# bastienjacquet/CudaDepthMapIntegration

Measured on AMD Instinct MI355X. Metric: Gvoxel-projections/s, higher is better.
Workload: dtype f64

## Files before the change

### cudadepthmapintegration_amd/csrc/dmi_capi.hip

```cpp
#include "dmi_context.h"

#include <chrono>
#include <cmath>
#include <cstdio>
#include <cstdlib>
#include <cstring>
#include <limits>

using dmi::Batch;
using dmi::drain_c2p;
using dmi::drain_events;
using dmi::EventPair;
using dmi::fail;
using dmi::flush_zero_fill;
using dmi::fuse_views;
using dmi::grid_axis_aligned;
using dmi::tile_eligible;
using dmi::FuseArgs;
using dmi::FuseConfig;
using dmi::guarded;
using dmi::MapRec;
using dmi::TileArgs;
using dmi::TileMapRec;

// ... 289 lines not shown
  if (!std::isfinite(czmin)) return;
  const bool per_lane = !(czmin > 0.0) || !(Sc / czmin + 1.0 < 0x1p22);
  const double pmax = per_lane ? 0.0 : Sc / czmin + 1.0;
  const bool index_exact = ((int64_t)ctx->views.H + 2 * dmi::kValidMargin + 8) * ((int64_t)ctx->views.W + 2 * dmi::kValidMargin) + ctx->views.H +
                               2 * dmi::kValidMargin < (int64_t(1) << 24);
  double e1 = cerr + 3.0 * 0x1p-24 * Dz * pmax + 0x1p-22 * Dz + nl * (pmax + 2.0) + 0x1p-53 * std::max(Sx, Sy);
  e1 *= 1.0 + 0x1p-10;
  t.t1_erel = 0x1p-22f * (1.0f + 0x1p-10f);
  t.t1_hspan = float_not_below(D * (1.0 + 0x1p-20));
  if (!(pmax < 0x1p22) || !index_exact || !(e1 > 0x1p-100) || !(Sc < 0x1p60) || !std::isfinite(e1)) return;
  t.t1_e1 = float_not_below(e1);
  t.t1_ok = 1;
  {
    const double *sp = ctx->grid.spacing;
    double d[3][2], c[3];
    for (int ax = 0; ax < 3; ++ax) {
      const double wxs = g[ax] * sp[ax], wys = g[4 + ax] * sp[ax], wzs = g[8 + ax] * sp[ax];
      d[ax][0] = (Pc[0] * wxs + Pc[1] * wys) + Pc[2] * wzs;
      d[ax][1] = (Qc[0] * wxs + Qc[1] * wys) + Qc[2] * wzs;
      c[ax] = (S[0] * wxs + S[1] * wys) + S[2] * wzs;
    }
    const double xpix = (double)(std::max(ctx->views.W, ctx->views.H) / 2 + dmi::kValidMargin + 1);
    const double xmax = xpix + (double)std::max(dmi::kWinAnchorX, dmi::kWinAnchorY);
    const double nl2 = 2.0 * nl;
    const double pwin = (dmi::kWinReach + 0.5) * dmi::kWinCzRatio + 3.0;
    const double steps[3] = {7.0, 7.0, (double)(kMaxColumn - 1)};
    double e_step = 0.0;
    for (int xy = 0; xy < 2; ++xy) {
      double e = 0.0;
      for (int ax = 0; ax < 3; ++ax) e += steps[ax] * (std::fabs(d[ax][xy]) + xmax * std::fabs(c[ax]));
      e_step = std::max(e_step, e * 0x1p-23);
    }
    double ew = (cerr + xmax * nl2) + e_step + pwin * nl2 + 0x1p-53 * std::max(Sx, Sy);
    ew *= 1.0 + 0x1p-10;
    bool ok = std::isfinite(ew) && ew > 0x1p-100 && ew < 0x1p60;
    for (int ax = 0; ax < 3; ++ax) ok = ok && std::fabs(d[ax][0]) < 0x1p60 && std::fabs(d[ax][1]) < 0x1p60 && std::fabs(c[ax]) < 0x1p60;
    if (ok) {
      for (int xy = 0; xy < 2; ++xy) {
        win->di[xy] = (float)d[0][xy];
        win->dj[xy] = (float)d[1][xy];
        win->dk[xy] = (float)d[2][xy];
      }
      win->ci[0] = (float)c[0]; win->ci[1] = (float)(c[0] * (double)dmi::kWinC1);
      win->cj[0] = (float)c[1]; win->cj[1] = (float)(c[1] * (double)dmi::kWinC1);
      win->ck[0] = (float)c[2]; win->ck[1] = (float)(c[2] * (double)dmi::kWinC1);
      win->e_abs = float_not_below(ew);
      for (int cnr = 0; cnr < 8; ++cnr) {
        const double ni = (cnr & 1) ? 7.0 : 0.0, nj = (cnr & 2) ? 7.0 : 0.0;
        for (int v = 0; v < 2; ++v) {
          const double nk = (cnr & 4) ? (v ? 15.0 : 7.0) : 0.0;
          float *dst = v ? foot->s16[cnr] : foot->s8[cnr];
          dst[0] = (float)((ni * d[0][0] + nj * d[1][0]) + nk * d[2][0]);
          dst[1] = (float)((ni * d[0][1] + nj * d[1][1]) + nk * d[2][1]);
          dst[2] = (float)((ni * c[0] + nj * c[1]) + nk * c[2]);
        }
      }
      foot->ferr = float_not_below(cerr + xpix * nl2);
    }
  }
  if (per_lane) {
    const double B = (3.0 * 0x1p-24 * Dz + nl) * (1.0 + 0x1p-10) * (1.0 + 0x1p-10);
    if (!(B < 0x1p60) || !(B >= 0.0)) {
      t.t1_ok = 0;
      t.t1_e1 = std::numeric_limits<float>::infinity();
      return;
    }
    t.t1_b = float_not_below(B);
    t.t1_ok = 2;
  }
}

TileMapRec make_tile_rec(const dmi_context *ctx, const MapRec &r, dmi::WinRec *win, dmi::FootRec *foot, double *zscale_out) {
  TileMapRec t;
  std::memset(&t, 0, sizeof(t));
  const double *rt = r.rt, *k = r.k;
  t.rz0 = rt[8];
  t.rz1 = rt[9];
  t.rz3 = rt[11];
  const bool general = classify_k(r.k, r.rt) == dmi::K_GENERAL;
  double P[4], Q[4], S[4];
  for (int c = 0; c < 4; ++c) {
    if (general) {
      P[c] = (k[0] * rt[c] + k[1] * rt[4 + c]) + k[2] * rt[8 + c];
      Q[c] = (k[4] * rt[c] + k[5] * rt[4 + c]) + k[6] * rt[8 + c];
      S[c] = (k[8] * rt[c] + k[9] * rt[4 + c]) + k[10] * rt[8 + c];
    } else {
      P[c] = k[0] * rt[c] + k[1] * rt[4 + c] + k[2] * rt[8 + c];
      Q[c] = k[5] * rt[4 + c] + k[6] * rt[8 + c];
      S[c] = rt[8 + c];
    }
  }
  if (general) {
    P[3] += k[3];
    Q[3] += k[7];
    S[3] += k[11];
  }
  t.px = P[0]; t.py = P[1]; t.pz = P[2]; t.p0 = P[3];
  t.qx = Q[0]; t.qy = Q[1]; t.qz = Q[2]; t.q0 = Q[3];
  t.sx = S[0]; t.sy = S[1]; t.sz = S[2]; t.s0 = S[3];
  const double *g = ctx->grid.grid_matrix;
  const double sz = ctx->grid.spacing[2];
  t.dhx = (P[0] * (g[2] * sz) + P[1] * (g[6] * sz)) + P[2] * (g[10] * sz);
  t.dhy = (Q[0] * (g[2] * sz) + Q[1] * (g[6] * sz)) + Q[2] * (g[10] * sz);
  t.dhz = (S[0] * (g[2] * sz) + S[1] * (g[6] * sz)) + S[2] * (g[10] * sz);
  double wm[3];
  const bool aligned = grid_axis_aligned(ctx->grid);
  if (aligned) {
    double lo[3], hi[3];
    voxel_world(ctx->grid, 0, 0, ctx->opt.z_first, lo);
    voxel_world(ctx->grid, ctx->grid.cell_dims[0] - 1, ctx->grid.cell_dims[1] - 1,
                ctx->opt.z_first + ctx->grid.cell_dims[2] - 1 + kMaxColumn, hi);
    for (int a = 0; a < 3; ++a) wm[a] = std::max(std::fabs(lo[a]), std::fabs(hi[a]));
  } else {
    double gm[3];
    for (int a = 0; a < 3; ++a)
      gm[a] = std::fabs(ctx->grid.origin[a]) +
              (ctx->grid.cell_dims[a] + 1.0 + (a == 2 ? ctx->opt.z_first + kMaxColumn : 0)) * std::fabs(ctx->grid.spacing[a]);
    for (int a = 0; a < 3; ++a)
      wm[a] = std::fabs(g[4 * a]) * gm[0] + std::fabs(g[4 * a + 1]) * gm[1] + std::fabs(g[4 * a + 2]) * gm[2] + std::fabs(g[4 * a + 3]);
  }
  double M[3];
  for (int row = 0; row < 3; ++row)
    M[row] = std::fabs(rt[4 * row]) * wm[0] + std::fabs(rt[4 * row + 1]) * wm[1] + std::fabs(rt[4 * row + 2]) * wm[2] +
             std::fabs(rt[4 * row + 3]);
  const double Sx = std::fabs(k[0]) * M[0] + std::fabs(k[1]) * M[1] + std::fabs(k[2]) * M[2] + (general ? std::fabs(k[3]) : 0.0);
  const double Sy = (general ? std::fabs(k[4]) * M[0] : 0.0) + std::fabs(k[5]) * M[1] + std::fabs(k[6]) * M[2] +
                    (general ? std::fabs(k[7]) : 0.0);
  const double Sz = general ? std::fabs(k[8]) * M[0] + std::fabs(k[9]) * M[1] + std::fabs(k[10]) * M[2] + std::fabs(k[11]) : M[2];
  t.err = std::max(Sx, Sy) * 0x1p-44;
  t.errz = general ? Sz * 0x1p-44 : 0.0;
  t.cz_err = aligned ? 0.0 : M[2] * 0x1p-47;
  double zabs = Sz, czlo = std::numeric_limits<double>::infinity(), czhi = -czlo;
  if (!general) {
    zabs = 0.0;
    for (int c = 0; c < 8; ++c) {
      double w[3];
      voxel_world(ctx->grid, (c & 1) ? ctx->grid.cell_dims[0] - 1 : 0, (c & 2) ? ctx->grid.cell_dims[1] - 1 : 0,
                  ctx->opt.z_first + ((c & 4) ? ctx->grid.cell_dims[2] - 1 + kMaxColumn : 0), w);
      const double cz = ((rt[8] * w[0] + rt[9] * w[1]) + rt[10] * w[2]) + rt[11];
      zabs = std::max(zabs, std::fabs(cz));
      czlo = std::min(czlo, cz);
      czhi = std::max(czhi, cz);
    }
    zabs = zabs * (1.0 + 0x1p-20) + (aligned ? 1.0 : 2.0) * 32.0 * 0x1p-52 * M[2];
    if (!std::isfinite(zabs)) zabs = Sz;
  }
  double zscale = 1.0;
  if (!general && std::isfinite(czlo) && std::isfinite(czhi)) zscale = std::max(1.0, std::max(czlo, czhi / 16.0));
  t.errk = (t.err + 65536.0 * t.errz) + 0x1p-22 * zabs * (1.0 + 0x1p-20);
  t.depth = r.depth;
  make_centred_rows(ctx, r, P, Q, S, Sx, Sy, M, zabs, zscale, general, aligned, &t, win, foot);
  if (zscale_out) *zscale_out = zscale;
  return t;
}

int add_views_impl(dmi_context *ctx, const double *depth64, const float *depth32, const double *best_cost,
                   double threshold, const double *K4, const double *RT4, int32_t n, int32_t width, int32_t height) {
  if (!ctx) return DMI_ERR_INVALID_ARGUMENT;
  if ((!depth64 && !depth32) || !K4 || !RT4) return fail(ctx, DMI_ERR_INVALID_ARGUMENT, "dmi_add_views: null pointer");
  if (n <= 0) return fail(ctx, DMI_ERR_INVALID_ARGUMENT, "dmi_add_views: n must be positive");
  if (width < 1 || height < 1 || width > 32768 || height > 32768)
    return fail(ctx, DMI_ERR_INVALID_ARGUMENT, "dmi_add_views: depth-map dimensions must be in [1, 32768]");
  if (!ctx->views.batches.empty() && (width != ctx->views.W || height != ctx->views.H))
    return fail(ctx, DMI_ERR_INVALID_ARGUMENT, "dmi_add_views: every view of a context must share width and height");
  DMI_HIP(ctx, hipSetDevice(ctx->opt.device));
  const auto t0 = std::chrono::steady_clock::now();
  if (ctx->views.batches.empty()) {
    ctx->views.W = width;
    ctx->views.H = height;
    ctx->views.depth_f64 = ctx->opt.depth_storage == DMI_DEPTH_F64;
    ctx->views.k_mode = ctx->finite_bounded ? (int)dmi::K_PINHOLE : (int)dmi::K_GENERAL;
    ctx->views.max_tile_err = 0.0;
    ctx->views.pyramid = dmi::make_pyramid_desc(width, height);
  }
  const size_t npix = (size_t)width * height;

  Batch b;
  unsigned long long lossy = 0;
  int rc = upload_batch(ctx, depth64, depth32, best_cost, threshold, n, &b, &lossy);
  if (rc != DMI_OK) return rc;
  if (lossy != 0 && !ctx->views.depth_f64 && ctx->opt.depth_storage == DMI_DEPTH_AUTO) {
    (void)hipFree(b.d_depth);
    (void)hipFree(b.d_pyramid);
    ctx->device_bytes -= npix * n * 4 + b.aux_bytes;
    rc = promote_to_f64(ctx);
    if (rc != DMI_OK) return rc;
    rc = upload_batch(ctx, depth64, depth32, best_cost, threshold, n, &b, &lossy);
    if (rc != DMI_OK) return rc;
  }
  ctx->views.batches.push_back(b);
  const size_t esz = depth_elem(ctx);
  for (int32_t m = 0; m < n; ++m) {
    MapRec r;
    std::memset(&r, 0, sizeof(r));
    std::memcpy(r.rt, RT4 + 16 * (size_t)m, 12 * sizeof(double));
    std::memcpy(r.k, K4 + 16 * (size_t)m, 12 * sizeof(double));
    r.depth = static_cast<const char *>(b.d_depth) + (size_t)m * npix * esz;
    r.pyramid = b.d_pyramid + (size_t)m * ctx->views.pyramid.total_tiles;
    ctx->views.h_maps.push_back(r);
    bool finite = true;
    for (int q = 0; q < 12; ++q) finite = finite && bounded(r.k[q]) && bounded(r.rt[q]);
    const int km = classify_k(r.k, r.rt);
    if (km < ctx->views.k_mode) ctx->views.k_mode = km;
    dmi::WinRec wrec;
    dmi::FootRec frec;
    double zscale = 1.0;
    TileMapRec t = make_tile_rec(ctx, r, &wrec, &frec, &zscale);
    t.valid = reinterpret_cast<const uint8_t *>(b.d_pyramid) + b.valid_offset + (size_t)m * (size_t)dmi::valid_map_bytes(ctx->views.W, ctx->views.H);
    t.vm_c0 = ((float)(ctx->views.H / 2 + dmi::kValidMargin) - 3.5f) * 0.125f;
    t.vm_w8 = (float)(8 * (ctx->views.W + 2 * dmi::kValidMargin) - 8);
    t.vm_base = 8 * (ctx->views.W / 2 + dmi::kValidMargin) + ctx->views.H / 2 + dmi::kValidMargin;
    t.vm_bytes = (int32_t)std::min<int64_t>(dmi::valid_map_bytes(ctx->views.W, ctx->views.H), 0x7fffffff);
    t.vbits = reinterpret_cast<const uint32_t *>(reinterpret_cast<const uint8_t *>(b.d_pyramid) + b.bits_offset +
                                                 (size_t)m * (size_t)dmi::valid_bits_bytes(ctx->views.W, ctx->views.H));
    t.vb_bytes = (int32_t)std::min<int64_t>(dmi::valid_bits_bytes(ctx->views.W, ctx->views.H), 0x7fffffff);
    t.vb_rowskip = (dmi::valid_bits_tiles_x(ctx->views.W) - 1) * 128;
    t.vb_mx = 0x4B400000 + dmi::kValidMargin + ctx->views.W / 2;
    t.vb_my = 0x4B400000 + dmi::kValidMargin + ctx->views.H / 2;
    ctx->views.h_tile_maps.push_back(t);
    wrec.vbits = t.vbits;
    ctx->views.h_win_recs.push_back(wrec);
    ctx->views.h_foot_recs.push_back(frec);
    if (!(t.err <= ctx->views.max_tile_err)) ctx->views.max_tile_err = t.err;
    ctx->views.view_k_mode.push_back((uint8_t)km);
    ctx->views.view_tile_ok.push_back(finite && t.err < 0x1p-12 * zscale && 65536.0 * t.errz < 0x1p-14 && t.cerrk < 0x1p-11 * zscale ? 1 : 0);
  }
  ctx->views.maps_dirty = true;
  ctx->timings.last_upload_ms =
      std::chrono::duration<double, std::milli>(std::chrono::steady_clock::now() - t0).count();
  return DMI_OK;
}

constexpr int64_t kConvertChunk = int64_t(32) << 20;

int ensure_convert_stage(dmi_context *ctx) {
  return dmi::ensure_buffer(ctx, ctx->volume.convert, (uint64_t)std::min<int64_t>(kConvertChunk, ctx->n_voxels) * 8);
}

template <typename HostT>
int upload_converted(dmi_context *ctx, const HostT *src) {
  int rc = ensure_convert_stage(ctx);
  if (rc != DMI_OK) return rc;
  const size_t gsz = grid_elem(ctx);
  for (int64_t i0 = 0; i0 < ctx->n_voxels; i0 += kConvertChunk) {
    const int64_t n = std::min<int64_t>(kConvertChunk, ctx->n_voxels - i0);
    DMI_HIP(ctx, hipMemcpyAsync(ctx->volume.convert.ptr, src + i0, (size_t)n * sizeof(HostT), hipMemcpyHostToDevice, ctx->stream));
    DMI_HIP(ctx, dmi::launch_convert_grid(ctx->volume.convert.ptr, sizeof(HostT) == 8 ? 1 : 0, static_cast<char *>(ctx->volume.d_grid) + (size_t)i0 * gsz, n,
                                          ctx->stream));
  }
  DMI_HIP(ctx, hipStreamSynchronize(ctx->stream));
  return DMI_OK;
}

template <typename HostT>
int download_converted(dmi_context *ctx, HostT *dst) {
  int rc = ensure_convert_stage(ctx);
  if (rc != DMI_OK) return rc;
  const size_t gsz = grid_elem(ctx);
  for (int64_t i0 = 0; i0 < ctx->n_voxels; i0 += kConvertChunk) {
    const int64_t n = std::min<int64_t>(kConvertChunk, ctx->n_voxels - i0);
    DMI_HIP(ctx, dmi::launch_convert_grid(static_cast<const char *>(ctx->volume.d_grid) + (size_t)i0 * gsz, gsz == 8 ? 1 : 0, ctx->volume.convert.ptr, n,
                                          ctx->stream));
    DMI_HIP(ctx, hipMemcpyAsync(dst + i0, ctx->volume.convert.ptr, (size_t)n * sizeof(HostT), hipMemcpyDeviceToHost, ctx->stream));
  }
  DMI_HIP(ctx, hipStreamSynchronize(ctx->stream));
  return DMI_OK;
}

}

extern "C" {

int dmi_abi_version(void) { return DMI_ABI_VERSION; }
size_t dmi_sizeof_info(void) { return sizeof(dmi_info); }
size_t dmi_sizeof_timings(void) { return sizeof(dmi_timings); }

int dmi_get_upload_kernel_ms(dmi_context *ctx, double *last, double *total) {
  if (!ctx) return DMI_ERR_INVALID_ARGUMENT;
  if (last) *last = ctx->views.last_upload_kernel_ms;
  if (total) *total = ctx->views.total_upload_kernel_ms;
  return DMI_OK;
}

int dmi_device_count(void) {
  int n = 0;
  if (hipGetDeviceCount(&n) != hipSuccess) {
    (void)hipGetLastError();
    return 0;
  }
  return n;
}

void dmi_default_options(dmi_options *opt) {
  if (!opt) return;
  std::memset(opt, 0, sizeof(*opt));
  opt->device = 0;
  opt->grid_dtype = DMI_F64;
  opt->depth_storage = DMI_DEPTH_AUTO;
}

const char *dmi_last_error(const dmi_context *ctx) { return ctx ? ctx->err.c_str() : g_create_error.c_str(); }

int dmi_create(const dmi_grid_desc *grid, const dmi_ray_potential *ray, const dmi_options *opt, dmi_context **out) {
  return guarded(nullptr, "dmi_create", [&]() -> int {
  auto bad = [](const char *m) {
    g_create_error = m;
    return (int)DMI_ERR_INVALID_ARGUMENT;
  };
  if (!grid || !ray || !out) return bad("dmi_create: null argument");
  *out = nullptr;
  for (int a = 0; a < 3; ++a)
    if (grid->cell_dims[a] < 1) return bad("dmi_create: cell_dims must be >= 1 (vtk point dims >= 2)");
  dmi_options o;
  dmi_default_options(&o);
  if (opt) o = *opt;
  if (o.grid_dtype != DMI_F32 && o.grid_dtype != DMI_F64) return bad("dmi_create: grid_dtype must be DMI_F32 or DMI_F64");
  if (o.depth_storage < DMI_DEPTH_AUTO || o.depth_storage > DMI_DEPTH_F64) return bad("dmi_create: bad depth_storage");
  if (o.z_first < 0 || (int64_t)o.z_first + grid->cell_dims[2] > (int64_t)0x3fffffff) return bad("dmi_create: z_first out of range");
  if (ray->rho == 0 && ray->thickness == 0) return bad("dmi_create: ray potential rho and thickness are both 0 (filt.cxx:138)");
  if ((int64_t)(grid->cell_dims[1] + 3) / 4 > 65535 || (int64_t)grid->cell_dims[2] > 65535)
    return bad("dmi_create: grid too large for one launch (ny <= 262140, nz <= 65535)");
  int ndev = dmi_device_count();
  if (ndev <= 0) return (g_create_error = "dmi_create: no HIP device available", (int)DMI_ERR_DEVICE);
  if (o.device < 0 || o.device >= ndev) return bad("dmi_create: device ordinal out of range");

  dmi_context *ctx = new (std::nothrow) dmi_context();
  if (!ctx) return (g_create_error = "dmi_create: host allocation failed", (int)DMI_ERR_OUT_OF_MEMORY);
  ctx->grid = *grid;
  ctx->ray = *ray;
  ctx->opt = o;
  ctx->n_voxels = (int64_t)grid->cell_dims[0] * grid->cell_dims[1] * grid->cell_dims[2];
  ctx->finite_bounded = true;
  for (int i = 0; i < 12; ++i) ctx->finite_bounded = ctx->finite_bounded && bounded(grid->grid_matrix[i]);
  for (int a = 0; a < 3; ++a)
    ctx->finite_bounded = ctx->finite_bounded && bounded(grid->origin[a]) &&
                          bounded(grid->spacing[a] * (grid->cell_dims[a] + 1.0 + (a == 2 ? o.z_first : 0)));

  auto hip_fail = [&](hipError_t e, const char *what) {
    (void)hipGetLastError();
    g_create_error = std::string("dmi_create: ") + what + ": " + hipGetErrorString(e);
    int code = e == hipErrorOutOfMemory ? DMI_ERR_OUT_OF_MEMORY : DMI_ERR_DEVICE;
    dmi_destroy(ctx);
    return code;
  };
  hipError_t e = hipSetDevice(o.device);
  if (e != hipSuccess) return hip_fail(e, "hipSetDevice");
  if (o.stream) {
    ctx->stream = static_cast<hipStream_t>(o.stream);
  } else {
    e = hipStreamCreateWithFlags(&ctx->stream, hipStreamNonBlocking);
    if (e != hipSuccess) return hip_fail(e, "hipStreamCreate");
    ctx->own_stream = true;
  }
  {
    int least = 0, greatest = 0;
    if (hipDeviceGetStreamPriorityRange(&least, &greatest) != hipSuccess) {
      (void)hipGetLastError();
      least = greatest = 0;
    }
    e = hipStreamCreateWithPriority(&ctx->upload_stream, hipStreamNonBlocking, greatest);
  }
  if (e != hipSuccess) return hip_fail(e, "hipStreamCreate(upload)");
  int rc = DMI_OK;
  auto own_failed = [&](int code) {
    rc = code;
    if (rc != DMI_OK) g_create_error = "dmi_create: " + ctx->err;
  };
  if (o.external_grid) {
    hipPointerAttribute_t attr;
    e = hipPointerGetAttributes(&attr, o.external_grid);
    if (e != hipSuccess || attr.type != hipMemoryTypeDevice) {
      (void)hipGetLastError();
      g_create_error = "dmi_create: external_grid is not a device pointer";
      dmi_destroy(ctx);
      return DMI_ERR_INVALID_ARGUMENT;
    }
    ctx->volume.d_grid = o.external_grid;
  } else {
    own_failed(dmi::ensure_buffer(ctx, ctx->volume.owned, ctx->n_voxels * grid_elem(ctx)));
    ctx->volume.d_grid = ctx->volume.owned.ptr;
    ctx->volume.own_grid = true;
  }
  if (rc == DMI_OK && o.count_hits) own_failed(dmi::ensure_buffer(ctx, ctx->hits.voxel, ctx->n_voxels * sizeof(uint32_t)));
  if (rc == DMI_OK) own_failed(dmi::ensure_buffer(ctx, ctx->views.lossy, 3 * sizeof(unsigned long long)));
  if (rc == DMI_OK && (hipEventCreate(&ctx->views.up_events[0]) != hipSuccess || hipEventCreate(&ctx->views.up_events[1]) != hipSuccess)) {
    (void)hipGetLastError();
    dmi::destroy_events(ctx->views.up_events);
  }
  if (rc == DMI_OK) own_failed(dmi_reset_grid(ctx));
  if (rc != DMI_OK) {
    dmi_destroy(ctx);
    return rc;
  }
  *out = ctx;
  return DMI_OK;
  });
}

void dmi_destroy(dmi_context *ctx) {
  if (!ctx) return;
  (void)hipSetDevice(ctx->opt.device);
  if (ctx->stream) (void)hipStreamSynchronize(ctx->stream);
  if (ctx->upload_stream) {
    (void)hipStreamSynchronize(ctx->upload_stream);
    (void)hipStreamDestroy(ctx->upload_stream);
  }
  for (EventPair &p : ctx->pending) {
    (void)hipEventDestroy(p.start);
    (void)hipEventDestroy(p.stop);
    (void)hipEventDestroy(p.mid);
  }
  for (EventPair &p : ctx->pool) {
    (void)hipEventDestroy(p.start);
    (void)hipEventDestroy(p.stop);
    (void)hipEventDestroy(p.mid);
  }
  ctx->views.release();
  ctx->hits.release();
  ctx->volume.release();
  ctx->tables.release();
  ctx->c2p.release();
  ctx->mesh.release();
  ctx->extraction.release();
  ctx->components.release();
  ctx->smoothing.release();
  ctx->decimation.release();
  ctx->support.release();
  ctx->coloration.release();
  for (hipEvent_t e : ctx->slab_events) (void)hipEventDestroy(e);
  if (ctx->download_stream) (void)hipStreamDestroy(ctx->download_stream);
  if (ctx->own_stream && ctx->stream) (void)hipStreamDestroy(ctx->stream);
  delete ctx;
}

int dmi_add_views(dmi_context *ctx, const double *depth, const double *best_cost, double threshold, const double *K4,
                  const double *RT4, int32_t n, int32_t width, int32_t height) {
  return guarded(ctx, "dmi_add_views", [&]() -> int {
  return add_views_impl(ctx, depth, nullptr, best_cost, threshold, K4, RT4, n, width, height);
  });
}

int dmi_add_views_f32(dmi_context *ctx, const float *depth, const double *K4, const double *RT4, int32_t n,
                      int32_t width, int32_t height) {
  return guarded(ctx, "dmi_add_views_f32", [&]() -> int {
  return add_views_impl(ctx, nullptr, depth, nullptr, 0.0, K4, RT4, n, width, height);
  });
}

int dmi_clear_views(dmi_context *ctx) {
  return guarded(ctx, "dmi_clear_views", [&]() -> int {
  if (!ctx) return DMI_ERR_INVALID_ARGUMENT;
  DMI_HIP(ctx, hipSetDevice(ctx->opt.device));
  DMI_HIP(ctx, hipStreamSynchronize(ctx->stream));
  const size_t npix = (size_t)ctx->views.W * ctx->views.H;
  for (Batch &b : ctx->views.batches) {
    (void)hipFree(b.d_depth);
    (void)hipFree(b.d_pyramid);
    ctx->device_bytes -= npix * b.n * depth_elem(ctx) + b.aux_bytes;
  }
  ctx->views.batches.clear();
  ctx->views.h_maps.clear();
  ctx->views.h_tile_maps.clear();
  ctx->views.h_win_recs.clear();
  ctx->views.h_foot_recs.clear();
  ctx->views.view_k_mode.clear();
  ctx->views.view_tile_ok.clear();
  ctx->views.max_tile_err = 0.0;
  ctx->views.maps_dirty = true;
  ctx->views.W = ctx->views.H = 0;
  return DMI_OK;
  });
}

int dmi_reset_grid(dmi_context *ctx) {
  return guarded(ctx, "dmi_reset_grid", [&]() -> int {
  if (!ctx) return DMI_ERR_INVALID_ARGUMENT;
  DMI_HIP(ctx, hipSetDevice(ctx->opt.device));
  if (ctx->volume.own_grid) {
    ctx->volume.zero_fill_pending = true;
  } else {
    DMI_HIP(ctx, hipMemsetAsync(ctx->volume.d_grid, 0, ctx->n_voxels * grid_elem(ctx), ctx->stream));
  }
  if (ctx->hits.voxel.ptr) DMI_HIP(ctx, hipMemsetAsync(ctx->hits.voxel.ptr, 0, ctx->n_voxels * sizeof(uint32_t), ctx->stream));
  if (ctx->hits.map.ptr)
    DMI_HIP(ctx, hipMemsetAsync(ctx->hits.map.ptr, 0, ctx->hits.map.capacity, ctx->stream));
  ctx->volume.layer_is_zero.assign((size_t)ctx->grid.cell_dims[2], 1);
  ctx->volume.grid_free_of_negative_zero = ctx->volume.own_grid;
  ctx->c2p.valid = false;
  return DMI_OK;
  });
}

int dmi_upload_grid(dmi_context *ctx, const double *grid) {
  return guarded(ctx, "dmi_upload_grid", [&]() -> int {
  if (!ctx || !grid) return fail(ctx, DMI_ERR_INVALID_ARGUMENT, "dmi_upload_grid: null argument");
  DMI_HIP(ctx, hipSetDevice(ctx->opt.device));
  ctx->volume.zero_fill_pending = false;
  if (ctx->opt.grid_dtype == DMI_F64) {
    DMI_HIP(ctx, hipMemcpyAsync(ctx->volume.d_grid, grid, ctx->n_voxels * 8, hipMemcpyHostToDevice, ctx->stream));
    DMI_HIP(ctx, hipStreamSynchronize(ctx->stream));
  } else {
    int rc_ = upload_converted<double>(ctx, grid);
    if (rc_ != DMI_OK) return rc_;
  }
  ctx->volume.layer_is_zero.assign((size_t)ctx->grid.cell_dims[2], 0);
  ctx->volume.grid_free_of_negative_zero = false;
  ctx->c2p.valid = false;
  return DMI_OK;
  });
}

int dmi_synchronize(dmi_context *ctx) {
  return guarded(ctx, "dmi_synchronize", [&]() -> int {
  if (!ctx) return DMI_ERR_INVALID_ARGUMENT;
  DMI_HIP(ctx, hipSetDevice(ctx->opt.device));
  DMI_HIP(ctx, hipStreamSynchronize(ctx->stream));
  return drain_events(ctx);
  });
}

int dmi_download_grid_f64(dmi_context *ctx, double *out) {
  return guarded(ctx, "dmi_download_grid_f64", [&]() -> int {
  if (!ctx || !out) return fail(ctx, DMI_ERR_INVALID_ARGUMENT, "dmi_download_grid_f64: null argument");
  DMI_HIP(ctx, hipSetDevice(ctx->opt.device));
  { int rc_ = flush_zero_fill(ctx); if (rc_ != DMI_OK) return rc_; }
  const auto t0 = std::chrono::steady_clock::now();
  if (ctx->opt.grid_dtype == DMI_F64) {
    DMI_HIP(ctx, hipMemcpyAsync(out, ctx->volume.d_grid, ctx->n_voxels * 8, hipMemcpyDeviceToHost, ctx->stream));
    DMI_HIP(ctx, hipStreamSynchronize(ctx->stream));
  } else {
    int rc_ = download_converted<double>(ctx, out);
    if (rc_ != DMI_OK) return rc_;
  }
  ctx->timings.last_download_ms =
      std::chrono::duration<double, std::milli>(std::chrono::steady_clock::now() - t0).count();
  return drain_events(ctx);
  });
}

int dmi_download_grid_f32(dmi_context *ctx, float *out) {
  return guarded(ctx, "dmi_download_grid_f32", [&]() -> int {
  if (!ctx || !out) return fail(ctx, DMI_ERR_INVALID_ARGUMENT, "dmi_download_grid_f32: null argument");
  DMI_HIP(ctx, hipSetDevice(ctx->opt.device));
  { int rc_ = flush_zero_fill(ctx); if (rc_ != DMI_OK) return rc_; }
  const auto t0 = std::chrono::steady_clock::now();
  if (ctx->opt.grid_dtype == DMI_F32) {
    DMI_HIP(ctx, hipMemcpyAsync(out, ctx->volume.d_grid, ctx->n_voxels * 4, hipMemcpyDeviceToHost, ctx->stream));
    DMI_HIP(ctx, hipStreamSynchronize(ctx->stream));
  } else {
    int rc_ = download_converted<float>(ctx, out);
    if (rc_ != DMI_OK) return rc_;
  }
  ctx->timings.last_download_ms =
      std::chrono::duration<double, std::milli>(std::chrono::steady_clock::now() - t0).count();
  return drain_events(ctx);
  });
}

int dmi_fuse_range_download(dmi_context *ctx, int32_t first, int32_t count, void *out, int32_t out_dtype, int32_t n_slabs) {
  return guarded(ctx, "dmi_fuse_range_download", [&]() -> int {
  if (!ctx || !out) return fail(ctx, DMI_ERR_INVALID_ARGUMENT, "dmi_fuse_range_download: null argument");
  if (out_dtype != DMI_F64 && out_dtype != DMI_F32) return fail(ctx, DMI_ERR_INVALID_ARGUMENT, "dmi_fuse_range_download: out_dtype must be DMI_F32 or DMI_F64");
  DMI_HIP(ctx, hipSetDevice(ctx->opt.device));
  const int32_t n_views = (int32_t)ctx->views.h_maps.size();
  if (first < 0 || count < 0 || first > n_views || count > n_views - first)
    return fail(ctx, DMI_ERR_INVALID_ARGUMENT, "dmi_fuse_range_download: range outside the resident views");
  const int32_t nz = ctx->grid.cell_dims[2];
  const int32_t max_slabs = std::max(1, (nz + DMI_SLAB_ALIGNMENT - 1) / DMI_SLAB_ALIGNMENT);
  n_slabs = std::min(std::max(n_slabs, 1), max_slabs);
  if (out_dtype != ctx->opt.grid_dtype || n_slabs == 1) {
    if (count > 0) {
      int rc = fuse_views(ctx, first, count, 0, nz);
      if (rc != DMI_OK) return rc;
    }
    return out_dtype == DMI_F64 ? dmi_download_grid_f64(ctx, static_cast<double *>(out)) : dmi_download_grid_f32(ctx, static_cast<float *>(out));
  }
  { int rc_ = flush_zero_fill(ctx); if (rc_ != DMI_OK) return rc_; }
  if (!ctx->download_stream) DMI_HIP(ctx, hipStreamCreateWithFlags(&ctx->download_stream, hipStreamNonBlocking));
  while ((int32_t)ctx->slab_events.size() < n_slabs) {
    hipEvent_t e = nullptr;
    DMI_HIP(ctx, hipEventCreateWithFlags(&e, hipEventDisableTiming));
    ctx->slab_events.push_back(e);
  }
  const auto t0 = std::chrono::steady_clock::now();
  const int32_t units = max_slabs, per = units / n_slabs, extra = units % n_slabs;
  const size_t gsz = grid_elem(ctx);
  const size_t layer = (size_t)ctx->grid.cell_dims[0] * ctx->grid.cell_dims[1];
  int32_t z0 = 0;
  for (int32_t i = 0; i < n_slabs; ++i) {
    const int32_t z1 = std::min(nz, z0 + (per + (i < extra ? 1 : 0)) * DMI_SLAB_ALIGNMENT);
    if (count > 0) {
      int rc = fuse_views(ctx, first, count, z0, z1 - z0);
      if (rc != DMI_OK) {
        (void)hipStreamSynchronize(ctx->download_stream);
        return rc;
      }
    }
    hipError_t he = hipEventRecord(ctx->slab_events[(size_t)i], ctx->stream);
    if (he == hipSuccess) he = hipStreamWaitEvent(ctx->download_stream, ctx->slab_events[(size_t)i], 0);
    if (he == hipSuccess)
      he = hipMemcpyAsync(static_cast<char *>(out) + (size_t)z0 * layer * gsz, static_cast<const char *>(ctx->volume.d_grid) + (size_t)z0 * layer * gsz,
                          (size_t)(z1 - z0) * layer * gsz, hipMemcpyDeviceToHost, ctx->download_stream);
    if (he != hipSuccess) {
      (void)hipStreamSynchronize(ctx->download_stream);
      (void)hipGetLastError();
      return fail(ctx, DMI_ERR_DEVICE, std::string("dmi_fuse_range_download: ") + hipGetErrorString(he));
    }
    z0 = z1;
  }
  DMI_HIP(ctx, hipStreamSynchronize(ctx->download_stream));
  DMI_HIP(ctx, hipStreamSynchronize(ctx->stream));
  ctx->timings.last_download_ms =
      std::chrono::duration<double, std::milli>(std::chrono::steady_clock::now() - t0).count();
  return drain_events(ctx);
  });
}

// ... 237 lines not shown
```

### cudadepthmapintegration_amd/csrc/dmi_capi_fuse.hip

```cpp
#include "dmi_context.h"

#include <algorithm>
#include <cmath>
#include <cstdlib>
#include <cstring>

using dmi::drain_events;
using dmi::EventPair;
using dmi::fail;
using dmi::flush_zero_fill;
using dmi::FuseArgs;
using dmi::FuseConfig;
using dmi::guarded;
using dmi::MapRec;
using dmi::TileArgs;
using dmi::TileMapRec;

namespace {

int sync_maps(dmi_context *ctx) {
  dmi_context::Views &v = ctx->views;
  const size_t n = v.h_maps.size();
  const size_t cap = std::max<size_t>(64, n * 2);
  bool fresh = false;
  int rc = dmi::ensure_idle_buffers(ctx, {{&v.maps, n * sizeof(MapRec), cap * sizeof(MapRec)},
                                          {&v.tile_maps, n * sizeof(TileMapRec), cap * sizeof(TileMapRec)},
                                          {&v.win_recs, n * sizeof(dmi::WinRec), cap * sizeof(dmi::WinRec)},
                                          {&v.foot_recs, n * sizeof(dmi::FootRec), cap * sizeof(dmi::FootRec)}}, &fresh);
  if (rc != DMI_OK) return rc;
  if (fresh) v.maps_dirty = true;
  dmi::DeviceBuffer &hits = ctx->hits.map;
  if (ctx->opt.count_hits && !dmi::holds(hits, n * sizeof(unsigned long long))) {
    dmi::DeviceBuffer grown;
    rc = dmi::ensure_buffer(ctx, grown, cap * sizeof(unsigned long long));
    if (rc != DMI_OK) return rc;
    hipError_t e = hipMemsetAsync(grown.ptr, 0, grown.capacity, ctx->stream);
    if (e == hipSuccess && hits.ptr) {
      e = hipMemcpyAsync(grown.ptr, hits.ptr, hits.capacity, hipMemcpyDeviceToDevice, ctx->stream);
      if (e == hipSuccess) e = hipStreamSynchronize(ctx->stream);
    }
    if (e != hipSuccess) {
      (void)hipGetLastError();
      dmi::drop_buffers(ctx, {&grown});
      return fail(ctx, DMI_ERR_DEVICE, std::string("growth of the views' hit counters: ") + hipGetErrorString(e));
    }
    std::swap(grown, hits);
    dmi::drop_buffers(ctx, {&grown});
  }
  if (v.maps_dirty) {
    DMI_HIP(ctx, hipMemcpyAsync(v.maps.ptr, v.h_maps.data(), n * sizeof(MapRec), hipMemcpyHostToDevice, ctx->stream));
    DMI_HIP(ctx, hipMemcpyAsync(v.tile_maps.ptr, v.h_tile_maps.data(), n * sizeof(TileMapRec), hipMemcpyHostToDevice, ctx->stream));
    DMI_HIP(ctx, hipMemcpyAsync(v.win_recs.ptr, v.h_win_recs.data(), n * sizeof(dmi::WinRec), hipMemcpyHostToDevice, ctx->stream));
    DMI_HIP(ctx, hipMemcpyAsync(v.foot_recs.ptr, v.h_foot_recs.data(), n * sizeof(dmi::FootRec), hipMemcpyHostToDevice, ctx->stream));
    v.maps_dirty = false;
  }
  return DMI_OK;
}

int slot_permutation(dmi_context *ctx, int32_t super_x, int32_t super_y, int32_t super_z, bool zmajor, const int32_t **out) {
  std::vector<dmi_context::SlotPerm> &perms = ctx->tables.slot_perms;
  for (const auto &sp : perms)
    if (sp.super_x == super_x && sp.super_y == super_y && sp.super_z == super_z && sp.zmajor == (zmajor ? 1 : 0)) {
      *out = sp.perm.as<int32_t>();
      return DMI_OK;
    }
  if (super_x > 1023 || super_y > 1023 || super_z > 1023)
    return fail(ctx, DMI_ERR_INVALID_ARGUMENT, "dmi_fuse: more than 1023 super-bricks along an axis");
  const size_t n = (size_t)super_x * super_y * super_z;
  auto spread = [](uint64_t v) {
    v &= 0x3ff;
    v = (v | (v << 16)) & 0x030000ffull;
    v = (v | (v << 8)) & 0x0300f00full;
    v = (v | (v << 4)) & 0x030c30c3ull;
    v = (v | (v << 2)) & 0x09249249ull;
    return v;
  };
  std::vector<std::pair<uint64_t, int32_t>> keyed(n);
  size_t q = 0;
  for (int32_t z = 0; z < super_z; ++z)
    for (int32_t y = 0; y < super_y; ++y)
      for (int32_t x = 0; x < super_x; ++x, ++q)
        keyed[q] = {zmajor ? (uint64_t)q : (spread(x) | (spread(y) << 1) | (spread(z) << 2)), x | (y << 10) | (z << 20)};
  if (!zmajor) std::sort(keyed.begin(), keyed.end());
  std::vector<int32_t> perm(n);
  for (size_t i = 0; i < n; ++i) perm[i] = keyed[i].second;
  dmi::DeviceBuffer d;
  const int rc = dmi::ensure_buffer(ctx, d, n * sizeof(int32_t));
  if (rc != DMI_OK) return rc;
  hipError_t e = hipMemcpyAsync(d.ptr, perm.data(), n * sizeof(int32_t), hipMemcpyHostToDevice, ctx->stream);
  if (e == hipSuccess && perms.size() >= 64) {
    e = hipStreamSynchronize(ctx->stream);
    if (e == hipSuccess) {
      for (auto &sp : perms) dmi::drop_buffers(ctx, {&sp.perm});
      perms.clear();
    }
  }
  if (e != hipSuccess) {
    (void)hipGetLastError();
    dmi::drop_buffers(ctx, {&d});
    return fail(ctx, DMI_ERR_DEVICE, std::string("slot permutation upload: ") + hipGetErrorString(e));
  }
  perms.push_back({super_x, super_y, super_z, zmajor ? 1 : 0, d});
  *out = d.as<int32_t>();
  return DMI_OK;
}


FuseArgs general_args(const dmi_context *ctx, int32_t first, int32_t count, int32_t z_first, int32_t z_count) {
  FuseArgs a;
  std::memset(&a, 0, sizeof(a));
  a.nx = ctx->grid.cell_dims[0];
  a.ny = ctx->grid.cell_dims[1];
  a.nz = ctx->grid.cell_dims[2];
  a.W = ctx->views.W;
  a.H = ctx->views.H;
  a.first_map = first;
  a.n_maps = count;
  a.init_from_grid = 0;
  for (int32_t z = z_first; z < z_first + z_count; ++z)
    if (!ctx->volume.layer_is_zero[(size_t)z]) a.init_from_grid = 1;
  a.kz0 = ctx->opt.z_first;
  a.k_first = z_first;
  a.k_count = z_count;
  a.ox = ctx->grid.origin[0];
  a.oy = ctx->grid.origin[1];
  a.oz = ctx->grid.origin[2];
  a.sx = ctx->grid.spacing[0];
  a.sy = ctx->grid.spacing[1];
  a.sz = ctx->grid.spacing[2];
  std::memcpy(a.g, ctx->grid.grid_matrix, 12 * sizeof(double));
  a.thick = ctx->ray.thickness;
  a.delta = ctx->ray.delta;
  a.rho_pos = ctx->ray.rho * 1.0;
  a.rho_neg = ctx->ray.rho * -1.0;
  a.rho_zero = ctx->ray.rho * 0.0;
  a.slope = ctx->ray.rho / ctx->ray.thickness;
  a.free_space = -ctx->ray.eta * ctx->ray.rho;
  a.maps = ctx->views.maps.as<MapRec>();
  a.grid = ctx->volume.d_grid;
  a.voxel_hits = ctx->hits.voxel.as<uint32_t>();
  a.map_hits = ctx->hits.map.as<unsigned long long>();
  return a;
}

dmi::HoleTraits resident_hole_traits(const dmi_context::Views &v) {
  unsigned long long mingled = 0, without = 0, strips = 0, pixels = 0;
  for (const dmi::Batch &bt : v.batches) {
    mingled += bt.mingled_strips;
    without += bt.holes;
    strips += (unsigned long long)bt.n * (unsigned long long)v.W * (unsigned long long)(v.H / 8);
    pixels += (unsigned long long)bt.n * (unsigned long long)v.W * (unsigned long long)v.H;
  }
  return dmi::hole_traits(mingled, without, strips, pixels);
}

int tile_geometry(dmi_context *ctx, const FuseArgs &a, const FuseConfig &cfg, const dmi::TileShape &sh, bool whole_grid, TileArgs *out) {
  TileArgs &t = *out;
  t.nx = a.nx; t.ny = a.ny; t.nz = a.nz; t.W = a.W; t.H = a.H;
  t.first_map = a.first_map; t.n_maps = a.n_maps; t.init_from_grid = a.init_from_grid;
  t.kpad = (a.nz + sh.tk - 1) / sh.tk * sh.tk;
  t.bricks_x = (a.nx + 8 * sh.wx - 1) / (8 * sh.wx);
  t.bricks_y = (a.ny + 8 * sh.wy - 1) / (8 * sh.wy);
  t.bricks_z = t.kpad / sh.tk;
  t.super_x = (t.bricks_x + 3) / 4;
  t.super_y = (t.bricks_y + 3) / 4;
  t.super_z = (t.bricks_z + 1) / 2;
  if (!whole_grid) {
    t.sbz_first = a.k_first / (2 * sh.tk);
    t.super_z = (a.k_first + a.k_count + 2 * sh.tk - 1) / (2 * sh.tk) - t.sbz_first;
  }
  if (t.bricks_x > 2047 || t.bricks_y > 2047 || t.bricks_z > 1023)
    return fail(ctx, DMI_ERR_INVALID_ARGUMENT, "dmi_fuse: more bricks along an axis than the tiled kernel's order entries hold");
  t.slot_base = t.sbz_first * t.super_x * t.super_y * 32;
  t.slot_count = t.super_x * t.super_y * t.super_z * 32;
  const int rc = slot_permutation(ctx, t.super_x, t.super_y, t.super_z, (cfg.variant & dmi::VAR_ZMAJOR_SLOTS) != 0, &t.sb_perm);
  if (rc != DMI_OK) return rc;
  t.xcd_run_wg = 32 * std::max(1, t.super_x * t.super_y);
  if (((int64_t)t.super_x * t.super_y * t.super_z * 32 + 16 * (int64_t)t.xcd_run_wg + 64) > (int64_t)0x7fffffff)
    return fail(ctx, DMI_ERR_INVALID_ARGUMENT, "dmi_fuse: grid too large for one launch");
  t.depth_bytes = (int32_t)((int64_t)a.W * a.H * (ctx->views.depth_f64 ? 8 : 4));
  t.kz0 = a.kz0;
  t.ox = a.ox; t.oy = a.oy; t.oz = a.oz; t.sx = a.sx; t.sy = a.sy; t.sz = a.sz;
  std::memcpy(t.g, a.g, sizeof(t.g));
  t.thick = a.thick; t.delta = a.delta; t.rho_pos = a.rho_pos; t.rho_neg = a.rho_neg;
  t.slope = a.slope; t.free_space = a.free_space;
  t.tile_maps = ctx->views.tile_maps.as<TileMapRec>();
  t.grid = a.grid; t.voxel_hits = a.voxel_hits; t.map_hits = a.map_hits;
  t.rotated = dmi::grid_axis_aligned(ctx->grid) ? 0 : 1;
  t.flags = ((cfg.variant & dmi::VAR_NO_INTERIOR) ? dmi::TILE_FLAG_NO_INTERIOR : 0) |
            ((cfg.variant & dmi::VAR_XCD_RUNS) ? dmi::TILE_FLAG_XCD_RUNS : 0);
  t.maps = ctx->views.maps.as<MapRec>();
  t.wbricks_x = (a.nx + 7) / 8;
  t.wbricks_y = (a.ny + 7) / 8;
  return DMI_OK;
}

int cz_table(dmi_context *ctx, const FuseArgs &a, TileArgs *t) {
  const size_t table_doubles = std::max<size_t>(ctx->views.h_maps.size(), 4) * (size_t)t->kpad;
  const size_t need = table_doubles + (size_t)dmi::kFreeSumsMax + 1;
  const int rc = dmi::ensure_idle_buffer(ctx, ctx->tables.cz_table, need * 8, need * 2 * 8);
  if (rc != DMI_OK) return rc;
  t->cz_table = ctx->tables.cz_table.as<double>();
  if (!a.init_from_grid && !ctx->opt.count_hits && a.n_maps <= dmi::kFreeSumsMax) t->free_sums = t->cz_table + table_doubles;
  return DMI_OK;
}

int zero_row(dmi_context *ctx, TileArgs *t) {
  bool fresh = false;
  const int rc = dmi::ensure_idle_buffer(ctx, ctx->tables.zero_row, (uint64_t)t->class_pitch, (uint64_t)t->class_pitch, &fresh);
  if (rc != DMI_OK) return rc;
  if (fresh) DMI_HIP(ctx, hipMemsetAsync(ctx->tables.zero_row.ptr, dmi::BRICK_MIXED, (size_t)t->class_pitch, ctx->stream));
  t->classes = ctx->tables.zero_row.as<uint8_t>();
  t->class_pitch = 0;
  return DMI_OK;
}

int class_table(dmi_context *ctx, const dmi::TileShape &sh, bool windows, TileArgs *t) {
  const size_t fine_bytes = ((size_t)t->wbricks_x * t->wbricks_y * t->bricks_z * (size_t)t->class_pitch + 255) / 256 * 256;
  const size_t coarse_end = (fine_bytes + (size_t)dmi::coarse_class_bytes(*t, sh.tk) + 255) / 256 * 256;
  const size_t cbytes = coarse_end + (windows ? fine_bytes * sizeof(dmi::WinPair) : 0);
  ctx->tables.coarse_offset = fine_bytes;
  bool fresh = false;
  const int rc = dmi::ensure_idle_buffer(ctx, ctx->tables.classes, cbytes, cbytes, &fresh);
  if (rc != DMI_OK) return rc;
  if (fresh) DMI_HIP(ctx, hipMemsetAsync(ctx->tables.classes.ptr, dmi::BRICK_SKIP, cbytes, ctx->stream));
  t->classes = ctx->tables.classes.as<uint8_t>();
  if (windows) {
    t->win_origin = reinterpret_cast<dmi::WinPair *>(ctx->tables.classes.as<uint8_t>() + coarse_end);
    t->win_delta = (int64_t)reinterpret_cast<intptr_t>(t->win_origin) - 16 * (int64_t)reinterpret_cast<intptr_t>(t->classes);
    t->win_recs = ctx->views.win_recs.as<dmi::WinRec>();
    t->foot_recs = ctx->views.foot_recs.as<dmi::FootRec>();
    t->vb_bytes = (int32_t)std::min<int64_t>(dmi::valid_bits_bytes(ctx->views.W, ctx->views.H), 0x7fffffff);
    t->vb_rowskip = (dmi::valid_bits_tiles_x(ctx->views.W) - 1) * 128;
    t->win_cx = dmi::kValidMargin + ctx->views.W / 2;
    t->win_cy = dmi::kValidMargin + ctx->views.H / 2;
  }
  return DMI_OK;
}

int order_tables(dmi_context *ctx, const dmi::TileShape &sh, int variant, TileArgs *t) {
  const size_t n_slots = (size_t)t->super_x * t->super_y * t->super_z * 32;
  const size_t order_bytes = (n_slots + 1) * sizeof(int32_t), level_bytes = dmi::order_scratch_bytes(n_slots);
  const int rc = dmi::ensure_idle_buffers(ctx, {{&ctx->tables.order, order_bytes, order_bytes}, {&ctx->tables.order_level, level_bytes, level_bytes}});
  if (rc != DMI_OK) return rc;
  t->order = ctx->tables.order.as<int32_t>() + 1;
  t->n_order = ctx->tables.order.as<int32_t>();
  t->order_levels = reinterpret_cast<const int32_t *>(ctx->tables.order_level.as<uint8_t>() + (n_slots + 15) / 16 * 16);
  t->xcd_run_wg = 32 * (4 / (sh.wx * sh.wy));
  if (dmi::cost_order(sh.wx * sh.wy, variant, n_slots)) {
    t->flags |= dmi::TILE_FLAG_COST_ORDER | dmi::TILE_FLAG_XCD_RUNS;
    t->xcd_run_wg = 16;
  }
  return DMI_OK;
}

#ifdef DMI_TUNING
int tuning_hooks(dmi_context *ctx, TileArgs *out) {
  TileArgs &t = *out;
  if (std::getenv("DMI_DEBUG_NO_DEPTH_LOADS")) t.depth_bytes = 0;
  if (std::getenv("DMI_DEBUG_WG_TIMES")) {
    const size_t per_round = 8 * (size_t)t.xcd_run_wg;
    const size_t blocks = ((size_t)t.super_x * t.super_y * t.super_z * 32 + 32 + per_round - 1) / per_round * per_round;
    const size_t bytes = (blocks * 3 + 2) * sizeof(unsigned long long);
    const int rc = dmi::ensure_idle_buffer(ctx, ctx->tables.wg_times, bytes, bytes);
    if (rc != DMI_OK) return rc;
    ctx->tables.wg_times_blocks = blocks;
    DMI_HIP(ctx, hipMemsetAsync(ctx->tables.wg_times.ptr, 0, bytes, ctx->stream));
    t.wg_times = ctx->tables.wg_times.as<unsigned long long>();
    t.wg_times_n = (int64_t)blocks;
  }
  if (const char *e = std::getenv("DMI_DEBUG_PAIRS")) {
    if (!std::strcmp(e, "nowin")) t.flags |= dmi::TILE_FLAG_DBG_SKIP_WINDOW_PAIRS;
    if (!std::strcmp(e, "onlywin")) t.flags |= dmi::TILE_FLAG_DBG_ONLY_WINDOW_PAIRS;
    if (!std::strcmp(e, "nowinloads")) t.flags |= dmi::TILE_FLAG_DBG_NO_WINDOW_LOADS;
  }
  if (const char *e = std::getenv("DMI_XCD_RUN_WG")) {
    t.xcd_run_wg = std::max(1, std::atoi(e));
    if (((int64_t)t.super_x * t.super_y * t.super_z * 32 + 8 * (int64_t)t.xcd_run_wg) > (int64_t)0x7fffffff)
      return fail(ctx, DMI_ERR_INVALID_ARGUMENT, "dmi_fuse: DMI_XCD_RUN_WG makes the launch too large");
  }
  return DMI_OK;
}
#endif

int tile_tables(dmi_context *ctx, const FuseArgs &a, FuseConfig *cfg, const dmi::TileShape &sh, const dmi::HoleTraits &traits, TileArgs *out) {
  TileArgs &t = *out;
  int rc = cz_table(ctx, a, &t);
  if (rc == DMI_OK) rc = dmi::ensure_buffer(ctx, ctx->tables.queue_heads, 128 * sizeof(int32_t));
  if (rc != DMI_OK) return rc;
  t.queue_heads = ctx->tables.queue_heads.as<int32_t>();
  if (dmi::fuse_without_classes(cfg->variant, (int64_t)t.wbricks_x * t.wbricks_y * (int64_t)t.bricks_z, a.n_maps))
    cfg->variant |= dmi::VAR_NO_BRICK_CLASSES;
  t.class_pitch = dmi::class_table_pitch((int32_t)ctx->views.h_maps.size());
  const bool zero_free = dmi::zero_free(a.init_from_grid != 0, ctx->volume.grid_free_of_negative_zero, ctx->opt.count_hits != 0, cfg->variant);
  if (cfg->variant & dmi::VAR_NO_BRICK_CLASSES) {
    rc = zero_row(ctx, &t);
  } else {
    bool any_tier1 = false;
    for (int32_t m = a.first_map; m < a.first_map + a.n_maps && !any_tier1; ++m) any_tier1 = std::isfinite(ctx->views.h_win_recs[(size_t)m].e_abs);
    dmi::WindowsQuestion q;
    q.tier1 = DMI_TIER1 != 0;
    q.general_k = cfg->general_k != 0;
    q.count_hits = cfg->count_hits != 0;
    q.variant = cfg->variant;
    q.holes = cfg->holes != 0;
    q.many_borders = traits.many_borders;
    q.any_tier1 = any_tier1;
    q.zero_free = zero_free;
    q.depth_f64 = ctx->views.depth_f64;
    rc = class_table(ctx, sh, dmi::use_windows(q), &t);
    if (rc == DMI_OK && !(cfg->variant & dmi::VAR_SPATIAL_ORDER)) rc = order_tables(ctx, sh, cfg->variant, &t);
  }
  if (zero_free) t.behind_mask = 0x0101010101010101ull;
  return rc;
}

int timed_launch(dmi_context *ctx, const FuseArgs &a, const TileArgs &t, const FuseConfig &cfg) {
  EventPair ev;
  if (!ctx->pool.empty()) {
    ev = ctx->pool.back();
    ctx->pool.pop_back();
  } else {
    DMI_HIP(ctx, hipEventCreate(&ev.start));
    DMI_HIP(ctx, hipEventCreate(&ev.stop));
    DMI_HIP(ctx, hipEventCreate(&ev.mid));
  }
  ev.has_mid = cfg.use_tile != 0 && !(cfg.variant & dmi::VAR_NO_BRICK_CLASSES);
  DMI_HIP(ctx, hipEventRecord(ev.start, ctx->stream));
  const dmi_context::LaunchTables &tb = ctx->tables;
  hipError_t e = cfg.use_tile ? dmi::launch_fuse_tiled(t, ctx->views.maps.as<MapRec>(), cfg, ctx->views.pyramid, tb.order_level.as<uint8_t>(),
                                                         tb.classes.ptr ? tb.classes.as<uint8_t>() + tb.coarse_offset : nullptr,
                                                         ev.has_mid ? ev.mid : nullptr, ctx->stream) : dmi::launch_fuse(a, cfg, ctx->stream);
  if (e != hipSuccess) {
    ctx->pool.push_back(ev);
    (void)hipGetLastError();
    return fail(ctx, DMI_ERR_DEVICE, std::string("fusion kernel launch: ") + hipGetErrorString(e));
  }
  DMI_HIP(ctx, hipEventRecord(ev.stop, ctx->stream));
  ctx->pending.push_back(ev);
  return DMI_OK;
}

int fuse_run(dmi_context *ctx, int32_t first, int32_t count, int32_t z_first, int32_t z_count, bool tiled, int run_k_mode,
             bool general_k) {
  DMI_HIP(ctx, hipSetDevice(ctx->opt.device));
  int rc = sync_maps(ctx);
  if (rc != DMI_OK) return rc;
  const bool whole_grid = z_first == 0 && z_count == ctx->grid.cell_dims[2];
  if (!whole_grid) {
    rc = flush_zero_fill(ctx);
    if (rc != DMI_OK) return rc;
  }
  const FuseArgs a = general_args(ctx, first, count, z_first, z_count);

  const dmi::HoleTraits traits = resident_hole_traits(ctx->views);
  FuseConfig cfg;
  cfg.depth_is_f64 = ctx->views.depth_f64 ? 1 : 0;
  cfg.grid_is_f64 = ctx->opt.grid_dtype == DMI_F64 ? 1 : 0;
  cfg.k_mode = run_k_mode;
  cfg.count_hits = ctx->opt.count_hits ? 1 : 0;
  cfg.use_tile = tiled ? 1 : 0;
  cfg.general_k = tiled && general_k ? 1 : 0;
  cfg.holes = traits.holes ? 1 : 0;
  cfg.variant = dmi::with_default_tile_shape(ctx->opt.kernel_variant, tiled, traits, a.nx, a.ny, a.nz);

  TileArgs t;
  std::memset(&t, 0, sizeof(t));
  if (cfg.use_tile) {
    const dmi::TileShape sh = dmi::tile_shape(cfg.variant, ctx->views.depth_f64, !dmi::grid_axis_aligned(ctx->grid), cfg.general_k != 0);
    rc = tile_geometry(ctx, a, cfg, sh, whole_grid, &t);
    if (rc == DMI_OK) rc = tile_tables(ctx, a, &cfg, sh, traits, &t);
#ifdef DMI_TUNING
    if (rc == DMI_OK) rc = tuning_hooks(ctx, &t);
#endif
    if (rc == DMI_OK) rc = dmi::ensure_buffer(ctx, ctx->tables.fuse_args, sizeof(FuseArgs));
    if (rc != DMI_OK) return rc;
    DMI_HIP(ctx, hipMemcpyAsync(ctx->tables.fuse_args.ptr, &a, sizeof(FuseArgs), hipMemcpyHostToDevice, ctx->stream));
    t.full = ctx->tables.fuse_args.as<FuseArgs>();
  }

  rc = timed_launch(ctx, a, t, cfg);
  if (rc != DMI_OK) return rc;

  dmi_context::LastLaunch &last = ctx->last;
  last.tiled = cfg.use_tile != 0;
  last.classes = cfg.use_tile != 0 && !(cfg.variant & dmi::VAR_NO_BRICK_CLASSES);
  last.class_bricks = (int64_t)t.wbricks_x * t.wbricks_y * t.bricks_z;
  last.bricks_z = t.bricks_z;
  last.tk = t.bricks_z > 0 ? t.kpad / t.bricks_z : 0;
  last.win_origin = t.win_origin;
  last.class_pitch = t.class_pitch;
  last.first = first;
  last.count = count;
  for (int32_t z = z_first; z < z_first + z_count; ++z) ctx->volume.layer_is_zero[(size_t)z] = 0;
  ctx->volume.zero_fill_pending = false;
  ctx->c2p.valid = false;
  if (ctx->pending.size() >= 256) return drain_events(ctx);
  return DMI_OK;
}

template <typename Visit>
int visit_last_classes(dmi_context *ctx, Visit &&visit) {
  const dmi_context::LastLaunch &last = ctx->last;
  if (!last.classes) return DMI_OK;
  DMI_HIP(ctx, hipSetDevice(ctx->opt.device));
  const size_t bytes = (size_t)last.class_bricks * last.class_pitch;
  std::vector<uint8_t> host(bytes);
  DMI_HIP(ctx, hipMemcpyAsync(host.data(), ctx->tables.classes.ptr, bytes, hipMemcpyDeviceToHost, ctx->stream));
  DMI_HIP(ctx, hipStreamSynchronize(ctx->stream));
  for (int64_t b = 0; b < last.class_bricks; ++b) {
    const uint8_t *row = host.data() + (size_t)b * last.class_pitch + last.first;
    for (int32_t m = 0; m < last.count; ++m) visit(b, row[m]);
  }
  return DMI_OK;
}

}

namespace dmi {

int fuse_views(dmi_context *ctx, int32_t first, int32_t count, int32_t z_first, int32_t z_count) {
  const dmi_context::Views &v = ctx->views;
  const int32_t n_views = (int32_t)v.h_maps.size();
  if (n_views == 0) return fail(ctx, DMI_ERR_STATE, "dmi_fuse: no views resident (call dmi_add_views first)");
  if (first < 0 || count < 0 || first > n_views || count > n_views - first)
    return fail(ctx, DMI_ERR_INVALID_ARGUMENT, "dmi_fuse_range: range outside the resident views");
  if (count == 0) return DMI_OK;
  const bool tile_possible = tile_eligible(ctx);
  int32_t m = first;
  while (m < first + count) {
    const bool tiled = tile_possible && v.view_tile_ok[(size_t)m];
    int32_t e = m;
    int km = dmi::K_PINHOLE;
    bool general_k = false;
    while (e < first + count && (tile_possible && v.view_tile_ok[(size_t)e]) == tiled) {
      km = std::min(km, (int)v.view_k_mode[(size_t)e]);
      general_k = general_k || v.view_k_mode[(size_t)e] == dmi::K_GENERAL;
      ++e;
    }
    const int rc = fuse_run(ctx, m, e - m, z_first, z_count, tiled, km, general_k);
    if (rc != DMI_OK) return rc;
    m = e;
  }
  return DMI_OK;
}

}

extern "C" {

int dmi_fuse_range(dmi_context *ctx, int32_t first, int32_t count) {
  return guarded(ctx, "dmi_fuse_range", [&]() -> int {
  if (!ctx) return DMI_ERR_INVALID_ARGUMENT;
  return dmi::fuse_views(ctx, first, count, 0, ctx->grid.cell_dims[2]);
  });
}

int dmi_fuse_slab(dmi_context *ctx, int32_t z_first, int32_t z_count) {
  return guarded(ctx, "dmi_fuse_slab", [&]() -> int {
  if (!ctx) return DMI_ERR_INVALID_ARGUMENT;
  const int32_t nz = ctx->grid.cell_dims[2];
  if (z_first < 0 || z_count < 0 || z_first > nz || z_count > nz - z_first)
    return fail(ctx, DMI_ERR_INVALID_ARGUMENT, "dmi_fuse_slab: layers outside the grid");
  if (z_first % DMI_SLAB_ALIGNMENT != 0 || (z_first + z_count != nz && (z_first + z_count) % DMI_SLAB_ALIGNMENT != 0))
    return fail(ctx, DMI_ERR_INVALID_ARGUMENT, "dmi_fuse_slab: slab boundaries must be multiples of DMI_SLAB_ALIGNMENT (32) cells");
  if (z_count == 0) return DMI_OK;
  return dmi::fuse_views(ctx, 0, (int32_t)ctx->views.h_maps.size(), z_first, z_count);
  });
}

int dmi_fuse(dmi_context *ctx) {
  return guarded(ctx, "dmi_fuse", [&]() -> int {
  if (!ctx) return DMI_ERR_INVALID_ARGUMENT;
  return dmi_fuse_range(ctx, 0, (int32_t)ctx->views.h_maps.size());
  });
}

int dmi_get_brick_class_histogram(dmi_context *ctx, uint64_t out[4]) {
  return guarded(ctx, "dmi_get_brick_class_histogram", [&]() -> int {
  if (!ctx || !out) return fail(ctx, DMI_ERR_INVALID_ARGUMENT, "dmi_get_brick_class_histogram: null argument");
  out[0] = out[1] = out[2] = out[3] = 0;
  return visit_last_classes(ctx, [&](int64_t, uint8_t c) { out[c & 3] += 1; });
  });
}

int dmi_get_mixed_reason_histogram(dmi_context *ctx, uint64_t out[8]) {
  return guarded(ctx, "dmi_get_mixed_reason_histogram", [&]() -> int {
  if (!ctx || !out) return fail(ctx, DMI_ERR_INVALID_ARGUMENT, "dmi_get_mixed_reason_histogram: null argument");
  for (int i = 0; i < 8; ++i) out[i] = 0;
  return visit_last_classes(ctx, [&](int64_t, uint8_t c) {
    if ((c & 3) == dmi::BRICK_MIXED) out[(c >> 2) & 7] += 1;
  });
  });
}

int dmi_get_window_pair_count(dmi_context *ctx, uint64_t *out) {
  return guarded(ctx, "dmi_get_window_pair_count", [&]() -> int {
  if (!ctx || !out) return fail(ctx, DMI_ERR_INVALID_ARGUMENT, "dmi_get_window_pair_count: null argument");
  *out = 0;
  const dmi_context::LastLaunch &last = ctx->last;
  if (!last.win_origin) return DMI_OK;
  const int64_t per_layer = last.class_bricks / std::max<int64_t>(1, last.bricks_z);
  return visit_last_classes(ctx, [&](int64_t b, uint8_t c) {
    const int64_t bz = b / std::max<int64_t>(1, per_layer);
    if (bz * last.tk + last.tk > ctx->grid.cell_dims[2]) return;
    if ((c & 0x3f) == (dmi::BRICK_MIXED | (dmi::MIXED_FREE_OR_NODEPTH << 2))) *out += 1;
  });
  });
}

}
```

### cudadepthmapintegration_amd/csrc/dmi_context.h

```cpp
#pragma once
#include "../../include/dmi.h"
#include "dmi_buffer.h"
#include "fusion_kernels.h"

#include <exception>
#include <initializer_list>
#include <new>
#include <string>
#include <vector>

namespace dmi {

struct Batch {
  void *d_depth = nullptr;
  DepthTile *d_pyramid = nullptr;
  size_t valid_offset = 0;
  size_t bits_offset = 0;
  size_t aux_bytes = 0;
  int32_t n = 0;
  unsigned long long holes = 0;
  unsigned long long mingled_strips = 0;
};

struct EventPair {
  hipEvent_t start = nullptr, stop = nullptr;
  hipEvent_t mid = nullptr;
  bool has_mid = false;
};

template <size_t N>
void destroy_events(hipEvent_t (&events)[N]) {
  for (hipEvent_t &e : events) {
    if (e) (void)hipEventDestroy(e);
    e = nullptr;
  }
}
}

struct dmi_context {
  dmi_grid_desc grid{};
  dmi_ray_potential ray{};
  dmi_options opt{};
  int64_t n_voxels = 0;

  hipStream_t stream = nullptr;
  bool own_stream = false;
  hipStream_t upload_stream = nullptr;
  hipStream_t download_stream = nullptr;
  std::vector<hipEvent_t> slab_events;

  bool finite_bounded = true;

  struct Views {
    int32_t W = 0, H = 0;
    bool depth_f64 = false;
    int k_mode = dmi::K_PINHOLE;
    std::vector<uint8_t> view_k_mode;
    std::vector<uint8_t> view_tile_ok;
    double max_tile_err = 0.0;
    dmi::PyramidDesc pyramid{};
    std::vector<dmi::Batch> batches;
    std::vector<dmi::MapRec> h_maps;
    std::vector<dmi::TileMapRec> h_tile_maps;
    std::vector<dmi::WinRec> h_win_recs;
    std::vector<dmi::FootRec> h_foot_recs;
    dmi::DeviceBuffer maps, tile_maps, win_recs, foot_recs;
    bool maps_dirty = false;
    dmi::DeviceBuffer stage_depth, stage_cost;
    dmi::DeviceBuffer lossy;
    hipEvent_t up_events[2] = {nullptr, nullptr};
    double last_upload_kernel_ms = 0.0, total_upload_kernel_ms = 0.0;
    void release() {
      for (dmi::Batch &b : batches) {
        (void)hipFree(b.d_depth);
        (void)hipFree(b.d_pyramid);
      }
      batches.clear();
      dmi::free_buffers({&maps, &tile_maps, &win_recs, &foot_recs, &stage_depth, &stage_cost, &lossy});
      dmi::destroy_events(up_events);
    }
  } views;
  struct Hits {
    dmi::DeviceBuffer voxel;
    dmi::DeviceBuffer map;
    void release() { dmi::free_buffers({&voxel, &map}); }
  } hits;
  struct Volume {
    void *d_grid = nullptr;
    dmi::DeviceBuffer owned;
    bool own_grid = false;
    std::vector<uint8_t> layer_is_zero;
    bool zero_fill_pending = false;
    bool grid_free_of_negative_zero = false;
    dmi::DeviceBuffer convert;
    void release() {
      dmi::free_buffers({&owned, &convert});
      d_grid = nullptr;
    }
  } volume;
  struct SlotPerm {
    int32_t super_x, super_y, super_z, zmajor;
    dmi::DeviceBuffer perm;
  };
  struct LaunchTables {
    dmi::DeviceBuffer cz_table;
    dmi::DeviceBuffer fuse_args;
    dmi::DeviceBuffer zero_row;
    dmi::DeviceBuffer classes;
    size_t coarse_offset = 0;
    dmi::DeviceBuffer queue_heads;
    dmi::DeviceBuffer wg_times;
    size_t wg_times_blocks = 0;
    std::vector<SlotPerm> slot_perms;
    dmi::DeviceBuffer order, order_level;
    void release() {
      for (SlotPerm &sp : slot_perms) dmi::free_buffers({&sp.perm});
      slot_perms.clear();
      dmi::free_buffers({&cz_table, &fuse_args, &zero_row, &classes, &queue_heads, &wg_times, &order, &order_level});
    }
  } tables;
  struct LastLaunch {
    bool tiled = false;
    bool classes = false;
    int64_t class_bricks = 0;
    int32_t bricks_z = 0, tk = 0;
    const dmi::WinPair *win_origin = nullptr;
    int32_t class_pitch = 0, first = 0, count = 0;
  } last;

  struct CellToPoint {
    dmi::DeviceBuffer points;
    bool valid = false;
    hipEvent_t events[2] = {nullptr, nullptr};
    bool pending = false;
    void release() { dmi::free_buffers({&points}); dmi::destroy_events(events); }
  } c2p;
  struct Mesh {
    dmi::DeviceBuffer vertices, triangles, normals;
    dmi::DeviceBuffer alt_vertices, alt_triangles, alt_normals;
    dmi::DeviceBuffer region_id, region_size;
    uint64_t n_vertices = 0, n_triangles = 0;
    uint64_t regions = 0;
    bool valid = false;
    bool has_normals = false;
    bool filtered = false;
    dmi::DeviceBuffer color_mean, color_median, color_count;
    dmi::DeviceBuffer alt_color_mean, alt_color_median, alt_color_count;
    bool colored = false;
    void release() {
      dmi::free_buffers({&vertices, &triangles, &normals, &alt_vertices, &alt_triangles, &alt_normals, &region_id, &region_size,
                         &color_mean, &color_median, &color_count, &alt_color_mean, &alt_color_median, &alt_color_count});
    }
  } mesh;
  struct Extraction {
    dmi::DeviceBuffer counts, bases, scan_temp;
    hipEvent_t events[4] = {nullptr, nullptr, nullptr, nullptr};
    double last_kernel_ms = 0.0;
    void release() { dmi::free_buffers({&counts, &bases, &scan_temp}); dmi::destroy_events(events); }
  } extraction;
  struct Components {
    dmi::DeviceBuffer vertex_scratch;
    dmi::DeviceBuffer triangle_scratch, counters, scan_temp;
    hipEvent_t events[5] = {nullptr, nullptr, nullptr, nullptr, nullptr};
    double last_kernel_ms = 0.0;
    uint64_t last_cas_retries = 0;
    double last_pass_ms[4] = {0.0, 0.0, 0.0, 0.0};
    void release() { dmi::free_buffers({&vertex_scratch, &triangle_scratch, &counters, &scan_temp}); dmi::destroy_events(events); }
  } components;
  struct Smoothing {
    dmi::DeviceBuffer vertices;
    dmi::DeviceBuffer keys;
    dmi::DeviceBuffer vertex_scratch;
    dmi::DeviceBuffer temp;
    hipEvent_t events[4] = {nullptr, nullptr, nullptr, nullptr};
    double last_kernel_ms = 0.0;
    double last_pass_ms[3] = {0.0, 0.0, 0.0};
    void release() { dmi::free_buffers({&vertices, &keys, &vertex_scratch, &temp}); dmi::destroy_events(events); }
  } smoothing;
  struct Decimation {
    dmi::DeviceBuffer vertex_scratch;
    dmi::DeviceBuffer triangle_scratch;
    dmi::DeviceBuffer bounds;
    hipEvent_t events[8] = {nullptr, nullptr, nullptr, nullptr, nullptr, nullptr, nullptr, nullptr};
    bool pending = false;
    bool pending_normals = false;
    double last_kernel_ms = 0.0;
    double last_pass_ms[4] = {0.0, 0.0, 0.0, 0.0};
    void release() { dmi::free_buffers({&vertex_scratch, &triangle_scratch, &bounds}); dmi::destroy_events(events); }
  } decimation;

  struct Support {
    dmi::DeviceBuffer counts;
    dmi::DeviceBuffer work, compacted;
    dmi::DeviceBuffer maps;
    dmi::DeviceBuffer vertex_scratch;
    dmi::DeviceBuffer triangle_scratch, scan_temp;
    bool valid = false;
    hipEvent_t events[4] = {nullptr, nullptr, nullptr, nullptr};
    double last_kernel_ms = 0.0;
    double last_pass_ms[3] = {0.0, 0.0, 0.0};
    void release() {
      dmi::free_buffers({&counts, &work, &compacted, &maps, &vertex_scratch, &triangle_scratch, &scan_temp});
      dmi::destroy_events(events);
    }
  } support;

  struct Coloration {
    hipEvent_t events[1] = {nullptr};
    double last_kernel_ms = 0.0;
    void release() { dmi::destroy_events(events); }
  } coloration;

  std::vector<dmi::EventPair> pending, pool;
  dmi_timings timings{};
  uint64_t device_bytes = 0;
  std::string err;
};

namespace dmi {

int fail(dmi_context *ctx, int code, const std::string &msg);
int drain_events(dmi_context *ctx);
int drain_c2p(dmi_context *ctx);
int flush_zero_fill(dmi_context *ctx);
inline size_t grid_elem(const dmi_context *c) { return c->opt.grid_dtype == DMI_F64 ? 8 : 4; }
bool grid_axis_aligned(const dmi_grid_desc &g);
bool tile_eligible(const dmi_context *ctx);
int fuse_views(dmi_context *ctx, int32_t first, int32_t count, int32_t z_first, int32_t z_count);
int ensure_buffer(dmi_context *ctx, DeviceBuffer &buffer, uint64_t bytes);
int ensure_idle_buffers(dmi_context *ctx, std::initializer_list<BufferGrowth> unit, bool *fresh = nullptr);
inline int ensure_idle_buffer(dmi_context *ctx, DeviceBuffer &buffer, uint64_t needed, uint64_t allocate, bool *fresh = nullptr) {
  return ensure_idle_buffers(ctx, {{&buffer, needed, allocate}}, fresh);
}
void drop_buffers(dmi_context *ctx, std::initializer_list<DeviceBuffer *> buffers);
struct BufferNeed {
  DeviceBuffer *buffer;
  uint64_t bytes;
};
int ensure_buffers(dmi_context *ctx, std::initializer_list<BufferNeed> needs);

template <typename Ctx, typename Body>
int guarded_by(int (*fail)(Ctx *, int, const std::string &), Ctx *ctx, const char *entry, Body &&body) noexcept {
  auto report = [&](int code, const char *what) noexcept {
    try {
      return fail(ctx, code, std::string(entry) + ": " + what);
    } catch (...) {
      return code;
    }
  };
  try {
    return body();
  } catch (const std::bad_alloc &) {
    return report(DMI_ERR_OUT_OF_MEMORY, "host allocation failed");
  } catch (const std::exception &e) {
    return report(DMI_ERR_STATE, e.what());
  } catch (...) {
    return report(DMI_ERR_STATE, "unexpected C++ exception");
  }
}
template <typename Body>
int guarded(dmi_context *ctx, const char *entry, Body &&body) noexcept {
  return guarded_by(&fail, ctx, entry, static_cast<Body &&>(body));
}


struct ColorContextShape {
  int32_t device, W, H;
  int64_t n_views;
  bool depth_test;
};
ColorContextShape color_context_shape(const dmi_color_context *c);
struct DeviceColoring {
  const double *points;
  int64_t n;
  uint8_t *mean, *median;
  int32_t *count;
  hipEvent_t after;
  const void *const *fused_tables;
  bool fused_f64;
// ... 18 lines not shown
```

### cudadepthmapintegration_amd/csrc/fusion_classify.hip

```cpp
#include <algorithm>
#include <cstring>

#include <stdlib.h>

#include "fusion_kernels.h"
#include "fusion_device.h"

namespace dmi {

namespace {

template <typename T>
__device__ __forceinline__ T cload(const T *p) {
  return *reinterpret_cast<const T __attribute__((address_space(4))) *>(reinterpret_cast<uintptr_t>(p));
}

__device__ __forceinline__ float float_below(double d) {
  float f = (float)d;
  if ((double)f > d) f = nextafterf(f, -__builtin_inff());
  return f;
}
__device__ __forceinline__ float float_above(double d) {
  float f = (float)d;
  if ((double)f < d) f = nextafterf(f, __builtin_inff());
// ... 403 lines not shown
  uint8_t cls = fp.cls;
  bool speckled = false;
  if (fp.query) {
    const TileAcc d = pyramid_query<5>(maps[m].pyramid, P, fp.x0, fp.x1, fp.y0, fp.y1);
    cls = class_from_bounds(a, d, fp.czmin, fp.czmax);
    speckled = !(d.flags & (TILE_PART_HOLE_FREE | TILE_PART_NO_VALID));
  } else if (fp.partial) {
    cls = border_class<GK>(a, fp, pyramid_query<5>(maps[m].pyramid, P, fp.x0, fp.x1, fp.y0, fp.y1));
  }
  const bool inherit_mixed = cls == (uint8_t)(BRICK_MIXED | (MIXED_FREE_OR_NODEPTH << 2)) && speckled;
  coarse[(int64_t)((cbz * cy_n + cby) * cx_n + cbx) * a.class_pitch + m] = inherit_mixed ? (uint8_t)(cls | COARSE_CHILDREN_WRITTEN) : cls;
  if ((cls & 3) == BRICK_MIXED && !inherit_mixed) return;
  for (int dz = 0; dz < per_z; ++dz) {
    const int bz = bz0 + dz;
    if (bz >= bz_first + bz_count) break;
    for (int dy = 0; dy < 4; ++dy) {
      const int by = cby * 4 + dy;
      if (by >= a.wbricks_y) break;
      for (int dx = 0; dx < 4; ++dx) {
        const int bx = cbx * 4 + dx;
        if (bx >= a.wbricks_x) break;
        classes[(int64_t)((bz * a.wbricks_y + by) * a.wbricks_x + bx) * a.class_pitch + m] = cls;
      }
    }
  }
}

constexpr int kWindow = 16;

template <int kQueryTiles, int kChildren, bool ROT, bool GK>
__global__ __launch_bounds__(256) void classify_kernel(const TileArgs a, const MapRec *__restrict__ maps,
                                                       const PyramidDesc P, int tk, uint8_t *__restrict__ classes,
                                                       const uint8_t *__restrict__ coarse, int group_views) {
  constexpr int children = kChildren;
  constexpr int views_per_wave = 64 / children;
  constexpr int per_z = children / 16;
  __shared__ float2 window_mm[4 * views_per_wave][kWindow * kWindow];
  __shared__ uint8_t window_fl[4 * views_per_wave][kWindow * kWindow];
  const int bz_first = 2 * a.sbz_first;
  const int bz_count = min(2 * a.super_z, a.bricks_z - bz_first);
  const int cx_n = (a.wbricks_x + 3) / 4, cy_n = (a.wbricks_y + 3) / 4;
  const int lane = threadIdx.x & 63, wave = __builtin_amdgcn_readfirstlane(threadIdx.x >> 6);
  const int local = blockIdx.x;
  const int cbx = local % cx_n;
  const int ct = local / cx_n;
  const int cby = ct % cy_n, cbz = ct / cy_n + bz_first / per_z;
  const int chunk0 = blockIdx.y * group_views;
  const uint8_t *__restrict__ crow = coarse + (int64_t)((cbz * cy_n + cby) * cx_n + cbx) * a.class_pitch + a.first_map + chunk0;
  const unsigned long long unproven = __builtin_amdgcn_ballot_w64(
      lane < group_views && chunk0 + lane < a.n_maps && (crow[lane] & (3 | COARSE_CHILDREN_WRITTEN)) == BRICK_MIXED);
  if (unproven == 0) return;
  unsigned long long items = views_per_wave == 1 ? unproven & (0x1111111111111111ull << wave)
                                                 : (unproven | (unproven >> 1)) & (0x0101010101010101ull << (2 * wave));
  const int child = lane % children;
  const int bx = cbx * 4 + (child & 3), by = cby * 4 + ((child >> 2) & 3), bz = cbz * per_z + (child >> 4);
  const bool in_grid = bx < a.wbricks_x && by < a.wbricks_y && bz < bz_first + bz_count;
  uint8_t *__restrict__ out = classes + (int64_t)((bz * a.wbricks_y + by) * a.wbricks_x + bx) * a.class_pitch;
  while (items) {
    const int first = __builtin_ctzll(items);
    items &= items - 1;
    const int rel = first + lane / children;
    const int mm = chunk0 + rel;
    const int m = a.first_map + min(mm, a.n_maps - 1);
    const bool mine = in_grid && ((unproven >> rel) & 1ull);
    const MapRec *__restrict__ mr = maps + m;
    BoxFootprint fp;
    fp.query = false;
    fp.partial = false;
    fp.in_margin = false;
    fp.cls = BRICK_SKIP;
    MapRec mr_u;
    TileMapRec tr_u;
    if constexpr (views_per_wave == 1) {
      const int mu = __builtin_amdgcn_readfirstlane(m);
      const MapRec *src = maps + mu;
      const TileMapRec *tsrc = a.tile_maps + mu;
#pragma unroll
      for (int q = 8; q < 12; ++q) mr_u.rt[q] = cload(&src->rt[q]);
      mr_u.pyramid = cload(&src->pyramid);
      tr_u.px = cload(&tsrc->px); tr_u.py = cload(&tsrc->py); tr_u.pz = cload(&tsrc->pz); tr_u.p0 = cload(&tsrc->p0);
      tr_u.qx = cload(&tsrc->qx); tr_u.qy = cload(&tsrc->qy); tr_u.qz = cload(&tsrc->qz); tr_u.q0 = cload(&tsrc->q0);
      tr_u.err = cload(&tsrc->err);
      tr_u.cz_err = cload(&tsrc->cz_err);
      tr_u.errz = cload(&tsrc->errz);
      if constexpr (GK) {
        tr_u.sx = cload(&tsrc->sx); tr_u.sy = cload(&tsrc->sy); tr_u.sz = cload(&tsrc->sz); tr_u.s0 = cload(&tsrc->s0);
      }
      mr = &mr_u;
      if (mine) {
        fp = box_footprint<ROT, GK>(a, &mr_u, &tr_u, bx * 8, bx * 8 + 7, by * 8, by * 8 + 7, bz * tk, bz * tk + tk - 1);
      }
    } else {
      if (mine) fp = box_footprint<ROT, GK>(a, mr, a.tile_maps + m, bx * 8, bx * 8 + 7, by * 8, by * 8 + 7, bz * tk, bz * tk + tk - 1);
    }
    const bool query = mine && (fp.query || fp.partial);
    uint8_t cls = fp.cls;
    const int li = query ? query_level<kQueryTiles>(P, max(fp.x1 - fp.x0, fp.y1 - fp.y0) + 1) : 0x7fff;
    bool from_window = false;
    {
      float2 *__restrict__ win_mm = window_mm[wave * views_per_wave + lane / children];
      uint8_t *__restrict__ win_fl = window_fl[wave * views_per_wave + lane / children];
      int li_w = li;
      for (int off = children >> 1; off > 0; off >>= 1) li_w = min(li_w, __shfl_xor(li_w, off, 64));
      if (li_w != 0x7fff) {
        const int L = kPyramidMinLevel + li_w;
        const bool at_level = query && li == li_w;
        int tx0 = at_level ? fp.x0 >> L : 0x7fffffff, ty0 = at_level ? fp.y0 >> L : 0x7fffffff;
        int tx1 = at_level ? fp.x1 >> L : -1, ty1 = at_level ? fp.y1 >> L : -1;
        int wx0 = tx0, wy0 = ty0, wx1 = tx1, wy1 = ty1;
        for (int off = children >> 1; off > 0; off >>= 1) {
          wx0 = min(wx0, __shfl_xor(wx0, off, 64));
          wy0 = min(wy0, __shfl_xor(wy0, off, 64));
          wx1 = max(wx1, __shfl_xor(wx1, off, 64));
          wy1 = max(wy1, __shfl_xor(wy1, off, 64));
        }
        if (wx1 - wx0 < kWindow && wy1 - wy0 < kWindow) {
          const DepthTile *__restrict__ level = mr->pyramid + P.offset[li_w];
          const int pitch = P.width[li_w];
          const int ww = wx1 - wx0 + 1, wh = wy1 - wy0 + 1;
          const int tx = child & 15;
          for (int ty = child >> 4; ty < wh; ty += children / 16)
            if (tx < ww) {
              const DepthTile t = level[(wy0 + ty) * pitch + wx0 + tx];
              win_mm[ty * kWindow + tx] = make_float2(t.dmin, t.dmax);
              win_fl[ty * kWindow + tx] = (uint8_t)t.flags;
            }
          __builtin_amdgcn_fence(__ATOMIC_RELEASE, "wavefront");
          __builtin_amdgcn_wave_barrier();
          __builtin_amdgcn_fence(__ATOMIC_ACQUIRE, "wavefront");
          if (at_level) {
            TileAcc d;
            for (int ty = ty0; ty <= ty1; ++ty)
              for (int tx = tx0; tx <= tx1; ++tx) {
                const int w = (ty - wy0) * kWindow + (tx - wx0);
                const float2 mm = win_mm[w];
                d.add_tile(DepthTile{mm.x, mm.y, (uint32_t)win_fl[w], 0u});
              }
            cls = fp.partial ? border_class<GK>(a, fp, d) : class_from_bounds(a, d, fp.czmin, fp.czmax);
            from_window = true;
          }
          __builtin_amdgcn_fence(__ATOMIC_RELEASE, "wavefront");
          __builtin_amdgcn_wave_barrier();
        }
      }
    }
    if (query && !from_window) {
      const TileAcc d = pyramid_query<kQueryTiles>(mr->pyramid, P, fp.x0, fp.x1, fp.y0, fp.y1);
      cls = fp.partial ? border_class<GK>(a, fp, d) : class_from_bounds(a, d, fp.czmin, fp.czmax);
    }
    if (mine) out[m] = cls;
  }
}

constexpr int kOriginViews = 8;
constexpr uint32_t kNotWanted = 0xfffffffeu;
template <bool ROT>
__global__ __launch_bounds__(256) void window_origin_kernel(const TileArgs a, const MapRec *__restrict__ maps, int tk,
                                                            uint8_t *__restrict__ classes, WinPair *__restrict__ origins,
                                                            int group_views) {
  __shared__ WinPair tile[kOriginViews][256 + 1];
  __shared__ int64_t rows[256];
  const int bz_first = 2 * a.sbz_first;
  const int bz_count = min(2 * a.super_z, a.bricks_z - bz_first);
  const int64_t n_bricks = (int64_t)a.wbricks_x * a.wbricks_y * bz_count;
  const int lane = threadIdx.x & 63;
  const int64_t local = (int64_t)blockIdx.x * 256 + threadIdx.x;
  const bool exists = local < n_bricks;
  const int bx = (int)(local % a.wbricks_x);
  const int64_t t = local / a.wbricks_x;
  const int by = (int)(t % a.wbricks_y), bz = (int)(t / a.wbricks_y) + bz_first;
  const int64_t row = (((int64_t)bz * a.wbricks_y + by) * a.wbricks_x + bx) * a.class_pitch;
  const bool eligible = exists && bz * tk + tk <= a.nz;
  (void)lane;
  double wxa, wya, wza;
  {
    const double gx = a.ox + (bx * 8 + 0.5) * a.sx;
    const double gy = a.oy + (by * 8 + 0.5) * a.sy;
    const double gz = a.oz + ((bz * tk + a.kz0) + 0.5) * a.sz;
    wxa = row4(a.g + 0, gx, gy, gz), wya = row4(a.g + 4, gx, gy, gz), wza = row4(a.g + 8, gx, gy, gz);
  }
  const int m_begin = a.first_map, m_end = a.first_map + a.n_maps;
  const int g_lo = (m_begin & ~3) + blockIdx.y * group_views;
  rows[threadIdx.x] = row;
  uint32_t held[kOriginViews / 4];
#pragma unroll
  for (int g = 0; g < kOriginViews / 4; ++g) {
    const int m4 = g_lo + 4 * g;
    held[g] = (eligible && 4 * g < group_views && m4 < m_end) ? *reinterpret_cast<const uint32_t *>(classes + row + m4) : 0u;
#pragma unroll
    for (int q = 0; q < 4; ++q) tile[4 * g + q][threadIdx.x].origin = kNotWanted;
  }
#pragma unroll
  for (int g = 0; g < kOriginViews / 4; ++g) {
    const int m4 = g_lo + 4 * g;
    if (4 * g >= group_views || m4 >= m_end) break;
    const uint32_t c4 = held[g];
#pragma unroll 1
    for (int q = 0; q < 4; ++q) {
      const int m = m4 + q;
      const uint8_t c = (uint8_t)(c4 >> (8 * q));
      const bool want = eligible && m >= m_begin && m < m_end && (c & 0x1f) == (uint8_t)(BRICK_MIXED | (MIXED_FREE_OR_NODEPTH << 2));
      if (__builtin_amdgcn_ballot_w64(want) == 0) continue;
      WinPair wp;
      wp.origin = kNotWanted;
      wp.ax = wp.ay = wp.acz = 0.f;
      if (cload(&a.win_recs[m].e_abs) < __builtin_inff()) {
        const MapRec *src = maps + m;
        const TileMapRec *tsrc = a.tile_maps + m;
        const FootRec *fr = a.foot_recs + m;
        const float(*scp)[4] = tk == 16 ? fr->s16 : fr->s8;
        if (want) {
          const double cza = ((cload(&src->rt[8]) * wxa + cload(&src->rt[9]) * wya) + cload(&src->rt[10]) * wza) + cload(&src->rt[11]);
          const double hxa = __builtin_fma(cload(&tsrc->cpx), wxa, __builtin_fma(cload(&tsrc->cpy), wya, __builtin_fma(cload(&tsrc->cpz), wza, cload(&tsrc->cp0))));
          const double hya = __builtin_fma(cload(&tsrc->cqx), wxa, __builtin_fma(cload(&tsrc->cqy), wya, __builtin_fma(cload(&tsrc->cqz), wza, cload(&tsrc->cq0))));
          const float hx0 = (float)hxa, hy0 = (float)hya, z0 = (float)cza;
          float umin = __builtin_inff(), umax = -__builtin_inff(), vmin = __builtin_inff(), vmax = -__builtin_inff();
          float zmin = __builtin_inff(), zmax = -__builtin_inff();
#pragma unroll
          for (int cnr = 0; cnr < 8; ++cnr) {
            const float z = z0 + cload(&scp[cnr][2]);
            const float r = __builtin_amdgcn_rcpf(z);
            const float u = (hx0 + cload(&scp[cnr][0])) * r, v = (hy0 + cload(&scp[cnr][1])) * r;
            umin = __builtin_fminf(umin, u), umax = __builtin_fmaxf(umax, u);
            vmin = __builtin_fminf(vmin, v), vmax = __builtin_fmaxf(vmax, v);
            zmin = __builtin_fminf(zmin, z), zmax = __builtin_fmaxf(zmax, z);
          }
          const float umag = __builtin_fmaxf(__builtin_fmaxf(__builtin_fabsf(umin), __builtin_fabsf(umax)), __builtin_fmaxf(__builtin_fabsf(vmin), __builtin_fabsf(vmax)));
          const float e = 2.0f * cload(&fr->ferr) * __builtin_amdgcn_rcpf(zmin) * (1.0f + 0x1p-20f) + (0x1p-19f * umag + 0x1p-12f);
          const bool sane = zmin > 0.0f && zmax <= (float)(kWinCzRatio * (1.0 - 0x1p-20)) * zmin && umin > -65536.0f && umax < 65536.0f &&
                            vmin > -65536.0f && vmax < 65536.0f && e < 0.25f;
          if (sane) {
            const int cxc = a.W / 2, cyc = a.H / 2;
            const int x0 = (int)__builtin_ceilf(umin - 0.5f - e) + cxc, x1 = (int)__builtin_floorf(umax + 0.5f + e) + cxc;
            const int y0 = (int)__builtin_ceilf(vmin - 0.5f - e) + cyc, y1 = (int)__builtin_floorf(vmax + 0.5f + e) + cyc;
            if (x0 >= -kValidMargin && y0 >= -kValidMargin && x1 < a.W + kValidMargin && y1 < a.H + kValidMargin &&
                x1 - x0 < kWindowCols && y1 - y0 < kWindowRows) {
              wp.origin = (uint32_t)(x0 + kValidMargin) | ((uint32_t)(y0 + kValidMargin) << 16);
              wp.ax = (float)(hxa - (double)(x0 + kWinAnchorX - cxc) * cza);
              wp.ay = (float)(hya - (double)(y0 + kWinAnchorY - cyc) * cza);
              wp.acz = z0;
            }
          }
        }
      }
      if (want) {
        if (wp.origin != kNotWanted)
          tile[4 * g + q][threadIdx.x] = wp;
        else
          classes[row + m] = (uint8_t)(c | CLASS_NO_WINDOW);
      }
    }
  }
  __syncthreads();
  const int v = threadIdx.x & (kOriginViews - 1);
  const int m = g_lo + v;
  if (v < group_views && m < m_end) {
#pragma unroll
    for (int it = 0; it < 8; ++it) {
      const int b = (threadIdx.x >> 3) + 32 * it;
      const WinPair wp = tile[v][b];
      if (wp.origin != kNotWanted) origins[rows[b] + m] = wp;
    }
  }
}


__device__ __forceinline__ bool slot_to_brick(const TileArgs &a, int slot, int &bx, int &by, int &bz) {
  const int within = slot & 31;
  const int code = a.sb_perm[(slot - a.slot_base) >> 5];
  const int sbx = code & 1023, sby = (code >> 10) & 1023, sbz = (code >> 20) + a.sbz_first;
  bx = sbx * 4 + (within & 3);
  by = sby * 4 + ((within >> 2) & 3);
  bz = sbz * 2 + (within >> 4);
  return bx < a.bricks_x && by < a.bricks_y && bz < a.bricks_z;
}

constexpr int kWorkLevels = 4;

__global__ __launch_bounds__(256) void brick_work_kernel(const TileArgs a, int wx, int wy, int n_slots,
                                                         uint8_t *__restrict__ level) {
  const int lane = threadIdx.x & 63;
  const int slot = blockIdx.x * 4 + (threadIdx.x >> 6);
  if (slot >= n_slots) return;
  int bx, by, bz;
  if (!slot_to_brick(a, slot + a.slot_base, bx, by, bz)) {
    if (lane == 0) level[slot] = 255;
    return;
  }
  int mixed = 0, total = 0;
  for (int v = 0; v < wy; ++v)
    for (int u = 0; u < wx; ++u) {
      const int wbx = bx * wx + u, wby = by * wy + v;
      if (wbx >= a.wbricks_x || wby >= a.wbricks_y) continue;
      const uint8_t *row = a.classes + (((int64_t)bz * a.wbricks_y + wby) * a.wbricks_x + wbx) * (int64_t)a.class_pitch;
      for (int m = a.first_map + lane; m < a.first_map + a.n_maps; m += 64) mixed += (row[m] & 3) == BRICK_MIXED ? 1 : 0;
      total += a.n_maps;
    }
  for (int off = 32; off > 0; off >>= 1) mixed += __shfl_xor(mixed, off, 64);
  if (lane == 0) level[slot] = mixed * 2 >= total ? 0 : (mixed * 4 >= total ? 1 : (mixed * 16 >= total ? 2 : 3));
}

constexpr int kOrderChunk = 1024;

__global__ __launch_bounds__(kOrderChunk) void order_count_kernel(const uint8_t *__restrict__ level, int n_slots,
                                                                  int *__restrict__ counts) {
  const int s = blockIdx.x * kOrderChunk + threadIdx.x;
  const int l = s < n_slots ? level[s] : 255;
  for (int q = 0; q < kWorkLevels; ++q) {
    const int c = __syncthreads_count(l == q);
    if (threadIdx.x == 0) counts[blockIdx.x * kWorkLevels + q] = c;
  }
}

__global__ __launch_bounds__(1024) void order_base_kernel(int *__restrict__ counts, int n_chunks, int *__restrict__ n_valid) {
  __shared__ int wave_totals[16];
  __shared__ int carry;
  if (threadIdx.x == 0) carry = 0;
  __syncthreads();
  const int lane = threadIdx.x & 63, wave = threadIdx.x >> 6;
  for (int q = 0; q < kWorkLevels; ++q)
    for (int c0 = 0; c0 < n_chunks; c0 += 1024) {
      const int c = c0 + threadIdx.x;
      const int v = c < n_chunks ? counts[c * kWorkLevels + q] : 0;
      int incl = v;
      for (int off = 1; off < 64; off <<= 1) {
        const int up = __shfl_up(incl, off, 64);
        if (lane >= off) incl += up;
      }
      if (lane == 63) wave_totals[wave] = incl;
      __syncthreads();
      int before = carry, all = 0;
      for (int w = 0; w < 16; ++w) {
        if (w < wave) before += wave_totals[w];
        all += wave_totals[w];
      }
      if (c < n_chunks) counts[c * kWorkLevels + q] = before + incl - v;
      __syncthreads();
      if (threadIdx.x == 0) carry += all;
      __syncthreads();
    }
  if (threadIdx.x == 0) *n_valid = carry;
}

__global__ __launch_bounds__(kOrderChunk) void order_scatter_kernel(const TileArgs a, const uint8_t *__restrict__ level,
                                                                    int n_slots, const int *__restrict__ bases,
                                                                    int *__restrict__ order) {
  __shared__ unsigned long long wave_totals[16];
  const int s = blockIdx.x * kOrderChunk + threadIdx.x;
  const int l = s < n_slots ? level[s] : 255;
  const unsigned long long one = l < kWorkLevels ? 1ull << (16 * l) : 0ull;
  const int lane = threadIdx.x & 63, wave = threadIdx.x >> 6;
  unsigned long long incl = one;
  for (int off = 1; off < 64; off <<= 1) {
    const unsigned long long up = __shfl_up(incl, off, 64);
    if (lane >= off) incl += up;
  }
  if (lane == 63) wave_totals[wave] = incl;
  __syncthreads();
  unsigned long long before = 0;
  for (int w = 0; w < wave; ++w) before += wave_totals[w];
  if (l < kWorkLevels) {
    const int rank = (int)(((before + incl - one) >> (16 * l)) & 0xffffull);
    int bx = 0, by = 0, bz = 0;
    slot_to_brick(a, s + a.slot_base, bx, by, bz);
    order[bases[blockIdx.x * kWorkLevels + l] + rank] = pack_brick(bx, by, bz);
  }
}

constexpr int kOrderOneLaunchSlots = 1 << 18;
__global__ __launch_bounds__(kOrderChunk) void order_rank_kernel(const TileArgs a, const uint8_t *__restrict__ level, int n_slots,
                                                                 int *__restrict__ level_starts, int *__restrict__ order,
                                                                 int *__restrict__ n_valid) {
  __shared__ int partial[16][2 * kWorkLevels];
  __shared__ unsigned long long wave_totals[16];
  const int lane = threadIdx.x & 63, wave = threadIdx.x >> 6;
  int cnt[2 * kWorkLevels];
#pragma unroll
  for (int q = 0; q < 2 * kWorkLevels; ++q) cnt[q] = 0;
  const int pieces = n_slots >> 4;
  const int my_first = blockIdx.x * (kOrderChunk / 16);
  for (int p = threadIdx.x; p < pieces; p += kOrderChunk) {
    const uint4 w = reinterpret_cast<const uint4 *>(level)[p];
    const uint32_t words[4] = {w.x, w.y, w.z, w.w};
    int n[kWorkLevels] = {0, 0, 0, 0};
#pragma unroll
    for (int q = 0; q < 4; ++q) {
      const uint32_t c = words[q];
      const uint32_t ok = (~c >> 7) & 0x01010101u;
      const uint32_t b0 = c & ok, b1 = (c >> 1) & ok;
      const int n3 = __builtin_popcount(b0 & b1), n2 = __builtin_popcount(b1 & ~b0), n1 = __builtin_popcount(b0 & ~b1);
      n[3] += n3, n[2] += n2, n[1] += n1, n[0] += __builtin_popcount(ok) - n1 - n2 - n3;
    }
    const bool before = p < my_first;
#pragma unroll
    for (int l = 0; l < kWorkLevels; ++l) {
      cnt[kWorkLevels + l] += n[l];
      cnt[l] += before ? n[l] : 0;
    }
  }
#pragma unroll
  for (int q = 0; q < 2 * kWorkLevels; ++q) {
    int v = cnt[q];
    for (int off = 32; off > 0; off >>= 1) v += __shfl_xor(v, off, 64);
    if (lane == 0) partial[wave][q] = v;
  }
  const int s = blockIdx.x * kOrderChunk + threadIdx.x;
  const int l = s < n_slots ? level[s] : 255;
  const unsigned long long one = l < kWorkLevels ? 1ull << (16 * l) : 0ull;
  unsigned long long incl = one;
  for (int off = 1; off < 64; off <<= 1) {
    const unsigned long long up = __shfl_up(incl, off, 64);
    if (lane >= off) incl += up;
  }
  if (lane == 63) wave_totals[wave] = incl;
  __syncthreads();
  int tot[2 * kWorkLevels];
#pragma unroll
  for (int q = 0; q < 2 * kWorkLevels; ++q) {
    tot[q] = 0;
    for (int w = 0; w < 16; ++w) tot[q] += partial[w][q];
  }
  if (blockIdx.x == 0 && threadIdx.x == 0) {
    level_starts[0] = 0;
    level_starts[1] = tot[4];
    level_starts[2] = tot[4] + tot[5];
    level_starts[3] = tot[4] + tot[5] + tot[6];
    *n_valid = tot[4] + tot[5] + tot[6] + tot[7];
  }
  unsigned long long before = 0;
  for (int w = 0; w < wave; ++w) before += wave_totals[w];
  if (l < kWorkLevels) {
    const int rank = (int)(((before + incl - one) >> (16 * l)) & 0xffffull);
    int base = 0;
#pragma unroll
    for (int q = 0; q < kWorkLevels; ++q) base += q < l ? tot[kWorkLevels + q] : (q == l ? tot[q] : 0);
    int bx = 0, by = 0, bz = 0;
    slot_to_brick(a, s + a.slot_base, bx, by, bz);
    order[base + rank] = pack_brick(bx, by, bz);
  }
}

__global__ __launch_bounds__(256) void brick_work_kernel_1x1(const TileArgs a, int n_slots, uint8_t *__restrict__ level) {
  const int lane = threadIdx.x & 63;
  const int slot = (blockIdx.x * 4 + (threadIdx.x >> 6)) * 4 + (lane >> 4);
  const int part = lane & 15;
  int bx = 0, by = 0, bz = 0;
  const bool exists = slot < n_slots;
  const bool in_grid = exists && slot_to_brick(a, slot + a.slot_base, bx, by, bz);
  int mixed = 0, light = 0;
  constexpr uint32_t kLight = (uint32_t)BRICK_MIXED | ((uint32_t)MIXED_FREE_OR_NODEPTH << 2);
  static_assert(BRICK_MIXED == 0, "a mixed pair's low two bits are 00");
  if (in_grid) {
    const uint8_t *row = a.classes + (((int64_t)bz * a.wbricks_y + by) * a.wbricks_x + bx) * (int64_t)a.class_pitch + a.first_map;
    for (int v0 = part * 16; v0 < a.n_maps; v0 += 256) {
      if (((a.first_map | a.class_pitch) & 15) == 0 && v0 + 16 <= a.n_maps) {
        const uint4 w = *reinterpret_cast<const uint4 *>(row + v0);
        const uint32_t words[4] = {w.x, w.y, w.z, w.w};
#pragma unroll
        for (int q = 0; q < 4; ++q) {
          const uint32_t c = words[q];
          const uint32_t nz = (c | (c >> 1)) & 0x01010101u;
          mixed += 4 - __builtin_popcount(nz);
          const uint32_t y = (c & 0x3f3f3f3fu) ^ (kLight * 0x01010101u);
          light += 4 - __builtin_popcount((y + 0x7f7f7f7fu) & 0x80808080u);
        }
      } else {
        for (int v = v0; v < min(v0 + 16, a.n_maps); ++v) {
          mixed += (row[v] & 3) == BRICK_MIXED ? 1 : 0;
          light += (row[v] & 0x3f) == kLight ? 1 : 0;
        }
      }
    }
  }
  for (int off = 8; off > 0; off >>= 1) {
    mixed += __shfl_xor(mixed, off, 64);
    light += __shfl_xor(light, off, 64);
  }
  if (a.flags & TILE_FLAG_COST_ORDER) {
    const int lv = !in_grid ? 255 : (mixed == 0 ? kCostLevels - 1 : (kCostLevels - 1) - (mixed * (kCostLevels - 1) + a.n_maps - 1) / a.n_maps);
    if (exists && part == 0) level[slot] = (uint8_t)lv;
    unsigned long long todo = __builtin_amdgcn_ballot_w64(exists && part == 0 && lv < kCostLevels);
    while (todo) {
      const int l0 = __shfl(lv, __builtin_ctzll(todo), 64);
      const unsigned long long same = __builtin_amdgcn_ballot_w64(lv == l0) & todo;
      if (lane == __builtin_ctzll(todo)) atomicAdd(const_cast<int32_t *>(a.order_levels) + l0, __builtin_popcountll(same));
      todo &= ~same;
    }
    return;
  }
  if (exists && part == 0)
    {
      const int cost2 = a.win_origin ? 2 * light + 5 * (mixed - light) : 2 * mixed;
      level[slot] = !in_grid ? 255 : (cost2 >= a.n_maps ? 0 : (cost2 * 2 >= a.n_maps ? 1 : (cost2 * 8 >= a.n_maps ? 2 : 3)));
    }
}

__global__ __launch_bounds__(kOrderChunk) void order_cost_kernel(const TileArgs a, const uint8_t *__restrict__ level, int n_slots,
                                                                 int *__restrict__ order, int *__restrict__ n_valid) {
  __shared__ int base[kCostLevels];
  int32_t *sizes = const_cast<int32_t *>(a.order_levels), *cursors = sizes + kCostLevels;
  const int lane = threadIdx.x & 63;
  if (threadIdx.x < 64) {
    const int v = sizes[lane];
    int incl = v;
    for (int off = 1; off < 64; off <<= 1) {
      const int up = __shfl_up(incl, off, 64);
      if (lane >= off) incl += up;
    }
    base[lane] = incl - v;
    if (blockIdx.x == 0 && lane == 63) *n_valid = incl;
  }
  __syncthreads();
  const int s = blockIdx.x * kOrderChunk + threadIdx.x;
  const int lv = s < n_slots ? level[s] : 255;
  int pos = -1;
  unsigned long long todo = __builtin_amdgcn_ballot_w64(lv < kCostLevels);
  while (todo) {
    const int leader = __builtin_ctzll(todo);
    const int l0 = __shfl(lv, leader, 64);
    const unsigned long long same = __builtin_amdgcn_ballot_w64(lv == l0) & todo;
    int first = 0;
    if (lane == leader) first = atomicAdd(cursors + l0, __builtin_popcountll(same));
    first = __shfl(first, leader, 64);
    if (lv == l0) pos = base[l0] + first + __builtin_popcountll(same & ((1ull << lane) - 1ull));
    todo &= ~same;
  }
  if (pos >= 0) {
    int bx = 0, by = 0, bz = 0;
    slot_to_brick(a, s + a.slot_base, bx, by, bz);
    order[pos] = pack_brick(bx, by, bz);
  }
}

inline unsigned blocks_of(int64_t n) { return (unsigned)((n + 255) / 256); }

}

PyramidDesc make_pyramid_desc(int W, int H) {
  PyramidDesc P;
  std::memset(&P, 0, sizeof(P));
  int off = 0;
  for (int li = 0; li < kPyramidMaxLevels; ++li) {
    const int L = kPyramidMinLevel + li, S = 1 << L;
    P.width[li] = (W + S - 1) / S;
    P.height[li] = (H + S - 1) / S;
    P.offset[li] = off;
    off += P.width[li] * P.height[li];
    P.n_levels = li + 1;
    if (P.width[li] == 1 && P.height[li] == 1) break;
  }
  P.total_tiles = off;
  return P;
}

hipError_t launch_upload_views(const void *in, int in_is_f64, const double *best_cost, double threshold, void *out, int out_is_f64,
                               int64_t n_maps, int W, int H, const PyramidDesc &P, DepthTile *pyramids, uint8_t *valid, uint32_t *bits,
                               unsigned long long *counters, hipStream_t stream) {
  if (n_maps <= 0) return hipSuccess;
  if (n_maps > 65535) return hipErrorInvalidConfiguration;
  const int cover_x = std::max(W + 2 * kValidMargin, valid_bits_tiles_x(W) * 32);
  const int cover_y = std::max(((H + 2 * kValidMargin + 7) / 8) * 8, valid_bits_tiles_y(H) * 32);
  const dim3 grid((unsigned)((cover_x + 511) / 512), (unsigned)((cover_y + 7) / 8), (unsigned)n_maps);
#define DMI_UPLOAD(IN, OUT)                                                                                                      \
  hipLaunchKernelGGL((upload_views_kernel<IN, OUT>), grid, dim3(512), 0, stream, static_cast<const IN *>(in), best_cost, threshold, \
                     static_cast<OUT *>(out), W, H, P, pyramids, valid, bits, counters)
  if (in_is_f64) {
    if (out_is_f64)
      DMI_UPLOAD(double, double);
    else
      DMI_UPLOAD(double, float);
  } else {
    if (out_is_f64)
      DMI_UPLOAD(float, double);
    else
      DMI_UPLOAD(float, float);
  }
#undef DMI_UPLOAD
  return hipGetLastError();
}

hipError_t launch_build_pyramid_levels(int64_t n_maps, const PyramidDesc &P, DepthTile *pyramids, hipStream_t stream) {
  if (n_maps <= 0 || P.n_levels <= 1) return hipSuccess;
  hipLaunchKernelGGL(pyramid_levels_kernel, dim3((unsigned)n_maps), dim3(1024), 0, stream, P, pyramids);
  return hipGetLastError();
}

hipError_t launch_window_origins(const TileArgs &a, const MapRec *maps_dev, int tk, uint8_t *classes, int general_k,
                                 hipStream_t stream) {
  if (general_k || !a.win_origin || a.n_maps <= 0) return hipSuccess;
  const int bz_count = std::min(2 * a.super_z, a.bricks_z - 2 * a.sbz_first);
  const int64_t n_bricks = (int64_t)a.wbricks_x * a.wbricks_y * bz_count;
  if (n_bricks <= 0) return hipSuccess;
  const int64_t brick_groups = (n_bricks + 255) / 256;
  const int span = a.first_map + a.n_maps - (a.first_map & ~3);
  int group_views = kOriginViews;
  while (group_views > 4 && brick_groups * ((span + group_views - 1) / group_views) < 2048) group_views >>= 1;
  const dim3 grid((unsigned)brick_groups, (unsigned)((span + group_views - 1) / group_views));
  if (a.rotated)
    hipLaunchKernelGGL((window_origin_kernel<true>), grid, dim3(256), 0, stream, a, maps_dev, tk, classes, a.win_origin, group_views);
  else
    hipLaunchKernelGGL((window_origin_kernel<false>), grid, dim3(256), 0, stream, a, maps_dev, tk, classes, a.win_origin, group_views);
  return hipGetLastError();
}

hipError_t launch_classify_bricks(const TileArgs &a, const MapRec *maps_dev, const PyramidDesc &P, int tk, uint8_t *classes,
                                  uint8_t *coarse, int general_k, hipStream_t stream) {
  const int bz_count = std::min(2 * a.super_z, a.bricks_z - 2 * a.sbz_first);
  const int64_t n_bricks = (int64_t)a.wbricks_x * a.wbricks_y * bz_count;
  if (n_bricks <= 0 || a.n_maps <= 0) return hipSuccess;
  if (n_bricks > (int64_t)0x7fffffff || (a.n_maps + 3) / 4 > 65535) return hipErrorInvalidConfiguration;
  const int per_z = 32 / tk;
  const int64_t n_boxes = (int64_t)((a.wbricks_x + 3) / 4) * ((a.wbricks_y + 3) / 4) * ((bz_count + per_z - 1) / per_z);
  const dim3 coarse_grid((unsigned)((n_boxes + 3) / 4), (unsigned)((a.n_maps + 63) / 64));
#define DMI_LAUNCH_COARSE(R, G) \
  hipLaunchKernelGGL((classify_coarse_kernel<R, G>), coarse_grid, dim3(64, 4), 0, stream, a, maps_dev, P, tk, classes, coarse)
  if (a.rotated && general_k)
    DMI_LAUNCH_COARSE(true, true);
  else if (a.rotated)
    DMI_LAUNCH_COARSE(true, false);
  else if (general_k)
    DMI_LAUNCH_COARSE(false, true);
  else
    DMI_LAUNCH_COARSE(false, false);
#undef DMI_LAUNCH_COARSE
  hipError_t e = hipGetLastError();
  if (e != hipSuccess) return e;
  int group_views = 64;
  while (group_views > 8 && n_boxes * ((a.n_maps + group_views - 1) / group_views) < 2048) group_views >>= 1;
  const dim3 fine_grid((unsigned)n_boxes, (unsigned)((a.n_maps + group_views - 1) / group_views));
  [[maybe_unused]] int q = 5;
#ifdef DMI_TUNING
  if (const char *env = getenv("DMI_QUERY_TILES")) q = atoi(env);
#endif
  const bool wide = tk == 8;
#define DMI_LAUNCH_FINE_G(Q, C, R, G) \
  hipLaunchKernelGGL((classify_kernel<Q, C, R, G>), fine_grid, dim3(256), 0, stream, a, maps_dev, P, tk, classes, coarse, group_views)
#define DMI_LAUNCH_FINE_R(Q, C, R)      \
  do {                                  \
    if (general_k)                      \
      DMI_LAUNCH_FINE_G(Q, C, R, true); \
    else                                \
      DMI_LAUNCH_FINE_G(Q, C, R, false);\
  } while (0)
#define DMI_LAUNCH_FINE(Q)                      \
  do {                                          \
    if (wide && a.rotated)                      \
      DMI_LAUNCH_FINE_R(Q, 64, true);           \
    else if (wide)                              \
      DMI_LAUNCH_FINE_R(Q, 64, false);          \
    else if (a.rotated)                         \
      DMI_LAUNCH_FINE_R(Q, 32, true);           \
    else                                        \
      DMI_LAUNCH_FINE_R(Q, 32, false);          \
  } while (0)
#ifdef DMI_TUNING
  if (q <= 2)
    DMI_LAUNCH_FINE(2);
  else if (q == 3)
    DMI_LAUNCH_FINE(3);
  else
#endif
    DMI_LAUNCH_FINE(5);
#undef DMI_LAUNCH_FINE_G
#undef DMI_LAUNCH_FINE_R
#undef DMI_LAUNCH_FINE
  return hipGetLastError();
}

int64_t coarse_class_bytes(const TileArgs &a, int tk) {
  const int per_z = 32 / tk;
  return (int64_t)((a.wbricks_x + 3) / 4) * ((a.wbricks_y + 3) / 4) * ((a.bricks_z + per_z - 1) / per_z) * (int64_t)a.class_pitch;
}

hipError_t launch_order_bricks(const TileArgs &a, int wx, int wy, uint8_t *level, int *order, int *n_valid,
                               hipStream_t stream) {
  const int n_slots = a.super_x * a.super_y * a.super_z * 32;
  if (wx == 1 && wy == 1)
    hipLaunchKernelGGL(brick_work_kernel_1x1, dim3((unsigned)((n_slots + 15) / 16)), dim3(256), 0, stream, a, n_slots, level);
  else
    hipLaunchKernelGGL(brick_work_kernel, dim3((unsigned)((n_slots + 3) / 4)), dim3(256), 0, stream, a, wx, wy, n_slots, level);
  hipError_t e = hipGetLastError();
  if (e != hipSuccess) return e;
  int *counts = reinterpret_cast<int *>(level + ((size_t)n_slots + 15) / 16 * 16);
  const int n_chunks = (n_slots + kOrderChunk - 1) / kOrderChunk;
  if ((a.flags & TILE_FLAG_COST_ORDER) && wx == 1 && wy == 1) {
    hipLaunchKernelGGL(order_cost_kernel, dim3((unsigned)n_chunks), dim3(kOrderChunk), 0, stream, a, level, n_slots, order, n_valid);
    return hipGetLastError();
  }
  if (n_slots <= kOrderOneLaunchSlots) {
    hipLaunchKernelGGL(order_rank_kernel, dim3((unsigned)n_chunks), dim3(kOrderChunk), 0, stream, a, level, n_slots, counts, order, n_valid);
    return hipGetLastError();
  }
  hipLaunchKernelGGL(order_count_kernel, dim3((unsigned)n_chunks), dim3(kOrderChunk), 0, stream, level, n_slots, counts);
  hipLaunchKernelGGL(order_base_kernel, dim3(1), dim3(1024), 0, stream, counts, n_chunks, n_valid);
  hipLaunchKernelGGL(order_scatter_kernel, dim3((unsigned)n_chunks), dim3(kOrderChunk), 0, stream, a, level, n_slots, counts, order);
  return hipGetLastError();
}

size_t order_scratch_bytes(size_t n_slots) {
  return (n_slots + 15) / 16 * 16 + std::max<size_t>(((n_slots + kOrderChunk - 1) / kOrderChunk) * kWorkLevels, 2 * kCostLevels) * sizeof(int) + 64;
}

}
```

### cudadepthmapintegration_amd/csrc/fusion_kernels.h

```cpp
#pragma once

#include <hip/hip_runtime.h>
#include <stddef.h>
#include <stdint.h>
#include <string.h>

#include "fusion_launch_rules.h"

struct dmi_context;

namespace dmi {

int grid_pointer_for_sums(::dmi_context *ctx, void **ptr);

struct alignas(16) DepthTile {
  float dmin, dmax;
  uint32_t flags;
  uint32_t pad;
};
enum TileFlags : uint32_t { TILE_HAS_SENTINEL = 1, TILE_HAS_VALID = 2, TILE_HAS_NAN = 4, TILE_PART_HOLE_FREE = 8, TILE_PART_NO_VALID = 16 };
constexpr uint8_t COARSE_CHILDREN_WRITTEN = 0x80;

constexpr int kPyramidMinLevel = 3;
constexpr int kPyramidMaxLevels = 13;

struct PyramidDesc {
  int32_t n_levels;
  int32_t total_tiles;
  int32_t width[kPyramidMaxLevels];
  int32_t height[kPyramidMaxLevels];
  int32_t offset[kPyramidMaxLevels];
};

struct alignas(16) MapRec {
  double rt[12];
  double k[12];
  const void *depth;
  const DepthTile *pyramid;
};
static_assert(sizeof(MapRec) == 208, "MapRec layout");

struct alignas(16) TileMapRec {
  double rz0, rz1, rz3;
  double px, py, pz, p0;
  double qx, qy, qz, q0;
  double dhx, dhy;
  double err;
  const void *depth;
  double cz_err;
  double errk;
  double sx, sy, sz, s0, dhz, errz;
  double cpx, cpy, cpz, cp0, cqx, cqy, cqz, cq0;
  double cdhx, cdhy, cerrk;
  float t1_dhx, t1_dhy, t1_dcz, t1_dthr;
  float t1_e1, t1_c1;
  float t1_erel, t1_hspan;
  int32_t t1_cidx;
  int32_t t1_ok;
  const uint8_t *valid;
  float vm_c0, vm_w8;
  int32_t vm_base, vm_bytes;
  const uint32_t *vbits;
  int32_t vb_bytes;
  int32_t vb_rowskip;
  int32_t vb_mx, vb_my;
  float t1_b;
  int32_t vb_pad;
};
#ifndef DMI_TIER1
#define DMI_TIER1 1
#endif
constexpr int kValidMargin = 32;
constexpr unsigned kValidByte = 10;
__host__ __device__ inline int64_t valid_map_bytes(int W, int H) {
  return (int64_t)((H + 2 * kValidMargin + 7) / 8) * (W + 2 * kValidMargin) * 8;
}
__host__ __device__ inline int valid_bits_tiles_x(int W) { return (W + 2 * kValidMargin + 31) / 32 + 1; }
__host__ __device__ inline int valid_bits_tiles_y(int H) { return (H + 2 * kValidMargin + 31) / 32; }
__host__ __device__ inline int64_t valid_bits_bytes(int W, int H) { return (int64_t)valid_bits_tiles_x(W) * valid_bits_tiles_y(H) * 128; }
constexpr int kWindowCols = 32, kWindowRows = 64;
constexpr uint8_t CLASS_NO_WINDOW = 0x20;
static_assert(sizeof(TileMapRec) == 368, "TileMapRec layout");

struct alignas(64) WinRec {
  const uint32_t *vbits;
  float di[2], dj[2], dk[2];
  float ci[2], cj[2], ck[2];
  float e_abs;
  float c1;
};
static_assert(sizeof(WinRec) == 64, "WinRec is one cache line");
struct alignas(64) FootRec {
  float s8[8][4];
  float s16[8][4];
  float ferr, pad[15];
};
static_assert(sizeof(FootRec) == 320, "FootRec layout");
#ifdef DMI_WIN_CORNER_ANCHOR
constexpr int kWinAnchorX = 0, kWinAnchorY = 0;
constexpr float kWinC1 = 0.5f - 0x1p-14f;
#else
constexpr int kWinAnchorX = kWindowCols / 2, kWinAnchorY = kWindowRows / 2;
constexpr float kWinC1 = 0.5f - 0x1p-15f;
#endif
constexpr int kWinReach = kWinAnchorY ? kWindowRows - kWinAnchorY : kWindowRows - 1;
constexpr double kWinCzRatio = 1.25;
struct alignas(16) WinPair {
  uint32_t origin;
  float ax, ay, acz;
};
static_assert(sizeof(WinPair) == 16, "WinPair layout");

enum KMode : int {
  K_GENERAL = 0,
  K_PINHOLE_SKEW = 1,
  K_PINHOLE = 2
};

struct FuseArgs {
  int32_t nx, ny, nz;
  int32_t W, H;
  int32_t first_map, n_maps;
  int32_t init_from_grid;
  int32_t kz0, pad1;
  int32_t k_first, k_count;
  double ox, oy, oz;
  double sx, sy, sz;
  double g[12];
  double thick, delta;
  double rho_pos, rho_neg, rho_zero;
  double slope;
  double free_space;
  const MapRec *maps;
  void *grid;
  uint32_t *voxel_hits;
  unsigned long long *map_hits;
};

struct TileArgs {
  int32_t nx, ny, nz, W, H, first_map, n_maps, init_from_grid;
  int32_t kpad;
  int32_t bricks_x, bricks_y, bricks_z;
  int32_t super_x, super_y, super_z;
  int32_t sbz_first, pad3;
  int32_t slot_base, slot_count;
  int32_t depth_bytes;
  int32_t kz0, pad1;
  double ox, oy, oz, sx, sy, sz;
  double g[12];
  double thick, delta, rho_pos, rho_neg, slope, free_space;
  const TileMapRec *tile_maps;
  const double *cz_table;
  void *grid;
  uint32_t *voxel_hits;
  unsigned long long *map_hits;
  const FuseArgs *full;
  const uint8_t *classes;
  int32_t class_pitch;
  int32_t wbricks_x, wbricks_y;
  int32_t xcd_run_wg;
  const int32_t *order;
  const int32_t *n_order;
  unsigned long long behind_mask;
  int32_t rotated;
  int32_t flags;
  const MapRec *maps;
  const int32_t *order_levels;
  const double *free_sums;
  const int32_t *sb_perm;
  unsigned long long *wg_times;
  int64_t wg_times_n;
  int32_t *queue_heads;
  WinPair *win_origin;
  int64_t win_delta;
  const WinRec *win_recs;
  const FootRec *foot_recs;
  int32_t vb_bytes, vb_rowskip;
  int32_t win_cx, win_cy;
};
constexpr int kFreeSumsMax = 4096;
__host__ __device__ inline int32_t pack_brick(int bx, int by, int bz) { return (int32_t)((uint32_t)bx | ((uint32_t)by << 11) | ((uint32_t)bz << 22)); }
static_assert(offsetof(TileArgs, nx) == 0 && offsetof(TileArgs, nz) == 8 && offsetof(TileArgs, kpad) == 32 &&
                  offsetof(TileArgs, bricks_x) == 36 && offsetof(TileArgs, bricks_z) == 44 && offsetof(TileArgs, sbz_first) == 60,
              "TileArgs head layout");
enum TileKernelFlags : int32_t {
  TILE_FLAG_NO_INTERIOR = 1,
  TILE_FLAG_XCD_RUNS = 2,
  TILE_FLAG_COST_ORDER = 4,
  TILE_FLAG_DBG_SKIP_WINDOW_PAIRS = 256,
  TILE_FLAG_DBG_ONLY_WINDOW_PAIRS = 512,
  TILE_FLAG_DBG_NO_WINDOW_LOADS = 1024
};

enum BrickClass : uint8_t {
  BRICK_MIXED = 0,
  BRICK_FREE = 1,
  BRICK_BEHIND = 2,
  BRICK_SKIP = 3
};

enum MixedReason : uint8_t {
  MIXED_UNSPECIFIED = 0,
  MIXED_DEGENERATE = 1,
  MIXED_CAMERA_PLANE = 2,
  MIXED_IMAGE_BORDER = 3,
  MIXED_NAN_DEPTH = 4,
  MIXED_SENTINEL_AND_DEPTH = 5,
  MIXED_NEAR_SURFACE = 6,
  MIXED_FREE_OR_NODEPTH = 7
};

struct FuseConfig {
  int depth_is_f64;
  int grid_is_f64;
  int k_mode;
  int count_hits;
  int variant;
  int use_tile;
  int general_k;
  int holes;
};


constexpr int kMaxColumnHeight = 16;
struct TileShape {
  int tk, wx, wy;
};
TileShape tile_shape(int variant, bool depth_is_f64, bool rotated, bool general_k);

hipError_t launch_fuse(const FuseArgs &args, const FuseConfig &cfg, hipStream_t stream);

hipError_t launch_fuse_tiled(const TileArgs &args, const MapRec *maps_dev, const FuseConfig &cfg, const PyramidDesc &pyramid,
                             uint8_t *order_scratch, uint8_t *coarse_classes, hipEvent_t before_main_kernel,
                             hipStream_t stream);

hipError_t launch_widen_depth(const float *in, double *out, int64_t n, hipStream_t stream);
hipError_t launch_convert_grid(const void *in, int in_is_f64, void *out, int64_t n, hipStream_t stream);

hipError_t launch_fp64_probe(double *out, int blocks, int iters, hipStream_t stream);

PyramidDesc make_pyramid_desc(int W, int H);
hipError_t launch_upload_views(const void *in, int in_is_f64, const double *best_cost, double threshold, void *out, int out_is_f64,
                               int64_t n_maps, int W, int H, const PyramidDesc &desc, DepthTile *pyramids, uint8_t *valid, uint32_t *bits,
                               unsigned long long *counters, hipStream_t stream);
hipError_t launch_build_pyramid_levels(int64_t n_maps, const PyramidDesc &desc, DepthTile *pyramids, hipStream_t stream);
hipError_t launch_window_origins(const TileArgs &args, const MapRec *maps_dev, int tk, uint8_t *classes, int general_k,
                                 hipStream_t stream);
hipError_t launch_classify_bricks(const TileArgs &args, const MapRec *maps_dev, const PyramidDesc &desc, int tk,
                                  uint8_t *classes, uint8_t *coarse, int general_k, hipStream_t stream);
int64_t coarse_class_bytes(const TileArgs &args, int tk);
size_t order_scratch_bytes(size_t n_slots);
hipError_t launch_order_bricks(const TileArgs &args, int wx, int wy, uint8_t *level, int *order, int *n_valid,
                               hipStream_t stream);

hipError_t launch_cell_to_point(const void *cells, int cells_are_f64, double *points, int nx, int ny, int nz,
                                hipStream_t stream);

size_t iso_block_count(int nx, int ny, int nz);
hipError_t launch_iso_count(const double *points, int nx, int ny, int nz, double iso, uint32_t *counts, uint64_t *bases,
                            void *scan_temp, size_t *scan_temp_bytes, hipStream_t stream);
hipError_t launch_iso_write(const double *points, int nx, int ny, int nz, double iso, const uint64_t *bases, int64_t *ids,
                            uint64_t capacity, hipStream_t stream);

struct MeshGeom {
  int nx, ny, nz, segs_per_row;
  double iso;
  double origin[3], spacing[3];
  double m[12];
  uint64_t n_vertices, n_triangles;
};
struct MeshNormals {
  double nm[9];
  float *normals;
};
int isosurface_max_triangles_per_cell();
size_t isosurface_segment_count(int nx, int ny, int nz);
hipError_t launch_isosurface_count(const double *points, const MeshGeom &g, uint32_t *counts, uint64_t *bases, void *scan_temp,
                                   size_t *scan_temp_bytes, hipStream_t stream);
hipError_t launch_isosurface_write(const double *points, const MeshGeom &g, const uint64_t *bases, double *verts, int64_t *tris,
                                   const MeshNormals *normals, hipStream_t stream);

struct ComponentsMesh {
  uint64_t n_vertices, n_triangles;
  const double *vertices;
  const float *normals;
  const int64_t *triangles;
  double *out_vertices;
  float *out_normals;
  int64_t *out_triangles;
  int64_t *region_id;
  int64_t *region_size;
};
struct ComponentsScratch {
  uint32_t *parent, *size;
  uint32_t *vmap, *rmap;
  uint32_t *tmap;
  unsigned long long *counters;
  void *scan_temp;
  size_t scan_temp_bytes;
};
hipError_t components_scan_temp_bytes(uint64_t n_vertices, uint64_t n_triangles, size_t *bytes);
hipError_t launch_isosurface_components(const ComponentsMesh &m, const ComponentsScratch &s, int largest, uint64_t min_triangles,
                                        hipEvent_t *events, hipStream_t stream);

struct SmoothMesh {
  uint64_t n_vertices, n_triangles;
  const double *vertices;
  const int64_t *triangles;
  float *normals_out;
};
struct SmoothScratch {
  uint64_t *keys[2];
  uint32_t *row_start;
  uint32_t *valence, *offsets;
  unsigned long long *fixed;
  double *positions[2];
  void *temp;
  size_t temp_bytes;
};
hipError_t smooth_temp_bytes(uint64_t n_vertices, uint64_t n_triangles, size_t *bytes);
hipError_t launch_isosurface_smooth(const SmoothMesh &m, const SmoothScratch &s, int iterations, double lambda, double mu,
                                    double **result, hipEvent_t *events, hipStream_t stream);
hipError_t launch_isosurface_geometric_normals(const double *vertices, const int64_t *triangles, uint64_t n_vertices, uint64_t n_triangles,
                                               uint64_t *const keys[2], uint32_t *row_start, void *temp, size_t temp_bytes,
                                               float *normals_out, hipStream_t stream);

struct DecimateMesh {
  uint64_t n_vertices, n_triangles;
  const double *vertices;
  const int64_t *triangles;
  double *out_vertices;
  int64_t *out_triangles;
};
struct DecimateGrid {
  double lo[3], h;
  uint64_t n[3];
};
struct DecimateScratch {
  unsigned long long *bounds;
  uint64_t *keys[2];
  uint32_t *ids[2];
  uint32_t *head, *rank;
  uint32_t *cluster_of, *start;
  uint32_t *mark, *cmap;
  uint32_t *keep, *tmap;
  void *temp;
  size_t temp_bytes;
};
constexpr int kDecimateMean = 0, kDecimateQuadric = 1;
hipError_t decimate_temp_bytes(uint64_t n_vertices, uint64_t n_triangles, int placement, size_t *bytes);
hipError_t launch_decimate_bounds(const DecimateMesh &m, const DecimateScratch &s, hipEvent_t *events, hipStream_t stream);
double decimate_decode_bound(unsigned long long ordered);
hipError_t launch_isosurface_decimate(const DecimateMesh &m, const DecimateGrid &g, const DecimateScratch &s, int placement,
                                      hipEvent_t *events, hipStream_t stream);

struct SupportMesh {
  uint64_t n_vertices, n_triangles;
  const double *vertices;
  const float *normals;
  const int64_t *triangles;
  double *out_vertices;
  float *out_normals;
  int64_t *out_triangles;
};
struct SupportViews {
  const MapRec *maps;
  int n_views, W, H;
  int depth_is_f64;
};
struct SupportScratch {
  int32_t *support;
  int32_t *out_support;
  uint32_t *mark, *vmap;
  uint32_t *tmap;
  void *scan_temp;
  size_t scan_temp_bytes;
};
hipError_t support_scan_temp_bytes(uint64_t n_vertices, uint64_t n_triangles, size_t *bytes);
hipError_t launch_isosurface_support_counts(const SupportMesh &m, const SupportViews &views, double tolerance, int require_facing,
                                            const SupportScratch &s, hipEvent_t *events, hipStream_t stream);
hipError_t launch_isosurface_support_filter(const SupportMesh &m, int32_t min_views, const SupportScratch &s, hipEvent_t *events,
                                            hipStream_t stream);

}
```

### cudadepthmapintegration_amd/csrc/fusion_tile.hip

```cpp
#include <stdlib.h>

#include <algorithm>
#include <type_traits>

#include "fusion_kernels.h"
#include "fusion_device.h"

#ifndef DMI_T1_CHAINS
#define DMI_T1_CHAINS 4
#endif
#ifndef DMI_T1_COLUMN_CHAINS
#define DMI_T1_COLUMN_CHAINS 2
#endif
#if !defined(DMI_TUNING) && (defined(DMI_EXP_SKIP_WINDOW_VIEWS) || defined(DMI_EXP_SAME_REC) || defined(DMI_EXP_NO_WINDOW_LOADS) || \
                             defined(DMI_EXP_NO_LANE_MARGIN))
#error "a DMI_EXP_* switch that changes results was defined without DMI_TUNING"
#endif

namespace dmi {

int tile_shape_index(int variant);

namespace {

// ... 249 lines not shown
  const int lane = threadIdx.x & 63;
  const int w = __builtin_amdgcn_readfirstlane(threadIdx.x >> 6);

  constexpr bool PERSIST = STAY && WX * WY == 1;
  const int b = blockIdx.x;
  int q = b >> 3;
  int helped = 0;
#define DMI_NEXT_BRICK \
  {                    \
    if (PERSIST)       \
      continue;        \
    else               \
      return;          \
  }
  for (;;) {
  const kernarg_t kb = KFRESH();
  typedef int i32x8 __attribute__((ext_vector_type(8)));
  const i32x8 head0 = *reinterpret_cast<const i32x8 __attribute__((address_space(4))) *>(kb);
  const i32x8 head1 = *(reinterpret_cast<const i32x8 __attribute__((address_space(4))) *>(kb) + 1);
  const int32_t *const p_order = kb->order, *const p_levels = kb->order_levels, *const p_n_order = kb->n_order;
  const int kflags = kb->flags;
  const int xq = (b + helped) & 7;
  if constexpr (PERSIST) {
    if (helped == 8) break;
    int taken = 0;
    if (lane == 0) taken = atomicAdd(kb->queue_heads + 16 * xq, 1);
    q = __builtin_amdgcn_readfirstlane(taken);
  }
  int entry = -1;
  int p = -1;
  bool used_up = false;
  if (p_order && !(kflags & TILE_FLAG_XCD_RUNS)) {
    int rest = q, found = -1;
    typedef int i32x4 __attribute__((ext_vector_type(4)));
    const i32x4 bounds = cload(reinterpret_cast<const i32x4 *>(p_levels));
    const int last = cload(p_n_order);
    int lo = bounds[0];
#pragma unroll
    for (int level = 0; level < 4; ++level) {
      const int hi = level < 3 ? bounds[level + 1] : last;
      const int n = hi - lo;
      const int s0 = (int)(((long long)xq * n) >> 3), s1 = (int)(((long long)(xq + 1) * n) >> 3);
      if (found < 0) {
        if (rest < s1 - s0)
          found = lo + s0 + rest;
        else
          rest -= s1 - s0;
      }
      lo = hi;
    }
    if (found < 0)
      used_up = true;
    else
      entry = cload(p_order + found);
    p = found;
  } else {
    const int run = kb->xcd_run_wg;
    p = (q / run) * (8 * run) + xq * run + q % run;
    if (p_order) {
      if (p >= cload(p_n_order))
        used_up = true;
      else
        entry = cload(p_order + p);
    } else if (p >= kb->slot_count) {
      used_up = true;
    }
  }
  if (used_up) {
    if constexpr (PERSIST) {
      ++helped;
      continue;
    } else {
      return;
    }
  }
  int bx, by, bz;
  if (p_order) {
    bx = entry & 2047, by = (entry >> 11) & 2047, bz = (int)((unsigned)entry >> 22);
  } else {
    const int within = p & 31;
    const int code = cload(kb->sb_perm + (p >> 5));
    const int sbx = code & 1023, sby = (code >> 10) & 1023, sbz = (code >> 20) + head1[7];
    bx = sbx * 4 + (within & 3), by = sby * 4 + ((within >> 2) & 3), bz = sbz * 2 + (within >> 4);
  }
  if ((bx >= head1[1]) | (by >= head1[2]) | (bz >= head1[3])) DMI_NEXT_BRICK

#ifdef DMI_TUNING
  unsigned long long wg_t0 = 0;
  if (kb->wg_times) wg_t0 = __builtin_amdgcn_s_memrealtime();
  unsigned dbg_cols = 0, dbg_redo = 0;
  unsigned dbg_win = 0, dbg_win_early = 0;
  unsigned dbg_win_redo = 0;
#endif
  const int wbx = bx * WX + (w % WX), wby = by * WY + (w / WX);
  if ((wbx >= kb->wbricks_x) | (wby >= kb->wbricks_y)) DMI_NEXT_BRICK
  const int i = wbx * kLX + (lane % kLX);
  const int j = wby * kLY + (lane / kLX);
  const int k0 = bz * TK;
  const int kcount = head0[2] - k0 < TK ? head0[2] - k0 : TK;
  const bool lane_ok = (i < head0[0]) & (j < head0[1]);

  const kernarg_t kg = kb;
  const double gx = kg->ox + (i + 0.5) * kg->sx;
  const double gy = kg->oy + (j + 0.5) * kg->sy;
  const double gz0 = kg->oz + ((k0 + kg->kz0) + 0.5) * kg->sz;
  double gm[12];
#pragma unroll
  for (int q = 0; q < 12; ++q) gm[q] = kg->g[q];
  const double wx = ROT ? gm[0] * gx + gm[1] * gy : row4(gm + 0, gx, gy, gz0);
  const double wy = ROT ? gm[4] * gx + gm[5] * gy : row4(gm + 4, gx, gy, gz0);
  const double wz0 = ROT ? gm[8] * gx + gm[9] * gy : row4(gm + 8, gx, gy, gz0);


  uint32_t nh[COUNT ? TK : 1];
#ifndef DMI_EXP_INIT_ALWAYS_OLD
  if constexpr (!PERSIST) {
    if (kg->init_from_grid) {
      GridT held[TK];
      const int ic = i < head0[0] ? i : head0[0] - 1, jc = j < head0[1] ? j : head0[1] - 1;
      const GridT *column = static_cast<const GridT *>(kg->grid) + ((int64_t)k0 * kg->ny + jc) * kg->nx + ic;
      const int64_t plane_in = (int64_t)kg->ny * kg->nx;
#pragma unroll
      for (int kk = 0; kk < TK; ++kk) held[kk] = column[(int64_t)(kk < kcount ? kk : kcount - 1) * plane_in];
#pragma unroll
      for (int kk = 0; kk < TK; ++kk) acc_set<BASE, TK>(kk, (double)held[kk]);
    } else {
#pragma unroll
      for (int kk = 0; kk < TK; ++kk) acc_set<BASE, TK>(kk, 0.0);
    }
  } else
#endif
  {
#pragma unroll
    for (int kk = 0; kk < TK; ++kk) {
      double v0 = 0.0;
      if (kg->init_from_grid && lane_ok && kk < kcount)
        v0 = (double)static_cast<const GridT *>(kg->grid)[(((int64_t)(k0 + kk)) * kg->ny + j) * kg->nx + i];
      acc_set<BASE, TK>(kk, v0);
    }
  }
  if (COUNT) {
#pragma unroll
    for (int kk = 0; kk < TK; ++kk) nh[kk] = 0;
  }

  const mask_t m_lane_ok_brick = ballot(lane_ok);

  const unsigned long long *crow = reinterpret_cast<const unsigned long long *>(
      KA(classes) + (((int64_t)bz * KA(wbricks_y) + wby) * KA(wbricks_x) + wbx) * (int64_t)KA(class_pitch));

  int n_uniform = (!COUNT && KA(free_sums) != nullptr) ? 0 : -1;
  unsigned long long cnext = cload(crow + (first_map >> 3));
  [[maybe_unused]] uint32_t pair_a = 0, pair_b = 0;
  for (int wbase = first_map & ~7; wbase < m_end; wbase += 8) {
    if constexpr (WIN) {
      if ((wbase & 24) == 0 || wbase == (first_map & ~7)) {
        const kernarg_t ko = KFRESH();
        if (ko->win_origin) {
          typedef uint32_t u32x2 __attribute__((ext_vector_type(2)));
          const u32x2 *row = reinterpret_cast<const u32x2 *>(ko->win_delta + 16 * (int64_t)reinterpret_cast<intptr_t>(crow));
          const u32x2 pr = row[2 * (wbase & ~31) + lane];
          pair_a = pr.x;
          pair_b = pr.y;
        }
      }
    }
    const unsigned long long cword = cnext | ((cnext >> 1) & (ZF ? 0x0101010101010101ull : KC(behind_mask)));
    if (wbase + 8 < m_end) cnext = cload(crow + (wbase >> 3) + 1);
    const unsigned long long nonskip = cword ^ 0x0303030303030303ull;
    unsigned long long todo = (nonskip | (nonskip >> 1)) & 0x0101010101010101ull;
    if (wbase < first_map) todo &= ~0ull << ((first_map - wbase) * 8);
    if (wbase + 8 > m_end) todo &= (1ull << ((m_end - wbase) * 8)) - 1;
    unsigned long long fr = COUNT ? 0ull : (todo & cword & ~(cword >> 1));
    unsigned long long other = todo ^ fr;
  for (;;) {
    const unsigned long long below = (other - 1) & ~other;
    const int n_free_now = __builtin_popcountll(fr & below);
    fr &= ~below;
    if (n_uniform >= 0) {
      n_uniform += n_free_now;
    } else {
      for (int n_free = n_free_now; n_free > 0; --n_free) {
#pragma unroll
        for (int q = 0; q < TK; q += 8) acc_add8_all<BASE, TK>(q, free_space);
      }
    }
    if (other == 0) break;
    const int vbit = __builtin_ctzll(other);
    other &= other - 1;
    const int m = wbase + (vbit >> 3);
    if (n_uniform >= 0) {
      const double v = cload(KC(free_sums) + n_uniform);
#pragma unroll
      for (int q = 0; q < TK; ++q) acc_set<BASE, TK>(q, v);
      n_uniform = -1;
    }
    const unsigned cbyte = (unsigned)(cword >> vbit) & 0x3fu;
    const unsigned cls = cbyte & 3u;
    if (cls != BRICK_MIXED) {
      const double v = cls == BRICK_FREE ? free_space : 0.0;
#pragma unroll
      for (int q = 0; q < TK; q += 8) acc_add8_all<BASE, TK>(q, v);
      if (COUNT) {
#pragma unroll
        for (int q = 0; q < TK; ++q) nh[q] += lane_ok ? 1u : 0u;
        const uint32_t hits = (uint32_t)__popcll(m_lane_ok_brick) * (uint32_t)kcount;
        if (hits != 0 && lane == 0) atomicAdd(&KC(map_hits)[m], (unsigned long long)hits);
      }
      continue;
    }
    [[maybe_unused]] const bool has_window = WIN && cbyte == ((unsigned)MIXED_FREE_OR_NODEPTH << 2 | BRICK_MIXED) && kcount == TK;
#ifdef DMI_TUNING
    ++dbg_cols;
    if ((kflags & TILE_FLAG_DBG_SKIP_WINDOW_PAIRS) && has_window) continue;
    if ((kflags & TILE_FLAG_DBG_ONLY_WINDOW_PAIRS) && !has_window) continue;
#endif
    if constexpr (WIN) {
      if (has_window) {
#ifdef DMI_TUNING
        ++dbg_win;
        if (dbg_cols == dbg_win) ++dbg_win_early;
#endif
        const int pl = (m & 31) * 2;
        const uint32_t org = (uint32_t)__builtin_amdgcn_readlane((int)pair_a, pl);
        const unsigned long long A2 = (unsigned long long)(uint32_t)__builtin_amdgcn_readlane((int)pair_b, pl) |
                                      ((unsigned long long)(uint32_t)__builtin_amdgcn_readlane((int)pair_a, pl + 1) << 32);
        const float acz = __int_as_float(__builtin_amdgcn_readlane((int)pair_b, pl + 1));
        const int x0p = (int)(org & 0xffffu), y0p = (int)(org >> 16);
        const kernarg_t kw = KFRESH();
        typedef uint32_t u32x16 __attribute__((ext_vector_type(16)));
        const WinRec *const wrec = kw->win_recs + m;
        const u32x16 R = *reinterpret_cast<const u32x16 __attribute__((address_space(4))) *>(reinterpret_cast<uintptr_t>(wrec));
#ifndef DMI_NO_WINREC_PREFETCH
        int next_rec;
        asm volatile("s_load_dword %0, %1, 0x40" : "=&s"(next_rec) : "s"(wrec), "s"(R[15]));
#endif
        const __amdgpu_buffer_rsrc_t brsrc = __builtin_amdgcn_make_buffer_rsrc(
            reinterpret_cast<uint32_t *>((uintptr_t)R[0] | ((uintptr_t)R[1] << 32)), (short)0, kw->vb_bytes, 0x00020000);
        const unsigned lin = ((unsigned)lane << 2) + ((unsigned)y0p << 2);
        const unsigned off = __umul24(lin >> 7, (unsigned)kw->vb_rowskip) + lin + (((unsigned)x0p >> 5) << 7);
#ifdef DMI_TUNING
        uint32_t w_lo, w_hi;
        if (kflags & TILE_FLAG_DBG_NO_WINDOW_LOADS) {
          w_lo = off * 0x9e3779b9u, w_hi = ~w_lo;
        } else {
          w_lo = (uint32_t)__builtin_amdgcn_raw_buffer_load_b32(brsrc, (int)off, 0, 0);
          w_hi = (uint32_t)__builtin_amdgcn_raw_buffer_load_b32(brsrc, (int)(off + 128u), 0, 0);
        }
#else
        const uint32_t w_lo = (uint32_t)__builtin_amdgcn_raw_buffer_load_b32(brsrc, (int)off, 0, 0);
        const uint32_t w_hi = (uint32_t)__builtin_amdgcn_raw_buffer_load_b32(brsrc, (int)(off + 128u), 0, 0);
#endif
        const int x0c = x0p - kw->win_cx, y0c = y0p - kw->win_cy;
        f32x2 O, LJ;
        O.x = (float)(x0c + kWinAnchorX);
        O.y = (float)(y0c + kWinAnchorY);
        LJ.x = (float)(lane & 7);
        LJ.y = (float)(lane >> 3);
        auto pair_of = [&](int q) __attribute__((always_inline)) { return (unsigned long long)R[q] | ((unsigned long long)R[q + 1] << 32); };
        auto vec_of = [&](int q) __attribute__((always_inline)) {
          f32x2 v;
          v.x = __uint_as_float(R[q]);
          v.y = __uint_as_float(R[q + 1]);
          asm volatile("" : "+v"(v));
          return v;
        };
        const f32x2 Bwi = pk_fnma_slo(O, pair_of(8), vec_of(2));
        const f32x2 Bwj = pk_fnma_slo(O, pair_of(10), vec_of(4));
        const f32x2 DH = pk_fnma_slo(O, pair_of(12), vec_of(6));
        const f32x2 H0 = pk_fma_hi0_vv(LJ, Bwj, pk_fma_lo0_vs(LJ, Bwi, A2));
        f32x2 CA;
        CA.x = acz;
        CA.y = __builtin_fmaf(acz, __uint_as_float(R[15]), -__uint_as_float(R[14]));
        const f32x2 C0 = pk_fma_hi0_sv(LJ, pair_of(10), pk_fma_lo0_sv(LJ, pair_of(8), CA));
        const f32x2 DC = vec_of(12);
        unsigned long long M2 = (0x4B400000ull + (unsigned)kWinAnchorX) | ((0x4B400000ull + (unsigned)kWinAnchorY) << 32);
        asm volatile("" : "+s"(M2));
        float magic_v = 0x1.8p23f + (float)(4 * kWinAnchorY);
        asm volatile("" : "+v"(magic_v));
        auto first_voxel = [&](double &hxf, double &hyf, double &czf64) __attribute__((always_inline)) {
          const kernarg_t kf = KFRESH();
          const TileMapRec *rf = kf->tile_maps + m;
          double wxf = wx, wyf = wy, wzf = wz0;
          if constexpr (ROT) {
            const czvec4 b = cload(reinterpret_cast<const czvec4 *>(kf->cz_table + (int64_t)k0 * 4));
            wxf = (wx + b[0]) + kf->g[3], wyf = (wy + b[1]) + kf->g[7], wzf = (wz0 + b[2]) + kf->g[11];
            czf64 = ((cload(&rf->rz0) * wxf + cload(&rf->rz1) * wyf) + cload(&kf->maps[m].rt[10]) * wzf) + cload(&rf->rz3);
          } else {
            czf64 = ((cload(&rf->rz0) * wx + cload(&rf->rz1) * wy) + cload(kf->cz_table + (int64_t)m * kf->kpad + k0)) + cload(&rf->rz3);
          }
          hxf = __builtin_fma(cload(&rf->cpx), wxf, __builtin_fma(cload(&rf->cpy), wyf, __builtin_fma(cload(&rf->cpz), wzf, cload(&rf->cp0))));
          hyf = __builtin_fma(cload(&rf->cqx), wxf, __builtin_fma(cload(&rf->cqy), wyf, __builtin_fma(cload(&rf->cqz), wzf, cload(&rf->cq0))));
        };
        uint32_t undecided = 0, und_kk = 0;
        uint32_t window = 0;
        constexpr int WG = 4;
#ifdef DMI_T1_RCP_EVERY_VOXEL
        constexpr bool kNewton = false;
#else
        constexpr bool kNewton = true;
#endif
        [[maybe_unused]] f32x2 r_below;
        uint32_t pw[WG], pc[WG];
        auto consume = [&](int g0) __attribute__((always_inline)) {
          __builtin_amdgcn_s_waitcnt(0xc07f);
          if ((und_kk >> g0) & ((1u << WG) - 1u)) {
  #pragma unroll
            for (int q = 0; q < WG; ++q) pw[q] &= ((undecided >> (g0 + q)) & 1u) - 1u;
          }
  #pragma unroll
          for (int q = 0; q < WG; ++q) {
            int mbit;
            asm("v_bfe_i32 %0, %1, %2, 1" : "=v"(mbit) : "v"(pw[q]), "v"(pc[q]));
            acc_fma_vs<BASE, TK>(g0 + q, __hiloint2double(mbit & 0x3ff00000, 0), free_space);
          }
        };
  #pragma unroll
        for (int g0 = 0; g0 < TK; g0 += WG) {
          uint32_t wg[WG], cg[WG];
          mask_t m_und[WG];
          constexpr int IL = DMI_T1_CHAINS;
          if constexpr (kNewton) {
            static_assert(WG == 4, "the link order below is written for groups of four");
            f32x2 h[WG], cth[WG], r[WG], rpm[WG], rp[WG], t[WG];
            float tw[WG], mx[WG];
            auto kbits = [](int kk) __attribute__((always_inline)) { return (unsigned long long)(unsigned)__float_as_int((float)kk); };
            auto lz = [&](int u) __attribute__((always_inline)) { cth[u] = g0 + u > 0 ? ordered::pk_fma_s(kbits(g0 + u), DC, C0) : C0; };
            auto lh = [&](int u) __attribute__((always_inline)) { h[u] = g0 + u > 0 ? ordered::pk_fma_s(kbits(g0 + u), DH, H0) : H0; };
            auto l2 = [&](int u) __attribute__((always_inline)) {
              if (g0 + u > 0) tw[u] = ordered::two_minus(cth[u].x, u > 0 ? r[u > 0 ? u - 1 : 0].x : r_below.x);
            };
            auto lr = [&](int u) __attribute__((always_inline)) {
              r[u].x = g0 + u > 0 ? ordered::mul(u > 0 ? r[u > 0 ? u - 1 : 0].x : r_below.x, tw[u]) : ordered::rcp(cth[u].x);
            };
            auto lq = [&](int u) __attribute__((always_inline)) { rpm[u] = ordered::pk_fma_lo_s(h[u], r[u], M2); };
            auto lp = [&](int u) __attribute__((always_inline)) { rp[u] = ordered::pk_sub_s(rpm[u], M2); };
            auto lt = [&](int u) __attribute__((always_inline)) { t[u] = ordered::pk_fnma_lo(rp[u], cth[u], h[u]); };
            auto lm = [&](int u) __attribute__((always_inline)) { mx[u] = ordered::max_abs(t[u].x, t[u].y); };
            lz(0), lz(1), lz(2), lz(3);
            l2(0), lh(0), lr(0), lh(1), l2(1), lh(2), lr(1), lq(0), l2(2), lp(0), lr(2), lq(1), l2(3), lt(0), lr(3), lh(3);
            lp(1), lq(2), lm(0), lq(3), lt(1), lp(2), lm(1), lp(3), lt(2), lt(3), lm(2), lm(3);
            r_below = r[WG - 1];
  #pragma unroll
            for (int u = 0; u < WG; ++u) {
              m_und[u] = ballot(!(mx[u] < cth[u].y));
              wg[u] = (unsigned)__float_as_int(__builtin_fmaf(rp[u].y, 4.0f, magic_v));
              cg[u] = (uint32_t)__float_as_int(rpm[u].x);
            }
          } else {
  #pragma unroll
          for (int q0 = 0; q0 < WG; q0 += IL) {
            f32x2 h[IL], cth[IL], rr[IL], rpm[IL], rp[IL], t[IL];
            float mx[IL];
  #pragma unroll
            for (int u = 0; u < IL; ++u) {
              const int kk = g0 + q0 + u;
              const unsigned long long kbits = (unsigned long long)(unsigned)__float_as_int((float)kk);
              cth[u] = kk > 0 ? ordered::pk_fma_s(kbits, DC, C0) : C0;
            }
  #pragma unroll
            for (int u = 0; u < IL; ++u) {
              const int kk = g0 + q0 + u;
              const unsigned long long kbits = (unsigned long long)(unsigned)__float_as_int((float)kk);
              h[u] = kk > 0 ? ordered::pk_fma_s(kbits, DH, H0) : H0;
            }
  #pragma unroll
            for (int u = 0; u < IL; ++u) rr[u].x = ordered::rcp(cth[u].x);
  #pragma unroll
            for (int u = 0; u < IL; ++u) rpm[u] = ordered::pk_fma_lo_s(h[u], rr[u], M2);
  #pragma unroll
            for (int u = 0; u < IL; ++u) rp[u] = ordered::pk_sub_s(rpm[u], M2);
  #pragma unroll
            for (int u = 0; u < IL; ++u) t[u] = ordered::pk_fnma_lo(rp[u], cth[u], h[u]);
  #pragma unroll
            for (int u = 0; u < IL; ++u) mx[u] = ordered::max_abs(t[u].x, t[u].y);
  #pragma unroll
            for (int u = 0; u < IL; ++u) {
// ... 481 lines not shown
        if (exact) {
          hit = eh;
          val = ev;
        }
      }
#pragma unroll
      for (int q = 0; q < TK; ++q) {
        if (kk == q) {
          acc_add_v<BASE, TK>(q, ballot(hit), val);
          if (COUNT) nh[q] += hit ? 1u : 0u;
        }
      }
      if (COUNT) map_hits += (uint32_t)__popcll(ballot(hit));
    }
    if (COUNT) {
      if (map_hits != 0 && lane == 0) atomicAdd(&KC(map_hits)[m], (unsigned long long)map_hits);
    }
  }
  }

#ifdef DMI_TUNING
  if (KC(wg_times) && threadIdx.x == 0) {
    unsigned long long *wt = KC(wg_times);
    unsigned xcc;
    asm volatile("s_getreg_b32 %0, hwreg(HW_REG_XCC_ID)" : "=s"(xcc));
    const size_t uid = (size_t)p, n_uid = (size_t)KC(wg_times_n);
    if (uid < n_uid) {
      wt[2 * uid] = wg_t0;
      wt[2 * uid + 1] = __builtin_amdgcn_s_memrealtime();
      wt[2 * n_uid + uid] = (xcc & 15u) | ((unsigned long long)(blockIdx.x & 0xffffffu) << 8) | ((unsigned long long)(dbg_cols & 0x3ffu) << 32) |
                            ((unsigned long long)(dbg_win & 0x3ffu) << 42) | ((unsigned long long)(dbg_win_early & 0x3ffu) << 52) |
                            ((unsigned long long)(dbg_redo > 3 ? 3 : dbg_redo) << 62);
    }
  }
  if (KC(wg_times) && lane == 0 && (dbg_win | dbg_win_redo)) {
    unsigned long long *wc = KC(wg_times) + 3 * (size_t)KC(wg_times_n);
    atomicAdd(wc, (unsigned long long)dbg_win);
    atomicAdd(wc + 1, (unsigned long long)dbg_win_redo);
  }
#endif
  if (n_uniform > 0) {
    const double v = cload(KC(free_sums) + n_uniform);
#pragma unroll
    for (int q = 0; q < TK; ++q) acc_set<BASE, TK>(q, v);
  }
  if (lane_ok) {
    const kernarg_t ke = KFRESH();
    GridT *__restrict__ grid = static_cast<GridT *>(ke->grid);
    const int64_t plane = (int64_t)ke->ny * ke->nx;
    int64_t gid = ((int64_t)k0 * ke->ny + j) * ke->nx + i;
#pragma unroll
    for (int kk = 0; kk < TK; ++kk) {
      if (kk < kcount) {
        const GridT sum = stored_sum<GridT>(acc_get<BASE, TK>(kk));
        if constexpr (PERSIST)
          __builtin_nontemporal_store(sum, &grid[gid]);
        else
          grid[gid] = sum;
        if (COUNT) ke->voxel_hits[gid] += nh[kk];
      }
      gid += plane;
    }
  }
  if constexpr (!PERSIST) break;
  }
}
#undef DMI_NEXT_BRICK
#undef KA
#undef KC
#undef KFRESH

__global__ __launch_bounds__(256) void launch_tables_kernel(const TileArgs a, const MapRec *__restrict__ maps) {
  fill_launch_tables(a, maps, (int64_t)blockIdx.x * blockDim.x + threadIdx.x, (int64_t)gridDim.x * blockDim.x);
}

constexpr int kPersistentMinViews = 96;

template <typename Kernel>
unsigned resident_workgroups(Kernel kernel, int threads) {
  int device = 0, per_cu = 0;
  hipDeviceProp_t prop;
  if (hipGetDevice(&device) != hipSuccess || hipGetDeviceProperties(&prop, device) != hipSuccess ||
      hipOccupancyMaxActiveBlocksPerMultiprocessor(&per_cu, kernel, threads, 0) != hipSuccess || per_cu <= 0 ||
      prop.multiProcessorCount <= 0) {
    (void)hipGetLastError();
    return 8192u;
  }
  return (unsigned)(per_cu * prop.multiProcessorCount + 7) / 8u * 8u;
}

template <typename DepthT, typename GridT, int TK, int WX, int WY, int MINW, int GROUP, bool ROT = false, bool GENK = false, bool WIN = false>
hipError_t launch_shape(const TileArgs &a, const FuseConfig &cfg, hipStream_t s) {
  static_assert(TK <= kMaxColumnHeight, "dmi_multi_z_slab aligns slabs to kMaxColumnHeight");
  constexpr bool one_wave = WX * WY == 1;
  constexpr bool rare = std::is_same<DepthT, double>::value || GENK;
  static_assert(!WIN || (one_wave && !rare), "window launches are production launches");
  const int per_round = 8 * a.xcd_run_wg;
  unsigned blocks = (unsigned)((a.super_x * a.super_y * a.super_z * 32 + 32 + per_round - 1) / per_round * per_round);
  const dim3 block(64 * WX * WY);
  const bool zf = a.behind_mask != 0 && !cfg.count_hits;
  if (WIN && !zf) return hipErrorInvalidValue;
  bool stay = true;
  if constexpr (one_wave && !rare) {
    const int64_t voxels = (int64_t)a.super_x * a.super_y * a.super_z * 32 * 64 * TK;
    stay = (cfg.variant & VAR_PERSISTENT_ALWAYS) ? true
           : (cfg.variant & VAR_PERSISTENT_NEVER) ? false
           : (cfg.variant & VAR_NO_BRICK_CLASSES) ? true
           : cfg.holes ? (a.n_maps >= 48 && voxels >= (int64_t(1) << 25))
                       : (a.n_maps >= kPersistentMinViews && voxels >= (int64_t(1) << 27));
  }
  auto launch = [&](auto kernel, bool persistent) {
    unsigned n = blocks;
    if (persistent && one_wave) {
      static const unsigned resident = resident_workgroups(kernel, 64);
      n = std::min(n, resident);
    }
    hipLaunchKernelGGL(kernel, dim3(n), block, 0, s, a);
    return hipGetLastError();
  };
  if constexpr (!WIN) {
    if (cfg.count_hits) return launch(fuse_tile_kernel<DepthT, GridT, TK, WX, WY, MINW, GROUP, true, ROT, GENK>, true);
  }
  if constexpr (one_wave && !rare) {
    if (zf) {
      if (!stay) return launch(fuse_tile_kernel<DepthT, GridT, TK, WX, WY, MINW, GROUP, false, ROT, GENK, false, WIN, true>, false);
      return launch(fuse_tile_kernel<DepthT, GridT, TK, WX, WY, MINW, GROUP, false, ROT, GENK, true, WIN, true>, true);
    }
  }
  if constexpr (!WIN) return launch(fuse_tile_kernel<DepthT, GridT, TK, WX, WY, MINW, GROUP, false, ROT, GENK>, true);
  return hipErrorInvalidValue;
}

int effective_shape(int variant, bool depth_is_f64, bool rotated, bool general_k = false) {
  int shape = tile_shape_index(variant);
#ifndef DMI_TUNING
  shape = (shape == 1 || shape == 3 || shape == 4 || shape == 7) ? 7 : 0;
#endif
  if (general_k || depth_is_f64) return 0;
  return (rotated && shape != 7) ? 0 : shape;
}

template <typename DepthT, typename GridT, int TK, int MINW, bool ROT>
hipError_t launch_win(const TileArgs &a, const FuseConfig &cfg, hipStream_t s) {
  if constexpr (DMI_TIER1 != 0 && std::is_same<DepthT, float>::value)
    return launch_shape<DepthT, GridT, TK, 1, 1, MINW, 8, ROT, false, true>(a, cfg, s);
  else
    return hipErrorInvalidValue;
}

template <typename DepthT, typename GridT>
hipError_t launch_types(const TileArgs &a, const FuseConfig &cfg, hipStream_t s) {
  constexpr bool f32_depth = std::is_same<DepthT, float>::value;
  const int shape = effective_shape(cfg.variant, !f32_depth, a.rotated != 0, cfg.general_k != 0);
  const bool win = DMI_TIER1 != 0 && std::is_same<DepthT, float>::value && a.win_origin != nullptr && !cfg.count_hits && !cfg.general_k &&
                   a.behind_mask != 0;
#ifdef DMI_FAST_BUILD
  if (win) {
    if (shape == 7) return launch_win<DepthT, GridT, 8, 6, false>(a, cfg, s);
    return launch_win<DepthT, GridT, 16, 5, false>(a, cfg, s);
  }
  if constexpr (f32_depth) {
    if (shape == 7) return launch_shape<DepthT, GridT, 8, 1, 1, 6, 8>(a, cfg, s);
  }
  return launch_shape<DepthT, GridT, 16, 1, 1, 5, 8>(a, cfg, s);
#else
  if (cfg.general_k) {
    if (a.rotated) return launch_shape<DepthT, GridT, 16, 1, 1, 5, 8, true, true>(a, cfg, s);
    return launch_shape<DepthT, GridT, 16, 1, 1, 5, 8, false, true>(a, cfg, s);
  }
  if (a.rotated) {
    if (win) {
      if (shape == 7) return launch_win<DepthT, GridT, 8, 6, true>(a, cfg, s);
      return launch_win<DepthT, GridT, 16, 5, true>(a, cfg, s);
    }
    if constexpr (f32_depth) {
      if (shape == 7) return launch_shape<DepthT, GridT, 8, 1, 1, 6, 8, true>(a, cfg, s);
    }
    return launch_shape<DepthT, GridT, 16, 1, 1, 5, 8, true>(a, cfg, s);
  }
#ifdef DMI_TUNING
  if constexpr (std::is_same<DepthT, float>::value) {
    switch (shape) {
      case 1: return launch_shape<DepthT, GridT, 8, 2, 2, 6, 8>(a, cfg, s);
      case 2: return launch_shape<DepthT, GridT, 16, 2, 2, 5, 8>(a, cfg, s);
      case 3: return launch_shape<DepthT, GridT, 8, 2, 2, 6, 4>(a, cfg, s);
      case 4: return launch_shape<DepthT, GridT, 8, 2, 2, 7, 8>(a, cfg, s);
      case 5: return launch_shape<DepthT, GridT, 16, 2, 2, 5, 4>(a, cfg, s);
      case 6: return launch_shape<DepthT, GridT, 16, 2, 2, 6, 2>(a, cfg, s);
      default: break;
    }
  }
#endif
  if (win && (shape == 7 || shape == 0)) {
    if (shape == 7) return launch_win<DepthT, GridT, 8, 6, false>(a, cfg, s);
    return launch_win<DepthT, GridT, 16, 5, false>(a, cfg, s);
  }
  if constexpr (f32_depth) {
    if (shape == 7) return launch_shape<DepthT, GridT, 8, 1, 1, 6, 8>(a, cfg, s);
  }
  return launch_shape<DepthT, GridT, 16, 1, 1, 5, 8>(a, cfg, s);
#endif
}

}

int tile_shape_index(int variant) { return (variant & VAR_TILE_SHAPE_MASK) >> VAR_TILE_SHAPE_SHIFT; }

TileShape tile_shape(int variant, bool depth_is_f64, bool rotated, bool general_k) {
  switch (effective_shape(variant, depth_is_f64, rotated, general_k)) {
    case 0: return TileShape{16, 1, 1};
    case 7: return TileShape{8, 1, 1};
    case 1:
    case 3:
    case 4: return TileShape{8, 2, 2};
    default: return TileShape{16, 2, 2};
  }
}

#ifdef DMI_TUNING
__global__ __launch_bounds__(256) void remap_classes_kernel(uint8_t *classes, int64_t n, uint32_t table) {
  for (int64_t i = (int64_t)blockIdx.x * blockDim.x + threadIdx.x; i < n; i += (int64_t)gridDim.x * blockDim.x) {
    const uint8_t b = classes[i];
    classes[i] = (uint8_t)((table >> (8 * (b & 3))) & 0xff);
  }
}
#endif

hipError_t launch_fuse_tiled(const TileArgs &a, const MapRec *maps_dev, const FuseConfig &cfg, const PyramidDesc &pyramid,
                             uint8_t *order_scratch, uint8_t *coarse_classes, hipEvent_t before_main_kernel,
                             hipStream_t stream) {
  if (a.n_maps <= 0) return hipSuccess;
  hipError_t e = hipSuccess;
  if (cfg.variant & VAR_NO_BRICK_CLASSES) {
    const int64_t entries = a.rotated ? a.kpad : (int64_t)a.kpad * a.n_maps;
    hipLaunchKernelGGL(launch_tables_kernel, dim3((unsigned)std::min<int64_t>((entries + 255) / 256, 4096)), dim3(256), 0, stream, a, maps_dev);
    e = hipGetLastError();
    if (e != hipSuccess) return e;
  }
  if (!(cfg.variant & VAR_NO_BRICK_CLASSES)) {
    const TileShape sh = tile_shape(cfg.variant, cfg.depth_is_f64 != 0, a.rotated != 0, cfg.general_k != 0);
    e = launch_classify_bricks(a, maps_dev, pyramid, sh.tk, const_cast<uint8_t *>(a.classes), coarse_classes, cfg.general_k, stream);
    if (e != hipSuccess) return e;
    e = launch_window_origins(a, maps_dev, sh.tk, const_cast<uint8_t *>(a.classes), cfg.general_k, stream);
    if (e != hipSuccess) return e;
#ifdef DMI_TUNING
    if (const char *env = getenv("DMI_DEBUG_CLASS_REMAP")) {
      const int64_t n = (int64_t)a.wbricks_x * a.wbricks_y * a.bricks_z * (int64_t)a.class_pitch;
      hipLaunchKernelGGL(remap_classes_kernel, dim3(4096), dim3(256), 0, stream, const_cast<uint8_t *>(a.classes), n,
                         (uint32_t)strtoul(env, nullptr, 0));
    }
#endif
    if (a.order) {
      e = launch_order_bricks(a, sh.wx, sh.wy, order_scratch, const_cast<int *>(a.order), const_cast<int *>(a.n_order), stream);
      if (e != hipSuccess) return e;
    }
  }
  if (before_main_kernel) {
    e = hipEventRecord(before_main_kernel, stream);
    if (e != hipSuccess) return e;
  }
#ifndef DMI_FAST_BUILD
  if (cfg.depth_is_f64) {
    if (cfg.grid_is_f64) return launch_types<double, double>(a, cfg, stream);
    return launch_types<double, float>(a, cfg, stream);
  }
  if (cfg.grid_is_f64) return launch_types<float, double>(a, cfg, stream);
#endif
  return launch_types<float, float>(a, cfg, stream);
}

}
```

Measured before the change: 3044.

## Compute window origins inside the fused tile kernel instead of a separate pass

Removes the separate window_origin_kernel launch and its WinPair scratch table. Each fused-kernel wavefront now computes per-view window origins on the fly, using pairs of lanes per view (x/y split with DPP swaps), from a new view-blocked WinEntryRecs layout that gathers the required per-view constants into structure-of-arrays blocks of 32 views. This removes a kernel launch and a global write/read round trip of the origin table, at the cost of extra arithmetic and loads inside the main kernel's view loop. Brick ordering now also drops the light count for incomplete z-bricks.

```diff
diff --git a/cudadepthmapintegration_amd/csrc/dmi_capi.hip b/cudadepthmapintegration_amd/csrc/dmi_capi.hip
--- a/cudadepthmapintegration_amd/csrc/dmi_capi.hip
+++ b/cudadepthmapintegration_amd/csrc/dmi_capi.hip
@@ -465,6 +465,28 @@
   make_centred_rows(ctx, r, P, Q, S, Sx, Sy, M, zabs, zscale, general, aligned, &t, win, foot);
   if (zscale_out) *zscale_out = zscale;
   return t;
+}
+
+void set_win_entry(std::vector<dmi::WinEntryRecs> *table, size_t m, const MapRec &r, const TileMapRec &t, const dmi::WinRec &wrec,
+                   const dmi::FootRec &frec) {
+  const size_t block = m / dmi::kEntryViews, v = m % dmi::kEntryViews;
+  if (table->size() <= block) {
+    dmi::WinEntryRecs fresh;
+    std::memset(&fresh, 0, sizeof(fresh));
+    for (int q = 0; q < dmi::kEntryViews; ++q) fresh.e_abs[q] = std::numeric_limits<float>::infinity();
+    table->resize(block + 1, fresh);
+  }
+  dmi::WinEntryRecs &e = (*table)[block];
+  for (int q = 0; q < 4; ++q) e.rt2[q][v] = r.rt[8 + q];
+  const double rows[8] = {t.cpx, t.cpy, t.cpz, t.cp0, t.cqx, t.cqy, t.cqz, t.cq0};
+  for (int q = 0; q < 8; ++q) e.crow[q][v] = rows[q];
+  for (int c = 0; c < 8; ++c)
+    for (int q = 0; q < 3; ++q) {
+      e.s8[c][q][v] = frec.s8[c][q];
+      e.s16[c][q][v] = frec.s16[c][q];
+    }
+  e.ferr[v] = frec.ferr;
+  e.e_abs[v] = wrec.e_abs;
 }
 
 int add_views_impl(dmi_context *ctx, const double *depth64, const float *depth32, const double *best_cost,
@@ -534,6 +556,7 @@
     wrec.vbits = t.vbits;
     ctx->views.h_win_recs.push_back(wrec);
     ctx->views.h_foot_recs.push_back(frec);
+    set_win_entry(&ctx->views.h_win_entries, ctx->views.h_maps.size() - 1, r, t, wrec, frec);
     if (!(t.err <= ctx->views.max_tile_err)) ctx->views.max_tile_err = t.err;
     ctx->views.view_k_mode.push_back((uint8_t)km);
     ctx->views.view_tile_ok.push_back(finite && t.err < 0x1p-12 * zscale && 65536.0 * t.errz < 0x1p-14 && t.cerrk < 0x1p-11 * zscale ? 1 : 0);
@@ -776,6 +799,7 @@
   ctx->views.h_tile_maps.clear();
   ctx->views.h_win_recs.clear();
   ctx->views.h_foot_recs.clear();
+  ctx->views.h_win_entries.clear();
   ctx->views.view_k_mode.clear();
   ctx->views.view_tile_ok.clear();
   ctx->views.max_tile_err = 0.0;
diff --git a/cudadepthmapintegration_amd/csrc/dmi_capi_fuse.hip b/cudadepthmapintegration_amd/csrc/dmi_capi_fuse.hip
--- a/cudadepthmapintegration_amd/csrc/dmi_capi_fuse.hip
+++ b/cudadepthmapintegration_amd/csrc/dmi_capi_fuse.hip
@@ -22,11 +22,12 @@
   dmi_context::Views &v = ctx->views;
   const size_t n = v.h_maps.size();
   const size_t cap = std::max<size_t>(64, n * 2);
+  const size_t nb = v.h_win_entries.size(), cap_b = (cap + dmi::kEntryViews - 1) / dmi::kEntryViews;
   bool fresh = false;
   int rc = dmi::ensure_idle_buffers(ctx, {{&v.maps, n * sizeof(MapRec), cap * sizeof(MapRec)},
                                           {&v.tile_maps, n * sizeof(TileMapRec), cap * sizeof(TileMapRec)},
                                           {&v.win_recs, n * sizeof(dmi::WinRec), cap * sizeof(dmi::WinRec)},
-                                          {&v.foot_recs, n * sizeof(dmi::FootRec), cap * sizeof(dmi::FootRec)}}, &fresh);
+                                          {&v.win_entries, nb * sizeof(dmi::WinEntryRecs), cap_b * sizeof(dmi::WinEntryRecs)}}, &fresh);
   if (rc != DMI_OK) return rc;
   if (fresh) v.maps_dirty = true;
   dmi::DeviceBuffer &hits = ctx->hits.map;
@@ -51,7 +52,7 @@
     DMI_HIP(ctx, hipMemcpyAsync(v.maps.ptr, v.h_maps.data(), n * sizeof(MapRec), hipMemcpyHostToDevice, ctx->stream));
     DMI_HIP(ctx, hipMemcpyAsync(v.tile_maps.ptr, v.h_tile_maps.data(), n * sizeof(TileMapRec), hipMemcpyHostToDevice, ctx->stream));
     DMI_HIP(ctx, hipMemcpyAsync(v.win_recs.ptr, v.h_win_recs.data(), n * sizeof(dmi::WinRec), hipMemcpyHostToDevice, ctx->stream));
-    DMI_HIP(ctx, hipMemcpyAsync(v.foot_recs.ptr, v.h_foot_recs.data(), n * sizeof(dmi::FootRec), hipMemcpyHostToDevice, ctx->stream));
+    DMI_HIP(ctx, hipMemcpyAsync(v.win_entries.ptr, v.h_win_entries.data(), nb * sizeof(dmi::WinEntryRecs), hipMemcpyHostToDevice, ctx->stream));
     v.maps_dirty = false;
   }
   return DMI_OK;
@@ -217,8 +218,7 @@
 
 int class_table(dmi_context *ctx, const dmi::TileShape &sh, bool windows, TileArgs *t) {
   const size_t fine_bytes = ((size_t)t->wbricks_x * t->wbricks_y * t->bricks_z * (size_t)t->class_pitch + 255) / 256 * 256;
-  const size_t coarse_end = (fine_bytes + (size_t)dmi::coarse_class_bytes(*t, sh.tk) + 255) / 256 * 256;
-  const size_t cbytes = coarse_end + (windows ? fine_bytes * sizeof(dmi::WinPair) : 0);
+  const size_t cbytes = (fine_bytes + (size_t)dmi::coarse_class_bytes(*t, sh.tk) + 255) / 256 * 256;
   ctx->tables.coarse_offset = fine_bytes;
   bool fresh = false;
   const int rc = dmi::ensure_idle_buffer(ctx, ctx->tables.classes, cbytes, cbytes, &fresh);
@@ -226,10 +226,9 @@
   if (fresh) DMI_HIP(ctx, hipMemsetAsync(ctx->tables.classes.ptr, dmi::BRICK_SKIP, cbytes, ctx->stream));
   t->classes = ctx->tables.classes.as<uint8_t>();
   if (windows) {
-    t->win_origin = reinterpret_cast<dmi::WinPair *>(ctx->tables.classes.as<uint8_t>() + coarse_end);
-    t->win_delta = (int64_t)reinterpret_cast<intptr_t>(t->win_origin) - 16 * (int64_t)reinterpret_cast<intptr_t>(t->classes);
+    t->windows = 1;
     t->win_recs = ctx->views.win_recs.as<dmi::WinRec>();
-    t->foot_recs = ctx->views.foot_recs.as<dmi::FootRec>();
+    t->win_entries = ctx->views.win_entries.as<dmi::WinEntryRecs>();
     t->vb_bytes = (int32_t)std::min<int64_t>(dmi::valid_bits_bytes(ctx->views.W, ctx->views.H), 0x7fffffff);
     t->vb_rowskip = (dmi::valid_bits_tiles_x(ctx->views.W) - 1) * 128;
     t->win_cx = dmi::kValidMargin + ctx->views.W / 2;
@@ -388,7 +387,7 @@
   last.class_bricks = (int64_t)t.wbricks_x * t.wbricks_y * t.bricks_z;
   last.bricks_z = t.bricks_z;
   last.tk = t.bricks_z > 0 ? t.kpad / t.bricks_z : 0;
-  last.win_origin = t.win_origin;
+  last.windows = t.windows != 0;
   last.class_pitch = t.class_pitch;
   last.first = first;
   last.count = count;
@@ -499,7 +498,7 @@
   if (!ctx || !out) return fail(ctx, DMI_ERR_INVALID_ARGUMENT, "dmi_get_window_pair_count: null argument");
   *out = 0;
   const dmi_context::LastLaunch &last = ctx->last;
-  if (!last.win_origin) return DMI_OK;
+  if (!last.windows) return DMI_OK;
   const int64_t per_layer = last.class_bricks / std::max<int64_t>(1, last.bricks_z);
   return visit_last_classes(ctx, [&](int64_t b, uint8_t c) {
     const int64_t bz = b / std::max<int64_t>(1, per_layer);
diff --git a/cudadepthmapintegration_amd/csrc/dmi_context.h b/cudadepthmapintegration_amd/csrc/dmi_context.h
--- a/cudadepthmapintegration_amd/csrc/dmi_context.h
+++ b/cudadepthmapintegration_amd/csrc/dmi_context.h
@@ -64,7 +64,8 @@
     std::vector<dmi::TileMapRec> h_tile_maps;
     std::vector<dmi::WinRec> h_win_recs;
     std::vector<dmi::FootRec> h_foot_recs;
-    dmi::DeviceBuffer maps, tile_maps, win_recs, foot_recs;
+    std::vector<dmi::WinEntryRecs> h_win_entries;
+    dmi::DeviceBuffer maps, tile_maps, win_recs, win_entries;
     bool maps_dirty = false;
     dmi::DeviceBuffer stage_depth, stage_cost;
     dmi::DeviceBuffer lossy;
@@ -76,7 +77,7 @@
         (void)hipFree(b.d_pyramid);
       }
       batches.clear();
-      dmi::free_buffers({&maps, &tile_maps, &win_recs, &foot_recs, &stage_depth, &stage_cost, &lossy});
+      dmi::free_buffers({&maps, &tile_maps, &win_recs, &win_entries, &stage_depth, &stage_cost, &lossy});
       dmi::destroy_events(up_events);
     }
   } views;
@@ -124,7 +125,7 @@
     bool classes = false;
     int64_t class_bricks = 0;
     int32_t bricks_z = 0, tk = 0;
-    const dmi::WinPair *win_origin = nullptr;
+    bool windows = false;
     int32_t class_pitch = 0, first = 0, count = 0;
   } last;
 
diff --git a/cudadepthmapintegration_amd/csrc/fusion_classify.hip b/cudadepthmapintegration_amd/csrc/fusion_classify.hip
--- a/cudadepthmapintegration_amd/csrc/fusion_classify.hip
+++ b/cudadepthmapintegration_amd/csrc/fusion_classify.hip
@@ -579,118 +579,6 @@
   }
 }
 
-constexpr int kOriginViews = 8;
-constexpr uint32_t kNotWanted = 0xfffffffeu;
-template <bool ROT>
-__global__ __launch_bounds__(256) void window_origin_kernel(const TileArgs a, const MapRec *__restrict__ maps, int tk,
-                                                            uint8_t *__restrict__ classes, WinPair *__restrict__ origins,
-                                                            int group_views) {
-  __shared__ WinPair tile[kOriginViews][256 + 1];
-  __shared__ int64_t rows[256];
-  const int bz_first = 2 * a.sbz_first;
-  const int bz_count = min(2 * a.super_z, a.bricks_z - bz_first);
-  const int64_t n_bricks = (int64_t)a.wbricks_x * a.wbricks_y * bz_count;
-  const int lane = threadIdx.x & 63;
-  const int64_t local = (int64_t)blockIdx.x * 256 + threadIdx.x;
-  const bool exists = local < n_bricks;
-  const int bx = (int)(local % a.wbricks_x);
-  const int64_t t = local / a.wbricks_x;
-  const int by = (int)(t % a.wbricks_y), bz = (int)(t / a.wbricks_y) + bz_first;
-  const int64_t row = (((int64_t)bz * a.wbricks_y + by) * a.wbricks_x + bx) * a.class_pitch;
-  const bool eligible = exists && bz * tk + tk <= a.nz;
-  (void)lane;
-  double wxa, wya, wza;
-  {
-    const double gx = a.ox + (bx * 8 + 0.5) * a.sx;
-    const double gy = a.oy + (by * 8 + 0.5) * a.sy;
-    const double gz = a.oz + ((bz * tk + a.kz0) + 0.5) * a.sz;
-    wxa = row4(a.g + 0, gx, gy, gz), wya = row4(a.g + 4, gx, gy, gz), wza = row4(a.g + 8, gx, gy, gz);
-  }
-  const int m_begin = a.first_map, m_end = a.first_map + a.n_maps;
-  const int g_lo = (m_begin & ~3) + blockIdx.y * group_views;
-  rows[threadIdx.x] = row;
-  uint32_t held[kOriginViews / 4];
-#pragma unroll
-  for (int g = 0; g < kOriginViews / 4; ++g) {
-    const int m4 = g_lo + 4 * g;
-    held[g] = (eligible && 4 * g < group_views && m4 < m_end) ? *reinterpret_cast<const uint32_t *>(classes + row + m4) : 0u;
-#pragma unroll
-    for (int q = 0; q < 4; ++q) tile[4 * g + q][threadIdx.x].origin = kNotWanted;
-  }
-#pragma unroll
-  for (int g = 0; g < kOriginViews / 4; ++g) {
-    const int m4 = g_lo + 4 * g;
-    if (4 * g >= group_views || m4 >= m_end) break;
-    const uint32_t c4 = held[g];
-#pragma unroll 1
-    for (int q = 0; q < 4; ++q) {
-      const int m = m4 + q;
-      const uint8_t c = (uint8_t)(c4 >> (8 * q));
-      const bool want = eligible && m >= m_begin && m < m_end && (c & 0x1f) == (uint8_t)(BRICK_MIXED | (MIXED_FREE_OR_NODEPTH << 2));
-      if (__builtin_amdgcn_ballot_w64(want) == 0) continue;
-      WinPair wp;
-      wp.origin = kNotWanted;
-      wp.ax = wp.ay = wp.acz = 0.f;
-      if (cload(&a.win_recs[m].e_abs) < __builtin_inff()) {
-        const MapRec *src = maps + m;
-        const TileMapRec *tsrc = a.tile_maps + m;
-        const FootRec *fr = a.foot_recs + m;
-        const float(*scp)[4] = tk == 16 ? fr->s16 : fr->s8;
-        if (want) {
-          const double cza = ((cload(&src->rt[8]) * wxa + cload(&src->rt[9]) * wya) + cload(&src->rt[10]) * wza) + cload(&src->rt[11]);
-          const double hxa = __builtin_fma(cload(&tsrc->cpx), wxa, __builtin_fma(cload(&tsrc->cpy), wya, __builtin_fma(cload(&tsrc->cpz), wza, cload(&tsrc->cp0))));
-          const double hya = __builtin_fma(cload(&tsrc->cqx), wxa, __builtin_fma(cload(&tsrc->cqy), wya, __builtin_fma(cload(&tsrc->cqz), wza, cload(&tsrc->cq0))));
-          const float hx0 = (float)hxa, hy0 = (float)hya, z0 = (float)cza;
-          float umin = __builtin_inff(), umax = -__builtin_inff(), vmin = __builtin_inff(), vmax = -__builtin_inff();
-          float zmin = __builtin_inff(), zmax = -__builtin_inff();
-#pragma unroll
-          for (int cnr = 0; cnr < 8; ++cnr) {
-            const float z = z0 + cload(&scp[cnr][2]);
-            const float r = __builtin_amdgcn_rcpf(z);
-            const float u = (hx0 + cload(&scp[cnr][0])) * r, v = (hy0 + cload(&scp[cnr][1])) * r;
-            umin = __builtin_fminf(umin, u), umax = __builtin_fmaxf(umax, u);
-            vmin = __builtin_fminf(vmin, v), vmax = __builtin_fmaxf(vmax, v);
-            zmin = __builtin_fminf(zmin, z), zmax = __builtin_fmaxf(zmax, z);
-          }
-          const float umag = __builtin_fmaxf(__builtin_fmaxf(__builtin_fabsf(umin), __builtin_fabsf(umax)), __builtin_fmaxf(__builtin_fabsf(vmin), __builtin_fabsf(vmax)));
-          const float e = 2.0f * cload(&fr->ferr) * __builtin_amdgcn_rcpf(zmin) * (1.0f + 0x1p-20f) + (0x1p-19f * umag + 0x1p-12f);
-          const bool sane = zmin > 0.0f && zmax <= (float)(kWinCzRatio * (1.0 - 0x1p-20)) * zmin && umin > -65536.0f && umax < 65536.0f &&
-                            vmin > -65536.0f && vmax < 65536.0f && e < 0.25f;
-          if (sane) {
-            const int cxc = a.W / 2, cyc = a.H / 2;
-            const int x0 = (int)__builtin_ceilf(umin - 0.5f - e) + cxc, x1 = (int)__builtin_floorf(umax + 0.5f + e) + cxc;
-            const int y0 = (int)__builtin_ceilf(vmin - 0.5f - e) + cyc, y1 = (int)__builtin_floorf(vmax + 0.5f + e) + cyc;
-            if (x0 >= -kValidMargin && y0 >= -kValidMargin && x1 < a.W + kValidMargin && y1 < a.H + kValidMargin &&
-                x1 - x0 < kWindowCols && y1 - y0 < kWindowRows) {
-              wp.origin = (uint32_t)(x0 + kValidMargin) | ((uint32_t)(y0 + kValidMargin) << 16);
-              wp.ax = (float)(hxa - (double)(x0 + kWinAnchorX - cxc) * cza);
-              wp.ay = (float)(hya - (double)(y0 + kWinAnchorY - cyc) * cza);
-              wp.acz = z0;
-            }
-          }
-        }
-      }
-      if (want) {
-        if (wp.origin != kNotWanted)
-          tile[4 * g + q][threadIdx.x] = wp;
-        else
-          classes[row + m] = (uint8_t)(c | CLASS_NO_WINDOW);
-      }
-    }
-  }
-  __syncthreads();
-  const int v = threadIdx.x & (kOriginViews - 1);
-  const int m = g_lo + v;
-  if (v < group_views && m < m_end) {
-#pragma unroll
-    for (int it = 0; it < 8; ++it) {
-      const int b = (threadIdx.x >> 3) + 32 * it;
-      const WinPair wp = tile[v][b];
-      if (wp.origin != kNotWanted) origins[rows[b] + m] = wp;
-    }
-  }
-}
-
 
 __device__ __forceinline__ bool slot_to_brick(const TileArgs &a, int slot, int &bx, int &by, int &bz) {
   const int within = slot & 31;
@@ -903,6 +791,8 @@
     mixed += __shfl_xor(mixed, off, 64);
     light += __shfl_xor(light, off, 64);
   }
+  const int tk = a.kpad / max(a.bricks_z, 1);
+  if (bz * tk + tk > a.nz) light = 0;
   if (a.flags & TILE_FLAG_COST_ORDER) {
     const int lv = !in_grid ? 255 : (mixed == 0 ? kCostLevels - 1 : (kCostLevels - 1) - (mixed * (kCostLevels - 1) + a.n_maps - 1) / a.n_maps);
     if (exists && part == 0) level[slot] = (uint8_t)lv;
@@ -917,7 +807,7 @@
   }
   if (exists && part == 0)
     {
-      const int cost2 = a.win_origin ? 2 * light + 5 * (mixed - light) : 2 * mixed;
+      const int cost2 = a.windows ? 2 * light + 5 * (mixed - light) : 2 * mixed;
       level[slot] = !in_grid ? 255 : (cost2 >= a.n_maps ? 0 : (cost2 * 2 >= a.n_maps ? 1 : (cost2 * 8 >= a.n_maps ? 2 : 3)));
     }
 }
@@ -1009,24 +899,6 @@
 hipError_t launch_build_pyramid_levels(int64_t n_maps, const PyramidDesc &P, DepthTile *pyramids, hipStream_t stream) {
   if (n_maps <= 0 || P.n_levels <= 1) return hipSuccess;
   hipLaunchKernelGGL(pyramid_levels_kernel, dim3((unsigned)n_maps), dim3(1024), 0, stream, P, pyramids);
-  return hipGetLastError();
-}
-
-hipError_t launch_window_origins(const TileArgs &a, const MapRec *maps_dev, int tk, uint8_t *classes, int general_k,
-                                 hipStream_t stream) {
-  if (general_k || !a.win_origin || a.n_maps <= 0) return hipSuccess;
-  const int bz_count = std::min(2 * a.super_z, a.bricks_z - 2 * a.sbz_first);
-  const int64_t n_bricks = (int64_t)a.wbricks_x * a.wbricks_y * bz_count;
-  if (n_bricks <= 0) return hipSuccess;
-  const int64_t brick_groups = (n_bricks + 255) / 256;
-  const int span = a.first_map + a.n_maps - (a.first_map & ~3);
-  int group_views = kOriginViews;
-  while (group_views > 4 && brick_groups * ((span + group_views - 1) / group_views) < 2048) group_views >>= 1;
-  const dim3 grid((unsigned)brick_groups, (unsigned)((span + group_views - 1) / group_views));
-  if (a.rotated)
-    hipLaunchKernelGGL((window_origin_kernel<true>), grid, dim3(256), 0, stream, a, maps_dev, tk, classes, a.win_origin, group_views);
-  else
-    hipLaunchKernelGGL((window_origin_kernel<false>), grid, dim3(256), 0, stream, a, maps_dev, tk, classes, a.win_origin, group_views);
   return hipGetLastError();
 }
 
diff --git a/cudadepthmapintegration_amd/csrc/fusion_kernels.h b/cudadepthmapintegration_amd/csrc/fusion_kernels.h
--- a/cudadepthmapintegration_amd/csrc/fusion_kernels.h
+++ b/cudadepthmapintegration_amd/csrc/fusion_kernels.h
@@ -110,6 +110,16 @@
   float ax, ay, acz;
 };
 static_assert(sizeof(WinPair) == 16, "WinPair layout");
+constexpr int kEntryViews = 32;
+struct alignas(128) WinEntryRecs {
+  double rt2[4][kEntryViews];
+  double crow[8][kEntryViews];
+  float s8[8][3][kEntryViews];
+  float s16[8][3][kEntryViews];
+  float ferr[kEntryViews];
+  float e_abs[kEntryViews];
+};
+static_assert(sizeof(WinEntryRecs) == 12 * 256 + 50 * 128, "WinEntryRecs: whole lines per field");
 
 enum KMode : int {
   K_GENERAL = 0,
@@ -171,10 +181,9 @@
   unsigned long long *wg_times;
   int64_t wg_times_n;
   int32_t *queue_heads;
-  WinPair *win_origin;
-  int64_t win_delta;
+  const WinEntryRecs *win_entries;
+  int32_t windows, pad4;
   const WinRec *win_recs;
-  const FootRec *foot_recs;
   int32_t vb_bytes, vb_rowskip;
   int32_t win_cx, win_cy;
 };
@@ -244,8 +253,6 @@
                                int64_t n_maps, int W, int H, const PyramidDesc &desc, DepthTile *pyramids, uint8_t *valid, uint32_t *bits,
                                unsigned long long *counters, hipStream_t stream);
 hipError_t launch_build_pyramid_levels(int64_t n_maps, const PyramidDesc &desc, DepthTile *pyramids, hipStream_t stream);
-hipError_t launch_window_origins(const TileArgs &args, const MapRec *maps_dev, int tk, uint8_t *classes, int general_k,
-                                 hipStream_t stream);
 hipError_t launch_classify_bricks(const TileArgs &args, const MapRec *maps_dev, const PyramidDesc &desc, int tk,
                                   uint8_t *classes, uint8_t *coarse, int general_k, hipStream_t stream);
 int64_t coarse_class_bytes(const TileArgs &args, int tk);
diff --git a/cudadepthmapintegration_amd/csrc/fusion_tile.hip b/cudadepthmapintegration_amd/csrc/fusion_tile.hip
--- a/cudadepthmapintegration_amd/csrc/fusion_tile.hip
+++ b/cudadepthmapintegration_amd/csrc/fusion_tile.hip
@@ -425,16 +425,72 @@
   int n_uniform = (!COUNT && KA(free_sums) != nullptr) ? 0 : -1;
   unsigned long long cnext = cload(crow + (first_map >> 3));
   [[maybe_unused]] uint32_t pair_a = 0, pair_b = 0;
+  constexpr uint32_t kNoWindow = 0xfffffffeu;
   for (int wbase = first_map & ~7; wbase < m_end; wbase += 8) {
     if constexpr (WIN) {
       if ((wbase & 24) == 0 || wbase == (first_map & ~7)) {
-        const kernarg_t ko = KFRESH();
-        if (ko->win_origin) {
-          typedef uint32_t u32x2 __attribute__((ext_vector_type(2)));
-          const u32x2 *row = reinterpret_cast<const u32x2 *>(ko->win_delta + 16 * (int64_t)reinterpret_cast<intptr_t>(crow));
-          const u32x2 pr = row[2 * (wbase & ~31) + lane];
-          pair_a = pr.x;
-          pair_b = pr.y;
+        if (kcount == TK) {
+          const kernarg_t ko = KFRESH();
+          constexpr uint32_t kWanted = (uint32_t)BRICK_MIXED | ((uint32_t)MIXED_FREE_OR_NODEPTH << 2);
+          int ev = lane >> 1;
+          asm volatile("" : "+v"(ev));
+          const int mv = (wbase & ~31) + ev;
+          uint8_t *const cbytes = const_cast<uint8_t *>(reinterpret_cast<const uint8_t *>(crow));
+          const bool in_range = (mv >= first_map) & (mv < m_end);
+          uint32_t c = BRICK_SKIP;
+          if (in_range) c = cbytes[mv];
+          const bool want = in_range && (c & 0x1fu) == kWanted;
+          if (ballot(want) != 0) {
+            const WinEntryRecs *const er = ko->win_entries + (wbase >> 5);
+            uint32_t origin = kNoWindow;
+            float a_own = 0.f, acz = 0.f;
+            int odd = lane & 1;
+            asm volatile("" : "+v"(odd));
+            auto swapped = [](int x) __attribute__((always_inline)) { return __builtin_amdgcn_update_dpp(0, x, 0xB1, 0xf, 0xf, false); };
+            if (want && er->e_abs[ev] < __builtin_inff()) {
+              auto lane0 = [](double x) __attribute__((always_inline)) {
+                return __hiloint2double(__builtin_amdgcn_readlane(__double2hiint(x), 0), __builtin_amdgcn_readlane(__double2loint(x), 0));
+              };
+              double wxa = lane0(wx), wya = lane0(wy), wza = lane0(wz0);
+              if constexpr (ROT) {
+                const czvec4 b = cload(reinterpret_cast<const czvec4 *>(ko->cz_table + (int64_t)k0 * 4));
+                wxa = (wxa + b[0]) + ko->g[3], wya = (wya + b[1]) + ko->g[7], wza = (wza + b[2]) + ko->g[11];
+              }
+              const float(*const scp)[3][kEntryViews] = TK == 16 ? er->s16 : er->s8;
+              const double(*const row)[kEntryViews] = er->crow + 4 * odd;
+              const double cza = ((er->rt2[0][ev] * wxa + er->rt2[1][ev] * wya) + er->rt2[2][ev] * wza) + er->rt2[3][ev];
+              const double ha = __builtin_fma(row[0][ev], wxa, __builtin_fma(row[1][ev], wya, __builtin_fma(row[2][ev], wza, row[3][ev])));
+              const float h0 = (float)ha, z0 = (float)cza;
+              float lo = __builtin_inff(), hi = -__builtin_inff(), zmin = __builtin_inff(), zmax = -__builtin_inff();
+#pragma unroll
+              for (int cnr = 0; cnr < 8; ++cnr) {
+                const float z = z0 + scp[cnr][2][ev];
+                const float r = __builtin_amdgcn_rcpf(z);
+                const float u = (h0 + scp[cnr][odd][ev]) * r;
+                lo = __builtin_fminf(lo, u), hi = __builtin_fmaxf(hi, u);
+                zmin = __builtin_fminf(zmin, z), zmax = __builtin_fmaxf(zmax, z);
+              }
+              const float mag = __builtin_fmaxf(__builtin_fabsf(lo), __builtin_fabsf(hi));
+              const float umag = __builtin_fmaxf(mag, __int_as_float(swapped(__float_as_int(mag))));
+              const float e = 2.0f * er->ferr[ev] * __builtin_amdgcn_rcpf(zmin) * (1.0f + 0x1p-20f) + (0x1p-19f * umag + 0x1p-12f);
+              const bool sane = zmin > 0.0f && zmax <= (float)(kWinCzRatio * (1.0 - 0x1p-20)) * zmin && lo > -65536.0f && hi < 65536.0f && e < 0.25f;
+              const int size = odd ? ko->H : ko->W;
+              const int centre = size / 2;
+              const int p0 = cvt_i32_f32(__builtin_ceilf(lo - 0.5f - e)) + centre, p1 = cvt_i32_f32(__builtin_floorf(hi + 0.5f + e)) + centre;
+              const bool fit_own = sane && p0 >= -kValidMargin && p1 < size + kValidMargin && p1 - p0 < (odd ? kWindowRows : kWindowCols);
+              const bool fit = fit_own && swapped(fit_own ? 1 : 0) != 0;
+              const int q0 = swapped(p0);
+              if (fit) {
+                origin = (uint32_t)(p0 + kValidMargin) | ((uint32_t)(q0 + kValidMargin) << 16);
+                a_own = (float)(ha - (double)(p0 + (odd ? kWinAnchorY : kWinAnchorX) - centre) * cza);
+                acz = z0;
+              }
+            }
+            const bool none = want && origin == kNoWindow;
+            if (none && odd == 0) cbytes[mv] = (uint8_t)(c | CLASS_NO_WINDOW);
+            pair_a = odd ? __float_as_uint(a_own) : origin;
+            pair_b = odd ? __float_as_uint(acz) : __float_as_uint(a_own);
+          }
         }
       }
     }
@@ -482,7 +538,14 @@
       }
       continue;
     }
-    [[maybe_unused]] const bool has_window = WIN && cbyte == ((unsigned)MIXED_FREE_OR_NODEPTH << 2 | BRICK_MIXED) && kcount == TK;
+    [[maybe_unused]] bool has_window = WIN && cbyte == ((unsigned)MIXED_FREE_OR_NODEPTH << 2 | BRICK_MIXED) && kcount == TK;
+    [[maybe_unused]] uint32_t org = 0;
+    if constexpr (WIN) {
+      if (has_window) {
+        org = (uint32_t)__builtin_amdgcn_readlane((int)pair_a, (m & 31) * 2);
+        has_window = org != kNoWindow;
+      }
+    }
 #ifdef DMI_TUNING
     ++dbg_cols;
     if ((kflags & TILE_FLAG_DBG_SKIP_WINDOW_PAIRS) && has_window) continue;
@@ -495,7 +558,6 @@
         if (dbg_cols == dbg_win) ++dbg_win_early;
 #endif
         const int pl = (m & 31) * 2;
-        const uint32_t org = (uint32_t)__builtin_amdgcn_readlane((int)pair_a, pl);
         const unsigned long long A2 = (unsigned long long)(uint32_t)__builtin_amdgcn_readlane((int)pair_b, pl) |
                                       ((unsigned long long)(uint32_t)__builtin_amdgcn_readlane((int)pair_a, pl + 1) << 32);
         const float acz = __int_as_float(__builtin_amdgcn_readlane((int)pair_b, pl + 1));
@@ -1283,7 +1345,7 @@
 hipError_t launch_types(const TileArgs &a, const FuseConfig &cfg, hipStream_t s) {
   constexpr bool f32_depth = std::is_same<DepthT, float>::value;
   const int shape = effective_shape(cfg.variant, !f32_depth, a.rotated != 0, cfg.general_k != 0);
-  const bool win = DMI_TIER1 != 0 && std::is_same<DepthT, float>::value && a.win_origin != nullptr && !cfg.count_hits && !cfg.general_k &&
+  const bool win = DMI_TIER1 != 0 && std::is_same<DepthT, float>::value && a.windows != 0 && !cfg.count_hits && !cfg.general_k &&
                    a.behind_mask != 0;
 #ifdef DMI_FAST_BUILD
   if (win) {
@@ -1372,8 +1434,6 @@
     const TileShape sh = tile_shape(cfg.variant, cfg.depth_is_f64 != 0, a.rotated != 0, cfg.general_k != 0);
     e = launch_classify_bricks(a, maps_dev, pyramid, sh.tk, const_cast<uint8_t *>(a.classes), coarse_classes, cfg.general_k, stream);
     if (e != hipSuccess) return e;
-    e = launch_window_origins(a, maps_dev, sh.tk, const_cast<uint8_t *>(a.classes), cfg.general_k, stream);
-    if (e != hipSuccess) return e;
 #ifdef DMI_TUNING
     if (const char *env = getenv("DMI_DEBUG_CLASS_REMAP")) {
       const int64_t n = (int64_t)a.wbricks_x * a.wbricks_y * a.bricks_z * (int64_t)a.class_pitch;
```

After: 3073 (median of 6 runs). Within noise of the previous version (+0.9%).
